# RNG65536/CUDA-volpath

Hardware: AMD Instinct MI355X
Metric: Msamples/sec (WxHxspp) + achieved HBM GB/s, Julia 256^3 @ 800x600 (higher is better)
Workload: dtype f32; 1 GPU; julia256_800x600_global_majorant; image=800x600, estimator=global_majorant, bound_brick=1, rng=philox2x32-7, parallelism=pixel-tiles x1

## Files before the change

### cuda-volpath_amd/csrc/vp_context.cpp

```cpp
#include "vp_state.h"

namespace vph __attribute__((visibility("hidden")))
{
State                      g_default;
static thread_local State* t_current = nullptr;
State& cur() { return t_current ? *t_current : g_default; }

int fail(int code, const char* fmt, ...)
{
    char    buf[512];
    va_list ap;
    va_start(ap, fmt);
    vsnprintf(buf, sizeof buf, fmt, ap);
    va_end(ap);
    G.err = buf;
    return code;
}
[[noreturn]] void die(const char* what)
{
    fprintf(stderr, "volpath_hip: %s: %s\n", what, G.err.c_str());
    exit(EXIT_FAILURE);
}
int ensure_device()
{
    if (G.dev_ready)
    {
        HIPCHK(hipSetDevice(G.device));
        return VP_OK;
    }
    int n = 0;
    if (hipGetDeviceCount(&n) != hipSuccess || n <= 0) return fail(VP_E_NODEVICE, "no HIP device visible");
    if (G.device >= n) return fail(VP_E_NODEVICE, "device %d out of range (%d visible)", G.device, n);
    HIPCHK(hipSetDevice(G.device));
    hipDeviceProp_t prop;
    HIPCHK(hipGetDeviceProperties(&prop, G.device));
    if (strncmp(prop.gcnArchName, "gfx950", 6) != 0)
        return fail(VP_E_NODEVICE, "device %d is %s; this library carries gfx950 code only", G.device, prop.gcnArchName);
    G.num_cu = prop.multiProcessorCount;
    HIPCHK(hipStreamCreateWithFlags(&G.own_stream, hipStreamNonBlocking));
    if (!G.stream) G.stream = G.own_stream;
    HIPCHK(hipMalloc((void**)&G.d_queue, 2 * kTargets * kQueueWords * sizeof(unsigned)));
    HIPCHK(hipMalloc((void**)&G.d_counters, kCounterWords * sizeof(unsigned long long)));
    HIPCHK(hipMemset(G.d_counters, 0, kCounterWords * sizeof(unsigned long long)));
    HIPCHK(hipMalloc((void**)&G.d_cancel, 3 * sizeof(unsigned)));
    HIPCHK(hipMemset(G.d_cancel, 0, 3 * sizeof(unsigned)));
    G.S.sun_cos = 94.0f / sqrtf(94.0f * 94.0f + 0.45f * 0.45f);
    G.S.cam_z   = (float)(-1.0f / tan((double)54.43f * 0.00872664626));
    auto knob = [](const char* name, long lo, long hi, long& out) {
        const char* e = getenv(name);
        if (!e || !*e) return false;
        char* end = nullptr;
        long  v   = strtol(e, &end, 10);
        if (*end || v < lo || v > hi)
        {
            fprintf(stderr, "volpath_hip: ignoring %s=%s (allowed %ld..%ld)\n", name, e, lo, hi);
            return false;
        }
        out = v;
        return true;
    };
    long v;
    if (knob("VP_WAIT_LANES", 1, 64, v)) { G.wait_lanes = (unsigned)v; G.wait_lanes_set = true; }
    if (knob("VP_WAIT_ITERS", VP_STEPS_PER_PASS, 1 << 20, v)) G.wait_iters = (unsigned)v;
    if (knob("VP_SETUP_LANES", 1, 64, v)) G.setup_lanes = (unsigned)v;
    if (knob("VP_END_LANES", 1, 64, v)) G.end_lanes = (unsigned)v;
    if (knob("VP_LIGHT_WAIT_ITERS", VP_STEPS_PER_PASS, 1 << 20, v)) G.light_wait_iters = (unsigned)v;
    if (knob("VP_STAGE_MB", 1, 256 << 10, v)) G.max_stage_bytes = (size_t)v << 20;
    if (knob("VP_BLOCKS_PER_CU", 1, 8, v)) G.blocks_per_cu = (unsigned)v;
    {
        long kmax = 0;
        while ((VP_CHUNK >> (kmax + 1)) >= 1) kmax++;
        if (knob("VP_CHUNK_FRAMES_LOG2", 0, kmax, v)) G.chunk_fshift = (unsigned)v;
    }
    if (knob("VP_NO_LDS_BOUNDS", 0, 1, v)) G.use_lds_bounds = v == 0;
    if (knob("VP_NO_LDS_HELPER", 0, 1, v)) G.lds_helper = v == 0;
    if (knob("VP_NO_LDS_COMPACT", 0, 1, v)) G.use_lds_compact = v == 0;
    if (knob("VP_LDS_COMPACT_CHROMATIC", 0, 1, v)) G.lds_compact_chromatic = v != 0;
    if (knob("VP_LDS_PAIRS", 0, 1, v)) G.lds_pairs = v != 0;
    if (knob("VP_CELL_BRICKS", 0, 1, v)) G.cell_bricks = (int)v;
    if (knob("VP_NO_CRAWL_TABLE", 0, 1, v)) G.use_crawl_table = v == 0;
    if (knob("VP_NO_EMPTY_TABLE", 0, 1, v)) G.use_empty_table = v == 0;
    if (knob("VP_NO_SUN_CLIP", 0, 1, v)) G.use_sun_clip = v == 0;
    if (knob("VP_DENSE_PERCENT", 0, 101, v)) G.dense_fraction = (float)v / 100.0f;
    if (knob("VP_NO_OPACITY_LDS", 0, 1, v)) G.opacity_lds = v == 0;
    if (knob("VP_NO_OPACITY_CELLS", 0, 1, v)) G.use_opacity_cells = v == 0;
    if (knob("VP_NO_LIGHT_CONST", 0, 1, v)) G.use_light_const = v == 0;
    if (knob("VP_NO_CONST_ROWS", 0, 1, v)) G.use_const_rows = v == 0;
    if (knob("VP_NO_APPROACH", 0, 1, v)) G.use_approach = v == 0;
    if (knob("VP_NO_APPROACH_LOCAL", 0, 1, v)) G.use_approach_local = v == 0;
    if (knob("VP_NO_APPROACH_TABLE", 0, 1, v)) G.use_approach_table = v == 0;
    if (knob("VP_APPROACH_FRAMES_LOG2", 0, 6, v)) G.approach_fshift_max = (unsigned)v;
    if (knob("VP_APPROACH_STEPS", 0, 1 << 30, v)) G.approach_steps = (unsigned)v;
    if (knob("VP_NO_LIGHT", 0, 1, v)) G.use_light = v == 0;
    if (knob("VP_NO_LIGHT_OVERLAP", 0, 1, v)) G.light_overlap = v == 0;
    if (knob("VP_NO_LIGHT_LOCAL", 0, 1, v)) G.use_light_local = v == 0;
    if (knob("VP_DEBUG_ONLY_CLASS", 0, 1, v)) G.debug_only_class = (int)v;
    if (knob("VP_GENERAL_BLOCKS_PER_CU", 1, 8, v)) G.general_blocks_per_cu = (unsigned)v;
    if (knob("VP_LIGHT_BLOCKS_PER_CU", 1, 8, v)) G.light_blocks_per_cu = (unsigned)v;
    if (knob("VP_THR_TABLE", 2, 1 << 20, v)) G.thr_entries = (unsigned)v;
    if (knob("VP_LOOKAHEAD", 0, 4096, v)) G.la_max = (int)v;
    if (knob("VP_LOOKAHEAD_OVERLAP_FROM", 1, 4096, v)) G.la_overlap_from = (int)v;
    if (knob("VP_LOOKAHEAD_RAMP_FROM", 2, 4096, v)) G.la_ramp_from = (int)v;
    if (knob("VP_LOOKAHEAD_FLOOR", 1, 4096, v)) G.la_floor = (int)v;
    if (knob("VP_LOOKAHEAD_DIV", 1, 16, v)) G.la_div = (int)v;
    if (knob("VP_LOOKAHEAD_NO_SPECULATION", 0, 1, v)) G.la_speculate = v == 0;
    if (knob("VP_NO_LA_CANCEL", 0, 1, v)) G.la_cancel = v == 0;
    if (knob("VP_NO_PIPELINE", 0, 1, v)) G.pipeline = v == 0;
    if (knob("VP_NO_EXIT", 0, 1, v)) G.use_exit = v == 0;
    if (knob("VP_EXIT_LOCAL", 0, 1, v)) { G.exit_local = v != 0; G.exit_local_auto = false; }
    if (knob("VP_EXIT_K", 1, VP_EXIT_TRIP, v)) G.exit_k = (unsigned)v;
    G.dev_ready = true;
    return VP_OK;
}


hipError_t create_internal_stream(hipStream_t* st)
{
    int lo = 0, hi = 0;
    if (hipDeviceGetStreamPriorityRange(&lo, &hi) != hipSuccess) { (void)hipGetLastError(); lo = hi = 0; }
    return hipStreamCreateWithPriority(st, hipStreamNonBlocking, lo);
}

int free_volume()
{
    G.epoch++;
    (void)la_quiesce();

    if (G.d_cells) HIPCHK(hipFree(G.d_cells));
    if (G.d_bounds) HIPCHK(hipFree(G.d_bounds));
    if (G.d_opacity) HIPCHK(hipFree(G.d_opacity));
    if (G.d_opacity_cells) { if (G.opacity_cells_on_host) HIPCHK(hipHostFree(G.h_opacity_cells)); else HIPCHK(hipFree(G.d_opacity_cells)); }
    G.d_opacity_cells = nullptr; G.h_opacity_cells = nullptr; G.S.opacity_cells = nullptr; G.opacity_cells_on_host = false;
    if (G.d_bound_codes) HIPCHK(hipFree(G.d_bound_codes));
    G.d_bound_codes = nullptr; G.bound_codes_ok = false;
    if (G.d_danger) HIPCHK(hipFree(G.d_danger));
    G.d_danger = nullptr;
    if (G.d_sunclip) HIPCHK(hipFree(G.d_sunclip));
    G.d_sunclip = nullptr; G.sunclip_key.clear();
    if (G.d_exit) HIPCHK(hipFree(G.d_exit));
    G.d_exit = nullptr;
    G.d_cells = G.d_bounds = nullptr;
    G.d_opacity   = nullptr;
    G.S.cells_u8  = nullptr;
    G.S.cells_f32 = nullptr;
    G.S.bounds_u8 = nullptr;
    G.S.bounds_f32 = nullptr;
    G.S.opacity    = nullptr;
    G.have_volume  = false;
    return VP_OK;
}

static int do_init_volume_(const void* h_volume, vp_extent ext, bool quantized, const vp_float3* bmin, const vp_float3* bmax);
int do_init_volume(const void* h_volume, vp_extent ext, bool quantized, const vp_float3* bmin, const vp_float3* bmax)
{
    int rc = do_init_volume_(h_volume, ext, quantized, bmin, bmax);
    if (rc)
    {
        std::string why = G.err;
        (void)free_volume();
        G.err = why;
    }
    return rc;
}
int do_init_volume_(const void* h_volume, vp_extent ext, bool quantized, const vp_float3* bmin, const vp_float3* bmax)
{
    G.epoch++;
    (void)la_quiesce();

    int rc = ensure_device();
    if (rc) return rc;
    if (ext.width == 0 || ext.height == 0 || ext.depth == 0) return fail(VP_E_ARG, "empty volume extent");
    size_t n = ext.width * ext.height * ext.depth;
    if (n > ((size_t)1 << 32) - 1) return fail(VP_E_ARG, "volume of %zu voxels exceeds the 2^32 cell index", n);
    if (ext.width > 4096 || ext.height > 4096 || ext.depth > 4096) return fail(VP_E_ARG, "volume edge > 4096 voxels");
    HIPCHK(hipStreamSynchronize(G.stream));
    rc = free_volume();
    if (rc) return rc;
    const int nx = (int)ext.width, ny = (int)ext.height, nz = (int)ext.depth;
    SceneDev& S = G.S;
    S.nx = nx; S.ny = ny; S.nz = nz;
    if (bmin && bmax)
    {
        S.bmin[0] = bmin->x; S.bmin[1] = bmin->y; S.bmin[2] = bmin->z;
        S.bmax[0] = bmax->x; S.bmax[1] = bmax->y; S.bmax[2] = bmax->z;
    }
    else
    {
        S.bmin[0] = -1.0f; S.bmin[1] = -(float)ny / (float)nx; S.bmin[2] = -(float)nz / (float)nx;
        S.bmax[0] = 1.0f;  S.bmax[1] = (float)ny / (float)nx;  S.bmax[2] = (float)nz / (float)nx;
    }
    for (int a = 0; a < 3; a++) S.linv[a] = 1.0f / (S.bmax[a] - S.bmin[a]);
    G.quant = quantized;
    struct Scratch
    {
        void* p[3] = {nullptr, nullptr, nullptr};
        ~Scratch() { for (void* q : p) if (q) (void)hipFree(q); }
    } tmp;
    void*& d_raw = tmp.p[0];
    void*& d_ta  = tmp.p[1];
    void*& d_tb  = tmp.p[2];
    const size_t vbytes = n * (quantized ? 1 : 4);
    HIPCHK(hipMalloc(&d_raw, vbytes));
    HIPCHK(hipMemcpyAsync(d_raw, h_volume, vbytes, hipMemcpyHostToDevice, G.stream));
    const size_t ncells_bricks = (((size_t)nx + 3) / 4) * (((size_t)ny + 3) / 4) * (((size_t)nz + 3) / 4) * 64;
    const bool   bricks = G.cell_bricks > 0;
    const size_t ncells = bricks ? ncells_bricks : n;
    S.cell_bricks = bricks ? 1 : 0;
    HIPCHK(hipMalloc(&G.d_cells, ncells * (quantized ? 8 : 32)));
    if (bricks && ncells != n) HIPCHK(hipMemsetAsync(G.d_cells, 0, ncells * (quantized ? 8 : 32), G.stream));
    if (quantized) launch_pack_u8((const unsigned char*)d_raw, (uint2*)G.d_cells, nx, ny, nz, bricks, G.stream);
    else launch_pack_f32((const float*)d_raw, (float*)G.d_cells, nx, ny, nz, bricks, G.stream);
    HIPCHK(hipGetLastError());
    G.brick  = G.brick_next;
    G.radius = bound_radius(nx, 0.05f ) + (G.brick > 1 ? 1 : 0);
    int shift = 0;
    while ((1 << shift) < G.brick) shift++;
    S.brick_shift = shift;
    S.bnx = (nx + G.brick - 1) / G.brick; S.bny = (ny + G.brick - 1) / G.brick; S.bnz = (nz + G.brick - 1) / G.brick;
    const size_t nb    = (size_t)S.bnx * S.bny * S.bnz;
    const size_t psize = quantized ? 2 : 8;
    HIPCHK(hipMalloc(&d_ta, n * psize));
// ... 223 lines not shown
}
void gamma_correct(vp_float4* dst, vp_float4* src, int size, float s, float gamma)
{
    if (ensure_device()) die("gamma_correct");
    launch_gamma((float4*)dst, (const float4*)src, size, s, 1.0f / gamma, G.stream);
}

const char* vp_last_error(void) { return G.err.c_str(); }
const char* vp_version(void) { return "volpath_hip 0.3 (gfx950)"; }
int vp_device_count(void)
{
    int n = 0;
    if (hipGetDeviceCount(&n) != hipSuccess) return 0;
    return n;
}
int vp_set_device(int device)
{
    if (G.dev_ready && device != G.device)
        return fail(VP_E_STATE, "this context is bound to device %d; use vp_ctx_create(%d) for another GPU", G.device, device);
    G.device = device;
    return ensure_device();
}

struct vp_ctx { State st; };
vp_ctx* vp_ctx_create(int device)
{
    int n = 0;
    if (hipGetDeviceCount(&n) != hipSuccess || device < 0 || device >= n)
    {
        fail(VP_E_NODEVICE, "vp_ctx_create: device %d not visible (%d devices)", device, n);
        return nullptr;
    }
    vp_ctx* c = new vp_ctx();
    c->st.device = device;
    State* prev = t_current;
    t_current   = &c->st;
    int rc      = ensure_device();
    std::string why = c->st.err;
    t_current   = prev;
    if (rc)
    {
        delete c;
        fail(rc, "vp_ctx_create(%d): %s", device, why.c_str());
        return nullptr;
    }
    return c;
}
int vp_ctx_set_current(vp_ctx* ctx)
{
    t_current = ctx ? &ctx->st : nullptr;
    if (G.dev_ready) HIPCHK(hipSetDevice(G.device));
    return VP_OK;
}
vp_ctx* vp_ctx_get_current(void) { return t_current ? reinterpret_cast<vp_ctx*>(t_current) : nullptr; }
int vp_ctx_device(void) { return G.device; }
int vp_ctx_destroy(vp_ctx* ctx)
{
    if (!ctx) return VP_OK;
    State* prev = t_current;
    t_current   = &ctx->st;
    State& D    = ctx->st;
    int rc = VP_OK;
    if (D.dev_ready)
    {
        (void)hipSetDevice(D.device);
        (void)hipStreamSynchronize(D.stream);
        (void)la_quiesce();
        rc = free_volume();
        free_envmap();
        for (auto& sl : D.la)
        {
            if (sl.done) (void)hipEventDestroy(sl.done);
            if (sl.stream) (void)hipStreamDestroy(sl.stream);
        }
        for (auto& ev : D.events) { (void)hipEventDestroy(ev.first); (void)hipEventDestroy(ev.second); }
        for (auto& ev : D.class_events) { (void)hipEventDestroy(ev.a); (void)hipEventDestroy(ev.b); }
        for (auto e : D.event_pool) (void)hipEventDestroy(e);
        (void)pipe_quiesce();
        for (hipStream_t st : D.pipe_stream) if (st) (void)hipStreamDestroy(st);
        for (hipEvent_t e : {D.pipe_done[0], D.pipe_done[1], D.pipe_free[0], D.pipe_free[1], D.pipe_gate[0], D.pipe_gate[1], D.pipe_fence_ev, D.last_end,
                             D.class_last_end[0], D.class_last_end[1], D.class_last_end[2]})
            if (e) (void)hipEventDestroy(e);
        D.d_crawl.release(); D.d_seg.release(); D.d_sub_cls.release(); D.d_tiles.release(); D.d_act.release(); D.d_act_scratch.release();
        for (void* q : {(void*)D.d_thr, (void*)D.d_sunclip, (void*)D.d_bound_codes, (void*)D.d_light_flag, (void*)D.d_tile_rows, (void*)D.d_tile_scratch})
            if (q) (void)hipFree(q);
        for (RenderTarget& t : D.target)
        {
            if (t.aux_stream) { (void)hipStreamSynchronize(t.aux_stream); (void)hipStreamDestroy(t.aux_stream); }
            t.stage.release();
            t.handover.release();
            for (hipEvent_t e : t.aux_ev) if (e) (void)hipEventDestroy(e);
        }
        if (D.d_queue) (void)hipFree(D.d_queue);
        if (D.d_counters) (void)hipFree(D.d_counters);
        if (D.ctrl_stream) (void)hipStreamDestroy(D.ctrl_stream);
        if (D.d_cancel) (void)hipFree(D.d_cancel);
        if (D.own_stream) (void)hipStreamDestroy(D.own_stream);
    }
    t_current = (prev == &ctx->st) ? nullptr : prev;
    delete ctx;
    if (G.dev_ready) (void)hipSetDevice(G.device);
    return rc;
}
int vp_accumulate(vp_float4* dst, const vp_float4* src, size_t n)
{
    int rc = ensure_device();
    if (rc) return rc;
    if (!dst || !src) return fail(VP_E_ARG, "vp_accumulate: null pointer");
    if (n) launch_accumulate((float4*)dst, (const float4*)src, n, G.stream);
    HIPCHK(hipGetLastError());
    return VP_OK;
}
int vp_tile_owner(unsigned tx, unsigned ty, int world)
{
    if (world < 1) return -1;
    return (int)((tx + vp::tile_row_shift(ty, (unsigned)world)) % (unsigned)world);
}
int vp_set_stream(void* s)
{
    int rc = ensure_device();
    if (rc) return rc;
    HIPCHK(hipStreamSynchronize(G.stream));
    if (la_quiesce()) return VP_E_NODEVICE;
    G.stream = s ? (hipStream_t)s : G.own_stream;
    return VP_OK;
}
void* vp_get_stream(void)
{
    if (ensure_device()) return nullptr;
    return (void*)G.stream;
}
int vp_synchronize(void)
{
    int rc = ensure_device();
    if (rc) return rc;
    HIPCHK(hipStreamSynchronize(G.stream));
    return VP_OK;
}
int vp_set_estimator(int est)
{
    if (int rc = pipe_quiesce()) return rc;
    if (est != VP_EST_GLOBAL && est != VP_EST_DECOMP && est != VP_EST_BOUNDED) return fail(VP_E_ARG, "unknown estimator %d", est);
    G.est = est;
    return VP_OK;
}
int vp_set_rng(int mode, uint32_t k0, uint32_t k1)
{
    if (int rc = pipe_quiesce()) return rc;
    if (mode != VP_RNG_SAMPLERH && mode != VP_RNG_PHILOX && mode != VP_RNG_PHILOX7) return fail(VP_E_ARG, "unknown rng %d", mode);
    G.rng = mode; G.key0 = k0; G.key1 = k1;
    return VP_OK;
}
int vp_set_exit_flights(int mode)
{
    if (mode < 0 || mode > 2) return fail(VP_E_ARG, "exit flights: 0 off, 1 global-majorant estimator (default), 2 every estimator that has them");
    int rc = ensure_device();
    if (rc || (rc = pipe_quiesce())) return rc;
    G.use_exit = mode != 0; G.exit_local = mode == 2; G.exit_local_auto = false;
    if (G.use_exit && G.have_volume && !G.d_exit && G.d_danger)
    {
        if (la_quiesce()) return VP_E_NODEVICE;
        const size_t n = (size_t)G.S.nx * G.S.ny * G.S.nz;
        if (hipMalloc((void**)&G.d_exit, 3 * n) == hipSuccess)
        {
            launch_exit_table(G.d_danger, G.d_exit, G.S.nx, G.S.ny, G.S.nz, G.stream);
            HIPCHK(hipGetLastError());
        }
// ... 277 lines not shown
```

### cuda-volpath_amd/csrc/vp_device.h

```cpp
#pragma once
#include <hip/hip_runtime.h>
#include <stdint.h>

#include "vp_math.h"

namespace vp
{
struct f3 { float x, y, z; };
VP_ARITH_BEGIN
__device__ __forceinline__ f3 mk3(float x, float y, float z) { return f3{x, y, z}; }
__device__ __forceinline__ f3 operator+(f3 a, f3 b) { return f3{a.x + b.x, a.y + b.y, a.z + b.z}; }
__device__ __forceinline__ f3 operator-(f3 a, f3 b) { return f3{a.x - b.x, a.y - b.y, a.z - b.z}; }
__device__ __forceinline__ f3 operator*(f3 a, f3 b) { return f3{a.x * b.x, a.y * b.y, a.z * b.z}; }
__device__ __forceinline__ f3 operator*(f3 a, float s) { return f3{a.x * s, a.y * s, a.z * s}; }
__device__ __forceinline__ f3 operator/(f3 a, float s) { return f3{a.x / s, a.y / s, a.z / s}; }
__device__ __forceinline__ float dot(f3 a, f3 b) { return a.x * b.x + a.y * b.y + a.z * b.z; }
__device__ __forceinline__ f3 cross(f3 a, f3 b)
{
    return f3{a.y * b.z - a.z * b.y, a.z * b.x - a.x * b.z, a.x * b.y - a.y * b.x};
}
__device__ __forceinline__ f3 normalize(f3 v) { return v * rsqrt_(dot(v, v)); }
__device__ __forceinline__ f3 normalize_ieee(f3 v) { return v * (1.0f / __builtin_sqrtf(dot(v, v))); }
__device__ __forceinline__ float max3(f3 v) { return fmaxf(fmaxf(v.x, v.y), v.z); }
__device__ __forceinline__ float min3(f3 v) { return fminf(fminf(v.x, v.y), v.z); }
// ... 292 lines not shown
    if (lz) hi = lo;
    float x00 = lerpf(lo.x, lo.y, fx);
    float x10 = lerpf(lo.z, lo.w, fx);
    float x01 = lerpf(hi.x, hi.y, fx);
    float x11 = lerpf(hi.z, hi.w, fx);
    float y0  = lerpf(x00, x10, fy);
    float y1  = lerpf(x01, x11, fy);
    return lerpf(y0, y1, fz);
}

template <bool QUANT>
__device__ __forceinline__ void sample_bound(const SceneDev& S, f3 pos, float& bmax, float& bmin)
{
    f3  p = to_local(S, pos);
    int i = axis_point(p.x, S.nx) >> S.brick_shift;
    int j = axis_point(p.y, S.ny) >> S.brick_shift;
    int k = axis_point(p.z, S.nz) >> S.brick_shift;
    size_t o = (size_t)((unsigned)i + (unsigned)S.bnx * ((unsigned)j + (unsigned)S.bny * (unsigned)k));
    if (QUANT)
    {
        unsigned short v = reinterpret_cast<const unsigned short*>(S.bounds_u8)[o];
        bmax = (float)(v & 0xffu) * VP_U8_SCALE;
        bmin = (float)(v >> 8) * VP_U8_SCALE;
    }
    else
    {
        float2 v = reinterpret_cast<const float2*>(S.bounds_f32)[o];
        bmax = v.x;
        bmin = v.y;
    }
}

__device__ __forceinline__ f3 eval_envmap(const SceneDev& S, f3 dir)
{
    float phi   = acosf_(dir.y);
    float theta = atanf_(dir.z / dir.x) + kPi2;
    if (dir.x < 0.0f) theta += kPi;
    float  u = theta * k1TwoPi;
    float  v = phi * k1Pi;
    int    i = axis_point(u, S.env_w);
    int    j = axis_point(v, S.env_h);
    float4 t = S.env[(size_t)i + (size_t)S.env_w * (size_t)j];
    return f3{t.x, t.y, t.z};
}

__device__ __forceinline__ float luminance(f3 c)
{
    return (float)((double)c.x * 0.2126 + (double)c.y * 0.7152 + (double)c.z * 0.0722);
}
__device__ __forceinline__ int cdf_search(const float* cdf, int n, float r)
{
    int begin = 0, end = n - 1;
    while (end > begin)
    {
        int   mid = begin + (end - begin) / 2;
        float c   = cdf[mid];
        if (c >= r) end = mid;
        else begin = mid + 1;
    }
    return begin;
}
__device__ __forceinline__ float sample_envmap(const SceneDev& S, float& u, float& v, f3& c)
{
    int iy = cdf_search(S.env_cdf_y, S.env_h, v);
    int ix = cdf_search(S.env_cdf_x + (size_t)iy * (size_t)S.env_w, S.env_w, u);
    u = ((float)ix + 0.5f) / (float)S.env_w;
    v = ((float)iy + 0.5f) / (float)S.env_h;
    int    i = axis_point(u, S.env_w);
    int    j = axis_point(v, S.env_h);
    float4 t = S.env[(size_t)i + (size_t)S.env_w * (size_t)j];
    c        = f3{t.x, t.y, t.z};
    return luminance(c) * S.env_pdfnorm_alt;
}
__device__ __forceinline__ f3 uv_to_dir(float u, float v)
{
    float theta = u * kTwoPi;
    float phi   = v * kPi;
    float st, ct, sp, cp;
    sincosf_(theta, st, ct);
    sincosf_(phi, sp, cp);
    return f3{sp * st, cp, sp * -ct};
}

__device__ __forceinline__ bool intersect_box(f3 o, f3 d, const SceneDev& S, float& tnear, float& tfar)
{
#ifndef VP_EXP_BOX_PARALLEL
    float tmn, tmx;
    {
        const float ir = 1.0f / d.x, tb = ir * (S.bmin[0] - o.x), tt = ir * (S.bmax[0] - o.x);
        tmn = fminf(tt, tb); tmx = fmaxf(tt, tb);
    }
    __builtin_amdgcn_sched_barrier(0);
    float tmn_y, tmx_y;
    {
        const float ir = 1.0f / d.y, tb = ir * (S.bmin[1] - o.y), tt = ir * (S.bmax[1] - o.y);
        tmn_y = fminf(tt, tb); tmx_y = fmaxf(tt, tb);
    }
    __builtin_amdgcn_sched_barrier(0);
    float tmn_z, tmx_z;
    {
        const float ir = 1.0f / d.z, tb = ir * (S.bmin[2] - o.z), tt = ir * (S.bmax[2] - o.z);
        tmn_z = fminf(tt, tb); tmx_z = fmaxf(tt, tb);
    }
    const float lt = max3(f3{tmn, tmn_y, tmn_z}), st_ = min3(f3{tmx, tmx_y, tmx_z});
    tnear = lt; tfar = st_;
    return st_ > lt && st_ >= 1e-3f;
#endif
    f3 invR = f3{1.0f / d.x, 1.0f / d.y, 1.0f / d.z};
    f3 tbot = invR * (f3{S.bmin[0], S.bmin[1], S.bmin[2]} - o);
    f3 ttop = invR * (f3{S.bmax[0], S.bmax[1], S.bmax[2]} - o);
    f3 tmin = f3{fminf(ttop.x, tbot.x), fminf(ttop.y, tbot.y), fminf(ttop.z, tbot.z)};
    f3 tmax = f3{fmaxf(ttop.x, tbot.x), fmaxf(ttop.y, tbot.y), fmaxf(ttop.z, tbot.z)};
    float largest_tmin  = max3(tmin);
    float smallest_tmax = min3(tmax);
    tnear = largest_tmin;
    tfar  = smallest_tmax;
    return smallest_tmax > largest_tmin && smallest_tmax >= 1e-3f;
}

__device__ __forceinline__ bool intersect_box_inv(f3 o, f3 invR, const SceneDev& S, float& tnear, float& tfar)
{
    f3 tbot = invR * (f3{S.bmin[0], S.bmin[1], S.bmin[2]} - o);
    f3 ttop = invR * (f3{S.bmax[0], S.bmax[1], S.bmax[2]} - o);
    f3 tmin = f3{fminf(ttop.x, tbot.x), fminf(ttop.y, tbot.y), fminf(ttop.z, tbot.z)};
    f3 tmax = f3{fmaxf(ttop.x, tbot.x), fmaxf(ttop.y, tbot.y), fmaxf(ttop.z, tbot.z)};
    float largest_tmin  = max3(tmin);
    float smallest_tmax = min3(tmax);
    tnear = largest_tmin;
    tfar  = smallest_tmax;
    return smallest_tmax > largest_tmin && smallest_tmax >= 1e-3f;
}

__device__ __forceinline__ void camera_ray(const SceneDev& S, unsigned width, unsigned height, unsigned px, unsigned py, f3& ro, f3& rd)
{
    float u = ((float)px * 2.0f - (float)width) / (float)width;
    float v = ((float)py * 2.0f - (float)height) / (float)width;
    ro      = f3{S.cam[3], S.cam[7], S.cam[11]};
    f3 dv   = f3{u, v, S.cam_z};
    rd      = normalize_ieee(f3{dot(dv, f3{S.cam[0], S.cam[1], S.cam[2]}), dot(dv, f3{S.cam[4], S.cam[5], S.cam[6]}), dot(dv, f3{S.cam[8], S.cam[9], S.cam[10]})});
}

__host__ __device__ __forceinline__ void subpixel_offset(unsigned px, unsigned py, unsigned frame, unsigned m, unsigned& i, unsigned& j)
{
    const unsigned h = wang_hash(((px << 16) | py) ^ 0x9E3779B9u);
    const unsigned k = (frame + h) & ((1u << (2u * m)) - 1u);
    i = j = 0u;
#pragma unroll
    for (unsigned b = 0; b < 3u; b++)
        if (b < m)
        {
            i |= ((k >> (2u * m - 1u - 2u * b)) & 1u) << b;
            j |= ((k >> (2u * m - 2u - 2u * b)) & 1u) << b;
        }
}

struct Frame
{
    f3 n, t, b;
    __device__ __forceinline__ explicit Frame(f3 normal)
    {
        n    = normal;
        f3 a = (__builtin_fabsf(n.x) >= 0.1f) ? f3{0.0f, 1.0f, 0.0f} : f3{1.0f, 0.0f, 0.0f};
        t    = normalize(cross(a, n));
        b    = cross(n, t);
    }
    __device__ __forceinline__ f3 to_world(f3 c) const { return (t * c.x + b * c.y) + n * c.z; }
};

__device__ __forceinline__ f3 hg_sample_local(float g, float rnd0, float rnd1)
{
    float cos_theta;
    if (__builtin_fabsf(g) > 1e-6f)
    {
        float s   = 2.0f * rnd0 - 1.0f;
        float f   = div_(1.0f - g * g, 1.0f + g * s);
        cos_theta = div_(0.5f, g) * (1.0f + g * g - f * f);
        cos_theta = fmaxf(0.0f, fminf(1.0f, cos_theta));
    }
    else
        cos_theta = 2.0f * rnd0 - 1.0f;
    float sin_theta = sqrt_(1.0f - cos_theta * cos_theta);
    float sp, cp;
    sincos_turns_(rnd1, sp, cp);
    return f3{cp * sin_theta, sp * sin_theta, cos_theta};
}
__device__ __forceinline__ float hg_eval(float g, float cos_theta)
{
    return div_(1.0f - g * g, (4.0f * kPi) * pow15f_(1.0f + g * g - (2.0f * g) * cos_theta));
}

__device__ __forceinline__ float hyperion_s(int n_minus)
{
    return fmaxf(0.0f, fminf(1.0f, (float)n_minus * 0.066666666666666666667f));
}

enum : int
{
    CR_G    = 0,
    CR_OMG2 = 1,
    CR_OPG2 = 2,
// ... 55 lines not shown
```

### cuda-volpath_amd/csrc/vp_integrator.h

```cpp
enum : int
{
    ST_DONE    = 0,
    ST_SETUP   = 1,
    ST_TRACK   = 2,
    ST_SHADOW  = 3,
    EV_SCATTER = 4,
    EV_NEE     = 5,
    EV_BG      = 6,
    EV_WRITE   = 7,
    EV_MIS     = 8,
    EV_HG      = 9
};

#ifndef VP_PAD_STEP
#define VP_PAD_STEP 0
#endif
#ifndef VP_PAD_FETCH
#define VP_PAD_FETCH 0
#endif
#ifndef VP_PAD_EOF
#define VP_PAD_EOF 0
#endif
#ifndef VP_PAD_SETUP
#define VP_PAD_SETUP 0
// ... 22 lines not shown
    }
}

__device__ __forceinline__ unsigned lane_rank(unsigned long long mask)
{
    return __builtin_amdgcn_mbcnt_hi((unsigned)(mask >> 32), __builtin_amdgcn_mbcnt_lo((unsigned)mask, 0u));
}

template <class T, bool COLD>
struct ColdVal;
template <class T>
struct ColdVal<T, true>
{
    static_assert(sizeof(T) == sizeof(float), "one LDS word per lane and field");
    float* p;
    __device__ __forceinline__ explicit ColdVal(float* q) : p(q) {}
    __device__ __forceinline__ operator T() const { return __builtin_bit_cast(T, *p); }
    __device__ __forceinline__ ColdVal& operator=(T v) { *p = __builtin_bit_cast(float, v); return *this; }
};
template <class T>
struct ColdVal<T, false>
{
    T v = T();
    __device__ __forceinline__ explicit ColdVal(float*) {}
    __device__ __forceinline__ operator T() const { return v; }
    __device__ __forceinline__ ColdVal& operator=(T w) { v = w; return *this; }
};
template <bool COLD, int STRIDE>
struct ColdF3;
template <int STRIDE>
struct ColdF3<true, STRIDE>
{
    float* p;
    __device__ __forceinline__ explicit ColdF3(float* q) : p(q) {}
    __device__ __forceinline__ operator f3() const { return f3{p[0], p[STRIDE], p[2 * STRIDE]}; }
    __device__ __forceinline__ ColdF3& operator=(f3 v) { p[0] = v.x; p[STRIDE] = v.y; p[2 * STRIDE] = v.z; return *this; }
};
template <int STRIDE>
struct ColdF3<false, STRIDE>
{
    f3 v = {};
    __device__ __forceinline__ explicit ColdF3(float*) {}
    __device__ __forceinline__ operator f3() const { return v; }
    __device__ __forceinline__ ColdF3& operator=(f3 w) { v = w; return *this; }
};
__device__ __forceinline__ float null_collision_in_empty_space(float t, float sigma_t_prime, float inv_sigma_t)
{
    float mn = __builtin_fabsf(sigma_t_prime * t);
    float Pn = (mn + mn) + mn;
    return t * (sigma_t_prime * wdiv_(inv_sigma_t * Pn, Pn));
}
__device__ __forceinline__ bool null_collision_is_identity(f3 t, float sigma_t_prime, float inv_sigma_t)
{
    const float Ps = __builtin_fabsf(0.0f * t.x) + __builtin_fabsf(0.0f * t.y) + __builtin_fabsf(0.0f * t.z);
    const float Pn = __builtin_fabsf(sigma_t_prime * t.x) + __builtin_fabsf(sigma_t_prime * t.y) + __builtin_fabsf(sigma_t_prime * t.z);
    const float c  = Ps + Pn;
    return Ps == 0.0f && sigma_t_prime * wdiv_(inv_sigma_t * c, Pn) == 1.0f;
}

__global__ void light_identity_k(ParamDev P, int local, const unsigned* mask, unsigned* flag)
{
    const unsigned b = threadIdx.x;
    if (local && !(mask[b >> 5] >> (b & 31u) & 1u)) return;
    if (!local && b) return;
    const float max_sig = max3(f3{P.sigma_t[0], P.sigma_t[1], P.sigma_t[2]});
    const float s       = hyperion_s(0 - 5);
    float sigma_t_prime;
    if (local)
    {
        const float reduction   = (1.0f - s) + s * (1.0f - P.g);
        const float cur_density = reduction * P.density;
        const float d_max       = fmaxf(0.0001f, (float)b * VP_U8_SCALE);
        sigma_t_prime           = max_sig * cur_density * d_max;
    }
    else
    {
        const float cur_density = (1.0f - s) * P.density + s * P.density * (1.0f - P.g);
        sigma_t_prime           = max_sig * cur_density;
    }
    const float inv_sigma_t = rcp_(sigma_t_prime);
    if (!(null_collision_in_empty_space(1.0f, sigma_t_prime, inv_sigma_t) == 1.0f)) atomicAnd(flag, 0u);
}

#ifndef VP_LOCAL_MIN_WAVES
#define VP_LOCAL_MIN_WAVES 6
#endif
constexpr int render_min_waves(int est, bool count, int ldsb, bool ach, bool mis, int trk, bool light, bool cancel)
{
    if (VP_MIN_WAVES > 1) return VP_MIN_WAVES;
    if (light) return count ? 5 : (est != EST_GLOBAL ? VP_LIGHT_LOCAL_MIN_WAVES : VP_LIGHT_MIN_WAVES);
    if (mis || ldsb == 1) return 1;
    if (count) return 4;
    if (est == EST_GLOBAL && trk == 0) return VP_GLOBAL_MIN_WAVES;
    if (trk) return 4;
    return (ach && !cancel) ? VP_LOCAL_MIN_WAVES : 5;
}
template <int EST, class RNG, bool QUANT, bool COUNT, int LDSB, bool ACH, bool MIS, int TRK, bool LIGHT = false, bool CANCEL = false>
__global__ __launch_bounds__(LDSB == 1 ? VP_BLOCK_LDS : VP_BLOCK, render_min_waves(EST, COUNT, LDSB, ACH, MIS, TRK, LIGHT, CANCEL))
void render_k(SceneDev S, LaunchDev L)
{
    __shared__ unsigned short lds_bounds[LDSB == 1 ? VP_LDS_BOUND_ENTRIES : 1];
    __shared__ unsigned lds_codes[LDSB == 2 ? VP_LDS_BOUND_ENTRIES / 16 : 1];
    if (LDSB == 2)
    {
        const uint4* src = reinterpret_cast<const uint4*>(L.bound_codes);
        uint4*       dst = reinterpret_cast<uint4*>(lds_codes);
        const int    n16 = (S.bnx * S.bny * S.bnz + 63) / 64;
        for (int w = threadIdx.x; w < n16; w += VP_BLOCK) dst[w] = src[w];
        __syncthreads();
    }
    if (LDSB == 1)
    {
        const uint4* src = reinterpret_cast<const uint4*>(S.bounds_u8);
        uint4*       dst = reinterpret_cast<uint4*>(lds_bounds);
        const int    n16 = (S.bnx * S.bny * S.bnz * 2 + 15) / 16;
        for (int w = threadIdx.x; w < n16; w += VP_BLOCK_LDS) dst[w] = src[w];
        __syncthreads();
    }
    constexpr unsigned KARG_L_   = ((sizeof(SceneDev) + alignof(LaunchDev) - 1) / alignof(LaunchDev)) * alignof(LaunchDev);
    constexpr unsigned KARG_WDS_ = (KARG_L_ + sizeof(LaunchDev) + 3) / 4;
    __shared__ __attribute__((aligned(16))) unsigned kargs_lds_[KARG_WDS_];
    {
        const unsigned* src = (const unsigned*)__builtin_amdgcn_kernarg_segment_ptr();
        for (unsigned w = threadIdx.x; w < KARG_WDS_; w += (LDSB == 1 ? VP_BLOCK_LDS : VP_BLOCK)) kargs_lds_[w] = src[w];
    }
    constexpr bool LOCAL = EST != EST_GLOBAL;
    constexpr bool TAB = TRK == 0 && LDSB != 1 && !LIGHT && !MIS;
    __shared__ __attribute__((aligned(16))) float coll_tab_[TAB ? VP_COLL_ROWS : 1][CR_WORDS];
    if (TAB && threadIdx.x < VP_COLL_ROWS)
        coll_row_fill(coll_tab_[threadIdx.x], (int)threadIdx.x, L.P.g, L.P.density, max3(f3{L.P.sigma_t[0], L.P.sigma_t[1], L.P.sigma_t[2]}), LOCAL);
    __syncthreads();
    auto coll_row = [&](int n) __attribute__((always_inline)) -> const float* {
        return TAB ? coll_tab_[n < 0 ? 0 : (n > VP_COLL_ROWS - 1 ? VP_COLL_ROWS - 1 : n)] : nullptr;
    };
    constexpr bool EARLY = RNG::kShadowSubstream && !MIS && !LIGHT;
    constexpr bool APPR = EST == EST_GLOBAL && TRK == 0 && !LIGHT && !MIS;
    constexpr bool APPR_L = EST == EST_DECOMP && TRK == 0 && !LIGHT && !MIS;
    constexpr bool EXITC = TRK == 0 && !MIS && !LIGHT && EST != EST_BOUNDED && (QUANT || EST == EST_GLOBAL);
    const ParamDev& P = L.P;
    const f3    sig_t     = f3{P.sigma_t[0], P.sigma_t[1], P.sigma_t[2]};
    const f3    sig_s     = sig_t * f3{P.albedo[0], P.albedo[1], P.albedo[2]};
    const float max_sig   = max3(sig_t);
    const float min_sig   = min3(sig_t);
    const float density   = P.density;

    int      st = ST_DONE;
    bool     exhausted = false;
    constexpr bool COLD = LDSB != 1 && !LIGHT;
    constexpr int  CS_  = COLD ? VP_BLOCK : 1;
    static_assert(!COLD || (LOCAL ? VP_LOCAL_MIN_WAVES : VP_GLOBAL_MIN_WAVES) * (14 * VP_BLOCK * 4 + KARG_WDS_ * 4 + VP_COLL_ROWS * CR_WORDS * 4 + (LDSB == 2 ? VP_LDS_BOUND_ENTRIES / 4 : 0)) <= VP_LDS_BYTES_PER_CU,
                  "cold per-path state: more workgroups per CU than the LDS holds -- lower VP_*_MIN_WAVES for this ARCH");
    __shared__ float cold_[COLD ? 14 : 1][CS_];
    float* const cold_p = &cold_[0][COLD ? threadIdx.x : 0];
    ColdF3<COLD, CS_>       rad(cold_p), pd(cold_p + 3 * CS_);
    ColdVal<float, COLD>    ph(cold_p + 6 * CS_), phase_g(cold_p + 7 * CS_);
    ColdVal<unsigned, COLD> item(cold_p + 8 * CS_);
    ColdVal<unsigned, COLD> px(cold_p + 9 * CS_), py(cold_p + 10 * CS_);
    ColdVal<int, COLD>      frame(cold_p + 11 * CS_);
    ColdVal<int, COLD>      nsc(cold_p + 12 * CS_);
    ColdVal<unsigned, COLD> rng_saved(cold_p + 13 * CS_);
    if (COLD) { rad = f3{0.0f, 0.0f, 0.0f}; pd = f3{0.0f, 0.0f, 0.0f}; ph = 0.0f; phase_g = 0.0f; item = 0u; px = 0u; py = 0u; frame = 0; nsc = 0; rng_saved = 0u; }
    RNG      rng;
    f3       ro = {}, rd = {};
    f3       inv_rd = {};
    f3       thr = {};
    int      seg = 0;
    float    dist = 0, t_end = 0;
    float    t_far = 0, distc = 0, inv_sigma = 0, inv_sigma_t = 0, sigma_t_prime = 0, sigma_c = 0;
    float    cur_density = 0, d_max = 0;
    f3       nee_a = {};
    int      terms = 0;
    f3       nee_c = {}, nee_t = {}, seg_o = {};
    int      nee_stage = 0;
    float    sh_inv_sigma = 0, sh_density = 0;
    float    sig_base = density;
    int      chan = 0;
    float    t_empty = 0.0f;
    float    t_clip = 1e30f;
    bool     ex_clear = false;
    unsigned long long c_load = 0, c_xtest = 0, c_xout = 0, c_xok = 0;
    unsigned zrun = 0;

    unsigned long long c_den = 0, c_bnd = 0, c_opa = 0, c_env = 0, c_sca = 0, c_smp = 0;
    unsigned long long d_iter = 0, d_act = 0, d_outer = 0, d_shadow = 0;
    constexpr bool PROF = COUNT && VP_PROFILE_BLOCKS;
    unsigned long long t_slow = 0, t_fast = 0, t_mark = PROF ? __builtin_amdgcn_s_memtime() : 0ull;
    enum { B_SETUP, B_HALF, B_LOOK, B_EXIT, B_SCATTER, B_NEE, B_HG, B_BG, B_WRITE, B_REFILL, B_GSETUP, B_FETCH, B_ZERO, B_ZERO_SH, B_EXITT, B_NBLK };
    unsigned long long bw[B_NBLK] = {}, bl[B_NBLK] = {};
    unsigned long long hist[3][8] = {};
    unsigned long long ctrl_w = 0, ctrl_l = 0;
    auto tally = [&](int b, bool on) __attribute__((always_inline)) {
        if (PROF)
        {
            unsigned long long m = __ballot(on);
            if (m)
            {
                bw[b] += 1; bl[b] += (unsigned)__popcll(m);
                const int h = b == B_SCATTER ? 0 : b == B_EXIT ? 1 : b == B_SETUP ? 2 : -1;
                if (h >= 0) hist[h][((unsigned)__popcll(m) - 1u) >> 3] += 1;
            }
        }
    };

    const unsigned lane = threadIdx.x & 63u;
    unsigned chunk_s = 0, chunk_n = 0;
    unsigned chunk_q = 0, chunk_f0 = 0;
    bool     queue_empty = false;
    unsigned q_cur   = __builtin_amdgcn_s_getreg((4 - 1) << 11 | 20) & (VP_NQUEUES - 1);
    unsigned q_tried = 0;
    unsigned end_skipped = 0;
    unsigned visits = 0;

    for (;;)
    {
        if (PROF && lane == 0) d_outer++;
        {
#ifdef VP_EXP_FLAT_KARGS
        const char* kargs_ = (const char*)__builtin_amdgcn_kernarg_segment_ptr();
        asm volatile("" : "+s"(kargs_));
#else
        unsigned ko_ = 0;
        asm volatile("" : "+v"(ko_));
        const char* kargs_ = reinterpret_cast<const char*>(kargs_lds_) + ko_;
#endif
        const SceneDev&  S = *reinterpret_cast<const SceneDev*>(kargs_);
        const LaunchDev& L = *reinterpret_cast<const LaunchDev*>(kargs_ + KARG_L_);
        const ParamDev&  P = L.P;
        const f3 sun_dir   = f3{S.sun_dir[0], S.sun_dir[1], S.sun_dir[2]};
        const f3 sun_power = f3{S.sun_power[0], S.sun_power[1], S.sun_power[2]};
        auto start_shadow = [&](f3 end, float inv_s, float den, unsigned stage) __attribute__((always_inline)) {
            f3    sd = normalize(end - ro);
            float tn, tf;
            bool  hitv = intersect_box(ro, sd, S, tn, tf);
            if (!hitv)
            {
                nee_a = f3{1.0f, 1.0f, 1.0f};
                st    = EV_NEE;
            }
            else
            {
                if (tn < 0.0f) tn = 0.0f;
                f3 se       = ro - end;
                t_end       = fminf(tf, sqrt_(dot(se, se)));
                dist        = tn;
                terms       = 0;
                rd          = sd;
                inv_sigma   = inv_s;
                cur_density = den;
                st          = ST_SHADOW;
                rng_saved = rng.enter_shadow(2u * (unsigned)(int)nsc + stage);
                if (COUNT) t_clip = 1e30f;
                if (RNG::kShadowSubstream && stage == 0u && L.sun_clip)
                {
                    f3    pl = to_local(S, ro);
                    int   ci, cj, ck;
                    float w_;
                    axis_linear(pl.x, S.nx, ci, w_);
                    axis_linear(pl.y, S.ny, cj, w_);
                    axis_linear(pl.z, S.nz, ck, w_);
                    const unsigned n = L.sun_clip[(size_t)((unsigned)ci + __umul24((unsigned)S.nx, (unsigned)cj + __umul24((unsigned)S.ny, (unsigned)ck)))];
                    if (n != 0xffffu)
                    {
                        const float tc = (float)n * L.clip_ds;
                        if (COUNT && !L.count_clips) t_clip = tc;
                        else t_end = fminf(t_end, tc);
                    }
                }
            }
        };
        auto segment_medium = [&]() __attribute__((always_inline)) {
            if (LOCAL && TAB) cur_density = coll_row(nsc - 5)[CR_DENS];
            else if (LOCAL)
            {
                float s         = hyperion_s(nsc - 5);
                phase_g         = (1.0f - s) * P.g;
                float reduction = (1.0f - s) + s * (1.0f - P.g);
                cur_density     = TRK ? reduction * sig_base : reduction * density;
            }
        };
        auto next_segment = [&]() __attribute__((always_inline)) {
            st = ST_SETUP;
            if (LOCAL) dist = -1.0f;
            if (EXITC) terms = L.exit_start;
            if (EST == EST_GLOBAL) nsc = nsc + 1;
            if (EST == EST_BOUNDED) seg++;
            if ((EST == EST_BOUNDED ? seg : nsc) >= 800) st = EV_WRITE;
            segment_medium();
        };
        auto finish_light = [&]() __attribute__((always_inline)) {
            rad = rad + sun_power * (((ACH ? f3{thr.x, thr.x, thr.x} : thr) * ph) * nee_a);
            rd  = pd;
            next_segment();
        };
        tally(B_SCATTER, st == EV_SCATTER);
        if (!LIGHT && st == EV_SCATTER)
        {
            vp_pad<VP_PAD_COLL>();
            if (COUNT) c_sca++;
            if (PROF) zrun = 0;
            t_empty = 0.0f;
            if (LOCAL) nsc = nsc + 1;
            const int          n2   = LOCAL ? (nsc - 5) : (nsc - 4);
            const float* const row2 = coll_row(n2);
            const float* const rowp = coll_row(n2 - 1);
            float s2 = hyperion_s(n2);
            float dp2, stp2;
            if (TAB)
            {
                dp2  = row2[CR_DENS];
                stp2 = LOCAL ? row2[CR_STP] * d_max : row2[CR_STP];
            }
            else if (TRK)
            {
                thr  = thr * f3{P.albedo[0], P.albedo[1], P.albedo[2]};
                stp2 = LOCAL ? ((1.0f - s2) + s2 * (1.0f - P.g)) * sig_base : (1.0f - s2) * sig_base + s2 * sig_base * (1.0f - P.g);
                dp2  = stp2;
            }
            else if (LOCAL)
            {
                float reduction2 = (1.0f - s2) + s2 * (1.0f - P.g);
                dp2              = reduction2 * density;
                stp2             = max_sig * dp2 * d_max;
            }
            else
            {
                dp2  = (1.0f - s2) * density + s2 * density * (1.0f - P.g);
                stp2 = max_sig * dp2;
            }
            ph = TAB ? hg_eval_row(rowp, dot(rd, sun_dir)) : hg_eval(phase_g, dot(rd, sun_dir));
            pd = rd;
            if (EARLY)
            {
                Frame fr(rd);
                float r0 = rng.next_a();
                float r1 = rng.next_b();
                pd       = normalize(fr.to_world(TAB ? hg_sample_local_row(rowp, r0, r1) : hg_sample_local(phase_g, r0, r1)));
                if (LOCAL) { const f3 pdv = pd; inv_rd = f3{rcp_(pdv.x), rcp_(pdv.y), rcp_(pdv.z)}; }
            }
            if (MIS)
            {
                sh_inv_sigma = rcp_(stp2);
                sh_density   = dp2;
                nee_stage    = 0;
                nee_c        = sun_power;
                nee_t        = (ACH ? f3{thr.x, thr.x, thr.x} : thr) * ph;
            }
            if (EST == EST_DECOMP && frame > 10 && nsc > 20)
            {
                float op = sample_float_cells(S, S.opacity_cells, ro);
// ... 957 lines not shown
```

### cuda-volpath_amd/csrc/vp_kernels.h

```cpp
#pragma once
#include <hip/hip_runtime.h>

#include "vp_device.h"

#define VP_BLOCK 256
#ifndef VP_BLOCK_LDS
#define VP_BLOCK_LDS 512
#endif
#ifndef VP_MIN_WAVES
#define VP_MIN_WAVES 1
#endif
#define VP_LDS_BYTES_PER_CU (160 * 1024)
#define VP_LDS_BOUND_ENTRIES 32768
#ifndef VP_CHUNK
#define VP_CHUNK 128
#endif
#define VP_NQUEUES 8
#define VP_QUEUE_STRIDE 16
#ifndef VP_WAIT_LANES
#define VP_WAIT_LANES 28
#endif
#ifndef VP_WAIT_ITERS
#define VP_WAIT_ITERS 16
#endif
#ifndef VP_END_LANES
#define VP_END_LANES 4
#endif
#ifndef VP_SETUP_LANES
#define VP_SETUP_LANES 8
#endif
#ifndef VP_LIGHT_MIN_WAVES
#define VP_LIGHT_MIN_WAVES 8
#endif
#ifndef VP_PROFILE_BLOCKS
#define VP_PROFILE_BLOCKS 0
#endif
#ifndef VP_GLOBAL_MIN_WAVES
#define VP_GLOBAL_MIN_WAVES 7
#endif
#ifndef VP_LIGHT_LOCAL_MIN_WAVES
#define VP_LIGHT_LOCAL_MIN_WAVES 7
#endif
#ifndef VP_LIGHT_STEPS_PER_PASS
#define VP_LIGHT_STEPS_PER_PASS 16
#endif
#ifndef VP_STEPS_PER_PASS
#define VP_STEPS_PER_PASS 4
#endif
#define VP_EXIT_TRIP 64

namespace vp
{
__host__ __device__ inline unsigned tile_row_shift(unsigned ty, unsigned world) { return ((ty * 0x9E3779B1u) >> 15) % world; }
constexpr int EST_GLOBAL = 0, EST_DECOMP = 1, EST_BOUNDED = 2;
constexpr int RNG_SAMPLERH = 0, RNG_PHILOX = 1, RNG_PHILOX7 = 2;

struct LaunchDev
{
    ParamDev P;
    int      frame0, nframes;
    unsigned nslots;
    unsigned total_items;
    const unsigned* pixels;
    unsigned stage_stride;
    unsigned slot_base;
    float4*  out;
    float4*  stage;
    const float4* crawl;
    unsigned* queue;
    unsigned chunk_fshift;
    unsigned q_start[VP_NQUEUES + 1];
    unsigned long long* counters;
    unsigned key0, key1;
    unsigned wait_lanes, wait_iters;
    unsigned end_lanes;
    unsigned setup_lanes;
    const unsigned short* sun_clip;
    float    clip_ds;
    unsigned count_clips;
    const float* thr_table;
    unsigned thr_n;
    uint2*   approach_aux;
    unsigned approach;
    unsigned approach_fshift;
    unsigned approach_steps;
    const unsigned char* exit_oct;
    int      exit_start;
    unsigned exit_nbytes;
    unsigned exit_bytes;
    unsigned* cancel;
    unsigned  batch_id;
    unsigned      const_from;
    const float4* stage_const;
    const unsigned* bound_codes;
    unsigned        bound_pal[2];
    const float4* seg_table;
    unsigned sub_shift;
};

void launch_render(const SceneDev& S, const LaunchDev& L, int est, int rng, bool quant, bool count, int lds_form, bool mis, int trk,
                   int blocks, hipStream_t st);
void launch_render_fast(const SceneDev& S, const LaunchDev& L, int est, int rng, bool quant, bool count, int lds_form, bool mis, int trk,
                        int blocks, hipStream_t st);
void launch_render_light(const SceneDev& S, const LaunchDev& L, int est, int rng, bool quant, bool count, int blocks, hipStream_t st);
void launch_miss_fill(const SceneDev& S, const LaunchDev& L, bool local_estimator, hipStream_t st);
void launch_approach(const SceneDev& S, const LaunchDev& L, int est, int rng, bool quant, hipStream_t st);
void launch_approach_fast(const SceneDev& S, const LaunchDev& L, int est, int rng, bool quant, hipStream_t st);
unsigned segment_table_records(void);
void launch_segment_table(const SceneDev& S, unsigned width, unsigned height, const float4* crawl, const unsigned* pixels, unsigned nslots, float4* seg,
                          hipStream_t st);
void launch_thr_table(const ParamDev& P, float* table, unsigned count, hipStream_t st);
void launch_bound_bytes(const unsigned char* bounds, size_t nbricks, unsigned* mask, hipStream_t st);
void launch_light_identity(const ParamDev& P, bool local, const unsigned* mask, unsigned* flag, hipStream_t st);
void launch_light_identity_fast(const ParamDev& P, bool local, const unsigned* mask, unsigned* flag, hipStream_t st);
inline unsigned pixel_list_blocks(unsigned ntiles) { return (unsigned)(((size_t)ntiles * 64 + 1023) / 1024); }
void launch_pixel_lists(unsigned width, unsigned height, unsigned rank, unsigned world, unsigned ntiles, const unsigned* d_row_start,
                        const float4* table, const unsigned char* cls, unsigned* d_block_counts, unsigned* d_totals, unsigned* d_out, hipStream_t st);
void launch_subpixel_classes(const float4* fine, unsigned width, unsigned height, unsigned shift, unsigned char* cls, hipStream_t st);
void launch_env_tables(const float4* env, int w, int h, float* lum, float* row_sum, float* cdf_x, float* cdf_y, float* pdfnorm_alt,
                       hipStream_t st);
void launch_crawl_table(const SceneDev& S, bool quant, unsigned width, unsigned height, bool control_draw, const unsigned char* danger, float4* table,
                        hipStream_t st);
void launch_danger(const SceneDev& S, bool quant, unsigned char* out, unsigned long long* marked, hipStream_t st);
float sun_clip_step(const SceneDev& S);
void launch_sun_clip(const SceneDev& S, const unsigned char* danger, float ds, unsigned short* out, hipStream_t st);
void launch_empty_table(const SceneDev& S, unsigned width, unsigned height, const unsigned char* danger, float4* table, hipStream_t st);
void launch_exit_table(const unsigned char* danger, unsigned char* planes, int nx, int ny, int nz, hipStream_t st);
void launch_reduce(const LaunchDev& L, hipStream_t st);
struct PixelStatsDev { double sum_y, sum_y2; unsigned n, flags; };
struct StatsDev
{
    PixelStatsDev* stats;
    unsigned adaptive;
    unsigned min_frames;
    double   tol, fl;
};
void launch_reduce_stats(const LaunchDev& L, const StatsDev& T, hipStream_t st);
inline unsigned compact_blocks(unsigned n) { return (n + 1023u) / 1024u; }
void launch_compact_active(const unsigned* src, const unsigned n[3], unsigned width, const PixelStatsDev* stats, unsigned* d_block_counts,
                           unsigned* d_totals, unsigned* d_out, hipStream_t st);
void launch_scale_by_count(float4* dst, const float4* src, const PixelStatsDev* stats, int size, float s, hipStream_t st);
void launch_stats_rel_error(float* dst, const PixelStatsDev* stats, int size, float floor_y, hipStream_t st);
void launch_pack_u8(const unsigned char* vol, uint2* cells, int nx, int ny, int nz, bool bricks, hipStream_t st);
void launch_pack_f32(const float* vol, float* cells, int nx, int ny, int nz, bool bricks, hipStream_t st);
void launch_opacity(const SceneDev& S, bool quant, bool lds, const float dir[3], float* out, hipStream_t st);
void launch_build_bounds(const void* d_vol, bool quant, void* d_out, void* d_tmp_a, void* d_tmp_b, int nx, int ny, int nz, int radius, int brick,
                         hipStream_t st);
void launch_julia(unsigned char* grid, int n, hipStream_t st);
void launch_cloud(float* grid, int n, unsigned seed, hipStream_t st);
void launch_scale(float4* dst, const float4* src, int size, float s, hipStream_t st);
void launch_gamma(float4* dst, const float4* src, int size, float s, float inv_gamma, hipStream_t st);
void launch_accumulate(float4* dst, const float4* src, size_t n, hipStream_t st);
void launch_test_hg(const float* g, const float* r0, const float* r1, const float* nrm, const float* cosq, float* dir, float* ev, int n, hipStream_t st);
void launch_test_box(const SceneDev& S, const float* o, const float* d, int* hit, float* tn, float* tf, int n, hipStream_t st);
void launch_test_env(const SceneDev& S, const float* d, float* out, int n, hipStream_t st);
void launch_test_math(int which, const float* in, float* out, int n, hipStream_t st);
void launch_test_hg_fast(const float* g, const float* r0, const float* r1, const float* nrm, const float* cosq, float* dir, float* ev, int n, hipStream_t st);
void launch_test_math_fast(int which, const float* in, float* out, int n, hipStream_t st);
void launch_test_rng(int mode, unsigned x, unsigned y, unsigned f, unsigned k0, unsigned k1, int n, float* out, hipStream_t st);
void launch_test_density(const SceneDev& S, bool quant, const float* pos, float* out, int n, hipStream_t st);
}
```

### cuda-volpath_amd/csrc/vp_kernels.hip

```cpp
#include <hip/hip_runtime.h>

#include <cmath>
#include <cstdio>
#include <cstdlib>

#include "vp_device.h"
#include "vp_kernels.h"

namespace vp
{
#include "vp_integrator.h"

__global__ void thr_table_k(ParamDev P, float* table, unsigned count)
{
    if (threadIdx.x || blockIdx.x) return;
    const float max_sig       = max3(f3{P.sigma_t[0], P.sigma_t[1], P.sigma_t[2]});
    const float s             = hyperion_s(0 - 5);
    const float cur_density   = (1.0f - s) * P.density + s * P.density * (1.0f - P.g);
    const float sigma_t_prime = max_sig * cur_density;
    const float inv_sigma_t   = 1.0f / sigma_t_prime;
    float t = 1.0f;
    for (unsigned n = 0; n < count; n++)
    {
        table[n] = t;
// ... 38 lines not shown
        bool  hit = intersect_box_inv(ro, inv_rd, S, t_near, tf);
        t_near    = fmaxf(t_near, 0.0f);
        float t_far = fminf(tf, 0.05f);
        if (!hit || !(t_near >= t_far)) break;
        float bx, by;
        sample_bound<QUANT>(S, ro + rd * t_near, bx, by);
        draws += (control_draw && by > 0.0f) ? 2u : 1u;
        ro = ro + rd * t_far;
        t_left -= t_far;
    }
    table[2 * idx]     = make_float4(ro.x, ro.y, ro.z, u2f(segs | (draws << 16)));
    table[2 * idx + 1] = make_float4(t_left > 0.0f ? t_left : 0.0f, cls, 0.0f, 0.0f);
}

template <bool QUANT>
__global__ __launch_bounds__(256) void danger_k(SceneDev S, unsigned char* out, unsigned long long* marked)
{
    size_t n   = (size_t)S.nx * S.ny * S.nz;
    size_t idx = (size_t)blockIdx.x * blockDim.x + threadIdx.x;
    if (idx >= n) return;
    int i = (int)(idx % S.nx), j = (int)((idx / S.nx) % S.ny), k = (int)(idx / ((size_t)S.nx * S.ny));
    bool any = false;
    for (int dk = -1; dk <= 1; dk++)
        for (int dj = -1; dj <= 1; dj++)
            for (int di = -1; di <= 1; di++)
            {
                int a = min(max(i + di, 0), S.nx - 1), b = min(max(j + dj, 0), S.ny - 1), c = min(max(k + dk, 0), S.nz - 1);
                size_t o = cell_index(S, a, b, c);
                if (QUANT) { uint2 v = S.cells_u8[o]; any = any || (v.x | v.y) != 0u; }
                else
                {
                    const float4* q = reinterpret_cast<const float4*>(S.cells_f32) + o * 2;
                    float4 lo = q[0], hi = q[1];
                    any = any || lo.x != 0.0f || lo.y != 0.0f || lo.z != 0.0f || lo.w != 0.0f || hi.x != 0.0f || hi.y != 0.0f || hi.z != 0.0f || hi.w != 0.0f;
                }
            }
    bool self;
    {
        size_t o = cell_index(S, i, j, k);
        if (QUANT) { uint2 v = S.cells_u8[o]; self = (v.x | v.y) != 0u; }
        else
        {
            const float4* q = reinterpret_cast<const float4*>(S.cells_f32) + o * 2;
            float4 lo = q[0], hi = q[1];
            self = lo.x != 0.0f || lo.y != 0.0f || lo.z != 0.0f || lo.w != 0.0f || hi.x != 0.0f || hi.y != 0.0f || hi.z != 0.0f || hi.w != 0.0f;
        }
    }
    out[idx] = (unsigned char)((any ? 1 : 0) | (self ? 2 : 0));
    if (marked)
    {
        const unsigned long long m = __ballot(any);
        if ((threadIdx.x & 63u) == (unsigned)__builtin_ctzll(m | (1ull << 63)) && m) atomicAdd(marked, (unsigned long long)__popcll(m));
    }
}
__global__ __launch_bounds__(256) void exit_dir_slice_k(const unsigned char* danger, unsigned char* plane, int nx, int ny, int nz, int axis, int a, int up)
{
    const int n[3]  = {nx, ny, nz};
    const int B     = axis == 0 ? 1 : 0, C = axis == 2 ? 1 : 2;
    const int nb    = n[B], nc = n[C], na = n[axis];
    const int t     = blockIdx.x * blockDim.x + threadIdx.x;
    if (t >= nb * nc) return;
    const int b = t % nb, c = t / nb;
    const size_t st[3] = {1, (size_t)nx, (size_t)nx * ny};
    auto at = [&](int ia, int ib, int ic) -> size_t {
        ib = min(max(ib, 0), nb - 1); ic = min(max(ic, 0), nc - 1);
        return (size_t)ia * st[axis] + (size_t)ib * st[B] + (size_t)ic * st[C];
    };
    const int  an   = up ? a + 1 : a - 1;
    const bool more = an >= 0 && an < na;
    unsigned   bits = 0;
    for (int q = 0; q < 4; q++)
    {
        const int sb = (q & 1) ? 1 : -1, sc = (q & 2) ? 1 : -1;
        const unsigned bit = (up ? 1u : 0u) | ((q & 1) ? 2u : 0u) | ((q & 2) ? 4u : 0u);
        bool ok = !((danger[at(a, b, c)] | danger[at(a, b + sb, c)] | danger[at(a, b, c + sc)] | danger[at(a, b + sb, c + sc)]) & 1);
        if (ok && more)
            ok = ((plane[at(an, b, c)] & plane[at(an, b + sb, c)] & plane[at(an, b, c + sc)] & plane[at(an, b + sb, c + sc)]) >> bit) & 1u;
        bits |= ok ? (1u << bit) : 0u;
    }
    unsigned char* out = plane + at(a, b, c);
    const unsigned mine = up ? 0xaau : 0x55u;
    *out = (unsigned char)((*out & ~mine) | bits);
}
__global__ __launch_bounds__(256) void sun_clip_k(SceneDev S, const unsigned char* danger, float ds, unsigned short* out)
{
    const size_t n   = (size_t)S.nx * S.ny * S.nz;
    const size_t idx = (size_t)blockIdx.x * blockDim.x + threadIdx.x;
    if (idx >= n) return;
    if (!(danger[idx] & 2)) { out[idx] = 0xffffu; return; }
    const int i = (int)(idx % S.nx), j = (int)((idx / S.nx) % S.ny), k = (int)(idx / ((size_t)S.nx * S.ny));
    auto mid = [](int c, int nc) -> float {
        const float lo = c == 0 ? -0.5f : (float)c, hi = c == nc - 1 ? (float)nc - 0.5f : (float)c + 1.0f;
        return 0.5f * (lo + hi);
    };
    const f3 bmin = f3{S.bmin[0], S.bmin[1], S.bmin[2]};
    const f3 ext  = f3{S.bmax[0], S.bmax[1], S.bmax[2]} - bmin;
    const f3 pl   = f3{(mid(i, S.nx) + 0.5f) / (float)S.nx, (mid(j, S.ny) + 0.5f) / (float)S.ny, (mid(k, S.nz) + 0.5f) / (float)S.nz};
    const f3 o    = pl * ext + bmin;
    const f3 sun  = f3{S.sun_dir[0], S.sun_dir[1], S.sun_dir[2]};
    const f3 d    = normalize(sun * 1e10f - o);
    int      last = -1;
    unsigned m    = 0;
    for (; m < 65000u; m++)
    {
        const f3    q  = to_local(S, o + d * ((float)m * ds));
        const float xa = fma_(q.x, (float)S.nx, -0.5f), xb = fma_(q.y, (float)S.ny, -0.5f), xc = fma_(q.z, (float)S.nz, -0.5f);
        if (!(xa >= -1.5f && xa <= (float)S.nx + 0.5f && xb >= -1.5f && xb <= (float)S.ny + 0.5f && xc >= -1.5f && xc <= (float)S.nz + 0.5f)) break;
        int   a, b, c;
        float w_;
        axis_linear(q.x, S.nx, a, w_);
        axis_linear(q.y, S.ny, b, w_);
        axis_linear(q.z, S.nz, c, w_);
        if (danger[(size_t)a + (size_t)S.nx * ((size_t)b + (size_t)S.ny * c)] & 1) last = (int)m;
    }
    out[idx] = (m >= 65000u || !(d.x == d.x && d.y == d.y && d.z == d.z)) ? 0xffffu : (unsigned short)min(last + 2, 0xfffe);
}
template <bool QUANT>
__device__ bool chord_has_positive_minimum(const SceneDev& S, f3 ro, f3 rd)
{
    float t_near, tf;
    if (!intersect_box(ro, rd, S, t_near, tf)) return false;
    float t0   = fmaxf(t_near, 0.0f);
    float cell = fminf(fminf((S.bmax[0] - S.bmin[0]) / (float)S.nx, (S.bmax[1] - S.bmin[1]) / (float)S.ny), (S.bmax[2] - S.bmin[2]) / (float)S.nz);
    float ds   = 0.25f * cell;
    for (unsigned n = 0; n < 200000u; n++)
    {
        float tt = t0 + (float)n * ds;
        if (tt > tf + ds) return false;
        float bx, by;
        sample_bound<QUANT>(S, ro + rd * tt, bx, by);
        if (by > 0.0f) return true;
    }
    return true;
}
__device__ float certified_empty_distance(const SceneDev& S, f3 ro, f3 rd, const unsigned char* danger, float& cls)
{
    float t_near, tf;
    bool  hit = intersect_box(ro, rd, S, t_near, tf);
    cls = 0.0f;
    if (!hit && danger) cls = 2.0f;
    if (!danger || !hit || !(tf == tf) || !(t_near == t_near)) return 0.0f;
    float t0 = fmaxf(t_near, 0.0f);
    float cell = fminf(fminf((S.bmax[0] - S.bmin[0]) / (float)S.nx, (S.bmax[1] - S.bmin[1]) / (float)S.ny), (S.bmax[2] - S.bmin[2]) / (float)S.nz);
    float ds   = 0.25f * cell;
    float t_empty = 1e30f;
    for (unsigned n = 0; n < 200000u; n++)
    {
        float tt = t0 + (float)n * ds;
        if (tt > tf + ds) break;
        f3    p = to_local(S, ro + rd * tt);
        int   i, j, k;
        float w;
        axis_linear(p.x, S.nx, i, w);
        axis_linear(p.y, S.ny, j, w);
        axis_linear(p.z, S.nz, k, w);
        if (danger[(size_t)i + (size_t)S.nx * ((size_t)j + (size_t)S.ny * k)] & 1)
        {
            bool hit_cell = false;
            const float cx = fmaxf(fma_(p.x, (float)S.nx, -0.5f), 0.0f), cy = fmaxf(fma_(p.y, (float)S.ny, -0.5f), 0.0f),
                        cz = fmaxf(fma_(p.z, (float)S.nz, -0.5f), 0.0f);
            const int i0 = max((int)__builtin_floorf(cx - 0.27f), 0), i1 = min((int)__builtin_floorf(cx + 0.27f), S.nx - 1);
            const int j0 = max((int)__builtin_floorf(cy - 0.27f), 0), j1 = min((int)__builtin_floorf(cy + 0.27f), S.ny - 1);
            const int k0 = max((int)__builtin_floorf(cz - 0.27f), 0), k1 = min((int)__builtin_floorf(cz + 0.27f), S.nz - 1);
            for (int c = k0; c <= k1; c++)
                for (int b = j0; b <= j1; b++)
                    for (int a = i0; a <= i1; a++) hit_cell = hit_cell || (danger[(size_t)a + (size_t)S.nx * ((size_t)b + (size_t)S.ny * c)] & 2);
            if (hit_cell)
            {
                t_empty = fmaxf(tt - 2.0f * ds, 0.0f);
                break;
            }
        }
        if (n == 199999u) t_empty = 0.0f;
    }
    if (t_empty >= 1e29f) cls = 1.0f;
    return t_empty > t0 ? t_empty : 0.0f;
}
__global__ __launch_bounds__(256) void empty_table_k(SceneDev S, unsigned width, unsigned height, const unsigned char* danger, float4* table)
{
    unsigned idx = blockIdx.x * blockDim.x + threadIdx.x;
    if (idx >= width * height) return;
    unsigned py = idx / width, px = idx - py * width;
    f3 ro, rd;
    camera_ray(S, width, height, px, py, ro, rd);
    float cls;
    float te = certified_empty_distance(S, ro, rd, danger, cls);
    table[2 * idx]     = make_float4(ro.x, ro.y, ro.z, 0.0f);
    table[2 * idx + 1] = make_float4(te, cls, 0.0f, 0.0f);
}

__global__ __launch_bounds__(256) void reduce_stage_k(LaunchDev L)
{
    unsigned slot = blockIdx.x * blockDim.x + threadIdx.x;
    if (slot >= L.nslots) return;
    unsigned pix = L.pixels[slot];
    size_t   idx = (size_t)(pix & 0xffffu) + (size_t)(pix >> 16) * L.P.width;
    float4   a   = L.out[idx];
    if (slot >= L.const_from)
// ... 721 lines not shown
}
template <int EST, class RNG>
static void launch_render_scalar(const SceneDev& S, const LaunchDev& L, bool quant, int trk, int blocks, hipStream_t st)
{
    const dim3 blk(VP_BLOCK);
    if (quant)
    {
        if (trk == 1) hipLaunchKernelGGL((render_k<EST, RNG, true, false, false, false, false, 1>), dim3(blocks), blk, 0, st, S, L);
        else hipLaunchKernelGGL((render_k<EST, RNG, true, false, false, false, false, 2>), dim3(blocks), blk, 0, st, S, L);
    }
    else
    {
        if (trk == 1) hipLaunchKernelGGL((render_k<EST, RNG, false, false, false, false, false, 1>), dim3(blocks), blk, 0, st, S, L);
        else hipLaunchKernelGGL((render_k<EST, RNG, false, false, false, false, false, 2>), dim3(blocks), blk, 0, st, S, L);
    }
}
template <int EST, class RNG, int LDSB>
static void launch_render3(const SceneDev& S, const LaunchDev& L, bool quant, bool count, bool ach, bool mis, int blocks, hipStream_t st)
{
    if (mis)
    {
        if (ach) launch_render5<EST, RNG, 0, true, true>(S, L, quant, count, blocks, st);
        else launch_render5<EST, RNG, 0, false, true>(S, L, quant, count, blocks, st);
    }
    else if (ach) launch_render5<EST, RNG, LDSB, true, false>(S, L, quant, count, blocks, st);
    else launch_render5<EST, RNG, LDSB, false, false>(S, L, quant, count, blocks, st);
}

template <int EST, int LDSB>
static void launch_render_p7(const SceneDev& S, const LaunchDev& L, bool quant, bool count, bool ach, int blocks, hipStream_t st)
{
    if (ach) launch_render5<EST, RngPhilox7, LDSB, true, false>(S, L, quant, count, blocks, st);
    else launch_render5<EST, RngPhilox7, LDSB, false, false>(S, L, quant, count, blocks, st);
}

template <int EST, class RNGT>
static void launch_light2(const SceneDev& S, const LaunchDev& L, bool quant, bool count, bool ach, int blocks, hipStream_t st)
{
    const dim3 g(blocks), b(VP_BLOCK);
    constexpr bool LOC = EST != EST_GLOBAL;
#define VP_LL(Q, C, A) hipLaunchKernelGGL((render_k<EST, RNGT, Q, C, false, A, false, 0, true>), g, b, 0, st, S, L)
    (void)ach;
    if (LOC && !quant) { if (count) VP_LL(false, true, true); else VP_LL(false, false, true); }
    else { if (count) VP_LL(true, true, true); else VP_LL(true, false, true); }
#undef VP_LL
}
void launch_render_light(const SceneDev& S, const LaunchDev& L, int est, int rng, bool quant, bool count, int blocks, hipStream_t st)
{
    const ParamDev& P = L.P;
    const bool ach = P.sigma_t[0] == P.sigma_t[1] && P.sigma_t[1] == P.sigma_t[2] && P.albedo[0] == P.albedo[1] && P.albedo[1] == P.albedo[2];
#ifdef VP_DEV_BUILD
    if (rng == RNG_SAMPLERH || est == EST_BOUNDED) { fprintf(stderr, "volpath_hip DEV build: this kernel variant is not compiled\n"); abort(); }
#define VP_LE(RNGT)                                                                             \
    do                                                                                          \
    {                                                                                           \
        if (est == EST_DECOMP) launch_light2<EST_DECOMP, RNGT>(S, L, true, count, ach, blocks, st);  \
        else launch_light2<EST_GLOBAL, RNGT>(S, L, true, count, ach, blocks, st);                    \
    } while (0)
    if (rng == RNG_PHILOX) VP_LE(RngPhilox);
    else VP_LE(RngPhilox7);
#else
#define VP_LE(RNGT)                                                                             \
    do                                                                                          \
    {                                                                                           \
        if (est == EST_DECOMP) launch_light2<EST_DECOMP, RNGT>(S, L, quant, count, ach, blocks, st);        \
        else if (est == EST_BOUNDED) launch_light2<EST_BOUNDED, RNGT>(S, L, quant, count, ach, blocks, st); \
        else launch_light2<EST_GLOBAL, RNGT>(S, L, quant, count, ach, blocks, st);                          \
    } while (0)
    if (rng == RNG_PHILOX) VP_LE(RngPhilox);
    else if (rng == RNG_PHILOX7) VP_LE(RngPhilox7);
    else VP_LE(RngSamplerH);
#endif
#undef VP_LE
}
void launch_bound_bytes(const unsigned char* bounds, size_t nbricks, unsigned* mask, hipStream_t st)
{
    unsigned blocks = (unsigned)std::fmin((double)((nbricks + 255) / 256), 1024.0);
    hipLaunchKernelGGL(bound_bytes_k, dim3(blocks ? blocks : 1), dim3(256), 0, st, reinterpret_cast<const unsigned short*>(bounds), nbricks, mask);
}
void launch_light_identity(const ParamDev& P, bool local, const unsigned* mask, unsigned* flag, hipStream_t st)
{
    hipLaunchKernelGGL(light_identity_k, dim3(1), dim3(256), 0, st, P, local ? 1 : 0, mask, flag);
}
void launch_thr_table(const ParamDev& P, float* table, unsigned count, hipStream_t st)
{
    hipLaunchKernelGGL(thr_table_k, dim3(1), dim3(64), 0, st, P, table, count);
}
void launch_miss_fill(const SceneDev& S, const LaunchDev& L, bool local_estimator, hipStream_t st)
{
    if (L.sub_shift)
    {
        hipLaunchKernelGGL(subpixel_fill_k, dim3(((L.nslots << (2u * L.sub_shift)) + 255) / 256), dim3(256), 0, st, S, L);
        return;
    }
    hipLaunchKernelGGL(miss_fill_k, dim3((L.nslots + 255) / 256), dim3(256), 0, st, S, L, local_estimator ? 1 : 0);
}
unsigned segment_table_records(void) { return 2u * VP_SEG_CAP; }
void launch_segment_table(const SceneDev& S, unsigned width, unsigned height, const float4* crawl, const unsigned* pixels, unsigned nslots, float4* seg,
                          hipStream_t st)
{
    hipLaunchKernelGGL(approach_segments_k, dim3((nslots + 255u) / 256u), dim3(256), 0, st, S, width, height, crawl, pixels, nslots, seg);
}
void launch_approach(const SceneDev& S, const LaunchDev& L, int est, int rng, bool quant, hipStream_t st)
{
    const unsigned sh = L.approach_fshift, spb = 256u >> sh;
    const dim3 grid((L.nslots + spb - 1u) / spb, ((unsigned)L.nframes + (1u << sh) - 1u) >> sh);
    if (est == EST_GLOBAL)
    {
        if (rng == RNG_PHILOX7) hipLaunchKernelGGL(approach_k<RngPhilox7>, grid, dim3(256), 0, st, S, L);
        else if (rng == RNG_PHILOX) hipLaunchKernelGGL(approach_k<RngPhilox>, grid, dim3(256), 0, st, S, L);
        else hipLaunchKernelGGL(approach_k<RngSamplerH>, grid, dim3(256), 0, st, S, L);
    }
    else if (quant && L.seg_table && sh == 6u)
    {
        static_assert(VP_SEG_CAP > 64 && VP_SEG_CAP <= 128, "approach_local_tab_k copies a chain with two loads per lane");
        if (rng == RNG_PHILOX7) hipLaunchKernelGGL(approach_local_tab_k<RngPhilox7>, grid, dim3(256), 0, st, S, L);
        else if (rng == RNG_PHILOX) hipLaunchKernelGGL(approach_local_tab_k<RngPhilox>, grid, dim3(256), 0, st, S, L);
        else hipLaunchKernelGGL(approach_local_tab_k<RngSamplerH>, grid, dim3(256), 0, st, S, L);
    }
    else if (quant)
    {
        if (rng == RNG_PHILOX7) hipLaunchKernelGGL((approach_local_k<RngPhilox7, true>), grid, dim3(256), 0, st, S, L);
        else if (rng == RNG_PHILOX) hipLaunchKernelGGL((approach_local_k<RngPhilox, true>), grid, dim3(256), 0, st, S, L);
        else hipLaunchKernelGGL((approach_local_k<RngSamplerH, true>), grid, dim3(256), 0, st, S, L);
    }
    else
    {
        if (rng == RNG_PHILOX7) hipLaunchKernelGGL((approach_local_k<RngPhilox7, false>), grid, dim3(256), 0, st, S, L);
        else if (rng == RNG_PHILOX) hipLaunchKernelGGL((approach_local_k<RngPhilox, false>), grid, dim3(256), 0, st, S, L);
        else hipLaunchKernelGGL((approach_local_k<RngSamplerH, false>), grid, dim3(256), 0, st, S, L);
    }
}
void launch_pixel_lists(unsigned width, unsigned height, unsigned rank, unsigned world, unsigned ntiles, const unsigned* d_row_start,
                        const float4* table, const unsigned char* cls, unsigned* d_block_counts, unsigned* d_totals, unsigned* d_out, hipStream_t st)
{
    PixListDev D;
    D.cls = cls;
    D.width = width; D.height = height; D.rank = rank; D.world = world;
    D.tiles_x = (width + 7) / 8; D.tiles_y = (height + 7) / 8; D.ntiles = ntiles; D.row_start = d_row_start; D.table = table;
    const unsigned nblocks = pixel_list_blocks(ntiles);
    if (!nblocks) return;
    hipLaunchKernelGGL(pixlist_count_k, dim3(nblocks), dim3(VP_PIXLIST_BLOCK), 0, st, D, d_block_counts);
    hipLaunchKernelGGL(pixlist_scan_k, dim3(1), dim3(VP_PIXLIST_BLOCK), 0, st, d_block_counts, nblocks, d_totals);
    hipLaunchKernelGGL(pixlist_write_k, dim3(nblocks), dim3(VP_PIXLIST_BLOCK), 0, st, D, (const unsigned*)d_block_counts, (const unsigned*)d_totals, d_out);
}

void launch_render(const SceneDev& S, const LaunchDev& L, int est, int rng, bool quant, bool count, int lds_form, bool mis, int trk,
                   int blocks, hipStream_t st)
{
    const bool lds_bounds = lds_form != 0;
    if (lds_form == 2 && est == EST_DECOMP && quant && !count && !mis && !trk && !L.cancel && (rng == RNG_PHILOX7 || rng == RNG_PHILOX))
    {
        const ParamDev& Pc = L.P;
        const bool achc = Pc.sigma_t[0] == Pc.sigma_t[1] && Pc.sigma_t[1] == Pc.sigma_t[2] && Pc.albedo[0] == Pc.albedo[1] && Pc.albedo[1] == Pc.albedo[2];
        if (rng == RNG_PHILOX7) launch_render_p7<EST_DECOMP, 2>(S, L, true, false, achc, blocks, st);
        else launch_render3<EST_DECOMP, RngPhilox, 2>(S, L, true, false, achc, false, blocks, st);
        return;
    }
#ifdef VP_DEV_BUILD
    {
        const ParamDev& Pd = L.P;
        const bool achd = Pd.sigma_t[0] == Pd.sigma_t[1] && Pd.sigma_t[1] == Pd.sigma_t[2] && Pd.albedo[0] == Pd.albedo[1] && Pd.albedo[1] == Pd.albedo[2];
        if (trk || mis || !quant || (rng != RNG_PHILOX && rng != RNG_PHILOX7) || est == EST_BOUNDED)
        {
            fprintf(stderr, "volpath_hip DEV build: this kernel variant is not compiled\n");
            abort();
// ... 57 lines not shown
        else launch_render3<EST_GLOBAL, RngSamplerH, 0>(S, L, quant, count, ach, mis, blocks, st);
    }
#endif
}

__global__ void env_lum_k(const float4* env, float* lum, int w, int h)
{
    int i = blockIdx.x * blockDim.x + threadIdx.x;
    if (i >= w * h) return;
    int    y   = i / w;
    float  phi = kPi * ((float)y + 0.5f) / (float)h;
    float  sp, cp;
    sincosf_(phi, sp, cp);
    float4 t = env[i];
    lum[i]   = luminance(f3{t.x, t.y, t.z}) * sp;
}
__global__ void env_row_cdf_k(const float* lum, float* cdf_x, float* row_sum, int w, int h)
{
    int y = blockIdx.x * blockDim.x + threadIdx.x;
    if (y >= h) return;
    const float* f   = lum + (size_t)y * w;
    float*       cdf = cdf_x + (size_t)y * w;
    float        sum = 0.0f;
    for (int i = 0; i < w; i++) sum += f[i];
    float norm = 1.0f / sum;
    float I    = 0.0f;
    for (int i = 0; i < w; i++) { I += f[i] * norm; cdf[i] = I; }
    cdf[w - 1] = 1.0f;
    row_sum[y] = sum;
}
__global__ void env_col_cdf_k(const float* lum, const float* row_sum, float* cdf_y, float* pdfnorm_alt, int w, int h)
{
    if (blockIdx.x || threadIdx.x) return;
    float lumsum = 0.0f;
    for (size_t i = 0, n = (size_t)w * h; i < n; i++) lumsum += lum[i];
    *pdfnorm_alt = (float)w * (float)h * k1TwoPiPi / lumsum;
    float sum = 0.0f;
    for (int i = 0; i < h; i++) sum += row_sum[i];
    float norm = 1.0f / sum;
    float I    = 0.0f;
    for (int i = 0; i < h; i++) { I += row_sum[i] * norm; cdf_y[i] = I; }
    cdf_y[h - 1] = 1.0f;
}
void launch_env_tables(const float4* env, int w, int h, float* lum, float* row_sum, float* cdf_x, float* cdf_y, float* pdfnorm_alt,
                       hipStream_t st)
{
    int n = w * h;
    hipLaunchKernelGGL(env_lum_k, dim3((n + 255) / 256), dim3(256), 0, st, env, lum, w, h);
    hipLaunchKernelGGL(env_row_cdf_k, dim3((h + 63) / 64), dim3(64), 0, st, lum, cdf_x, row_sum, w, h);
    hipLaunchKernelGGL(env_col_cdf_k, dim3(1), dim3(64), 0, st, lum, row_sum, cdf_y, pdfnorm_alt, w, h);
}
void launch_crawl_table(const SceneDev& S, bool quant, unsigned width, unsigned height, bool control_draw, const unsigned char* danger, float4* table,
                        hipStream_t st)
{
    unsigned n = width * height;
    if (quant) hipLaunchKernelGGL(crawl_table_k<true>, dim3((n + 255) / 256), dim3(256), 0, st, S, width, height, control_draw ? 1 : 0, danger, table);
    else hipLaunchKernelGGL(crawl_table_k<false>, dim3((n + 255) / 256), dim3(256), 0, st, S, width, height, control_draw ? 1 : 0, danger, table);
}
void launch_danger(const SceneDev& S, bool quant, unsigned char* out, unsigned long long* marked, hipStream_t st)
{
    size_t n = (size_t)S.nx * S.ny * S.nz;
    dim3   g((unsigned)((n + 255) / 256));
    if (quant) hipLaunchKernelGGL(danger_k<true>, g, dim3(256), 0, st, S, out, marked);
    else hipLaunchKernelGGL(danger_k<false>, g, dim3(256), 0, st, S, out, marked);
}
void launch_exit_table(const unsigned char* danger, unsigned char* planes, int nx, int ny, int nz, hipStream_t st)
{
    const size_t n = (size_t)nx * ny * nz;
    const int    dims[3] = {nx, ny, nz};
    for (int axis = 0; axis < 3; axis++)
    {
        unsigned char* plane = planes + (size_t)axis * n;
        const int      na = dims[axis], cells = (int)(n / (size_t)na);
        const dim3     g((unsigned)((cells + 255) / 256));
        for (int a = na - 1; a >= 0; a--) hipLaunchKernelGGL(exit_dir_slice_k, g, dim3(256), 0, st, danger, plane, nx, ny, nz, axis, a, 1);
        for (int a = 0; a < na; a++) hipLaunchKernelGGL(exit_dir_slice_k, g, dim3(256), 0, st, danger, plane, nx, ny, nz, axis, a, 0);
    }
}
float sun_clip_step(const SceneDev& S)
{
    const float cx = (S.bmax[0] - S.bmin[0]) / (float)S.nx, cy = (S.bmax[1] - S.bmin[1]) / (float)S.ny, cz = (S.bmax[2] - S.bmin[2]) / (float)S.nz;
    return 0.25f * std::fmin(std::fmin(cx, cy), cz);
}
void launch_sun_clip(const SceneDev& S, const unsigned char* danger, float ds, unsigned short* out, hipStream_t st)
{
    size_t n = (size_t)S.nx * S.ny * S.nz;
    hipLaunchKernelGGL(sun_clip_k, dim3((unsigned)((n + 255) / 256)), dim3(256), 0, st, S, danger, ds, out);
}
void launch_empty_table(const SceneDev& S, unsigned width, unsigned height, const unsigned char* danger, float4* table, hipStream_t st)
{
    unsigned n = width * height;
    hipLaunchKernelGGL(empty_table_k, dim3((n + 255) / 256), dim3(256), 0, st, S, width, height, danger, table);
}
void launch_subpixel_classes(const float4* fine, unsigned width, unsigned height, unsigned shift, unsigned char* cls, hipStream_t st)
{
    hipLaunchKernelGGL(subpixel_class_k, dim3((width * height + 255) / 256), dim3(256), 0, st, fine, width, height, shift, cls);
}
void launch_reduce(const LaunchDev& L, hipStream_t st)
{
    unsigned per_frame = L.nslots;
    hipLaunchKernelGGL(reduce_stage_k, dim3((per_frame + 255) / 256), dim3(256), 0, st, L);
}
void launch_reduce_stats(const LaunchDev& L, const StatsDev& T, hipStream_t st)
{
    hipLaunchKernelGGL(reduce_stats_k, dim3((L.nslots + 255) / 256), dim3(256), 0, st, L, T);
}
void launch_compact_active(const unsigned* src, const unsigned n[3], unsigned width, const PixelStatsDev* stats, unsigned* d_block_counts,
                           unsigned* d_totals, unsigned* d_out, hipStream_t st)
{
    CompactDev D;
    D.src = src; D.n[0] = n[0]; D.n[1] = n[1]; D.n[2] = n[2]; D.width = width; D.stats = stats;
    const unsigned nblocks = compact_blocks(n[0] + n[1] + n[2]);
    hipLaunchKernelGGL(compact_count_k, dim3(nblocks), dim3(VP_PIXLIST_BLOCK), 0, st, D, d_block_counts);
    hipLaunchKernelGGL(pixlist_scan_k, dim3(1), dim3(VP_PIXLIST_BLOCK), 0, st, d_block_counts, nblocks, d_totals);
    hipLaunchKernelGGL(compact_write_k, dim3(nblocks), dim3(VP_PIXLIST_BLOCK), 0, st, D, (const unsigned*)d_block_counts, (const unsigned*)d_totals, d_out);
}
void launch_scale_by_count(float4* dst, const float4* src, const PixelStatsDev* stats, int size, float s, hipStream_t st)
{
    hipLaunchKernelGGL(scale_by_count_k, dim3((size + 255) / 256), dim3(256), 0, st, dst, src, stats, size, s);
}
void launch_stats_rel_error(float* dst, const PixelStatsDev* stats, int size, float floor_y, hipStream_t st)
{
    hipLaunchKernelGGL(stats_rel_error_k, dim3((size + 255) / 256), dim3(256), 0, st, dst, stats, size, (double)floor_y);
}
void launch_pack_u8(const unsigned char* vol, uint2* cells, int nx, int ny, int nz, bool bricks, hipStream_t st)
{
    size_t n = (size_t)nx * ny * nz;
    hipLaunchKernelGGL(pack_cells_u8_k, dim3((unsigned)((n + 255) / 256)), dim3(256), 0, st, vol, cells, nx, ny, nz, bricks ? 1 : 0);
}
void launch_pack_f32(const float* vol, float* cells, int nx, int ny, int nz, bool bricks, hipStream_t st)
{
    size_t n = (size_t)nx * ny * nz;
    hipLaunchKernelGGL(pack_cells_f32_k, dim3((unsigned)((n + 255) / 256)), dim3(256), 0, st, vol, cells, nx, ny, nz, bricks ? 1 : 0);
}
void launch_opacity(const SceneDev& S, bool quant, bool lds, const float dir[3], float* out, hipStream_t st)
{
    size_t n = (size_t)S.nx * S.ny * S.nz;
    f3     d = f3{dir[0], dir[1], dir[2]};
    dim3   g((unsigned)((n + 255) / 256));
    if (quant && lds)
    {
        float per_step = 0.0f;
        const int nn[3] = {S.nx, S.ny, S.nz};
        for (int a = 0; a < 3; a++) per_step = fmaxf(per_step, fabsf(dir[a]) * 0.001f * S.linv[a] * (float)nn[a]);
        int chunk = per_step > 0.0f && per_step == per_step ? (int)fminf(5.0f / per_step, 64.0f) : 1;
        if (chunk < 1) chunk = 1;
        const unsigned nb = (unsigned)((S.nx + VP_OPA_B - 1) / VP_OPA_B) * (unsigned)((S.ny + VP_OPA_B - 1) / VP_OPA_B) * (unsigned)((S.nz + VP_OPA_B - 1) / VP_OPA_B);
        hipLaunchKernelGGL(opacity_lds_k, dim3(nb), dim3(VP_OPA_B * VP_OPA_B * VP_OPA_B), 0, st, S, d, out, chunk);
    }
    else if (quant) hipLaunchKernelGGL(opacity_k<true>, g, dim3(256), 0, st, S, d, out);
    else hipLaunchKernelGGL(opacity_k<false>, g, dim3(256), 0, st, S, d, out);
}
template <class PR>
static void build_bounds_t(const void* d_vol, void* d_out, void* d_tmp_a, void* d_tmp_b, int nx, int ny, int nz, int radius, int brick, hipStream_t st)
{
    typedef typename PR::P P;
    size_t   n = (size_t)nx * ny * nz;
    unsigned g = (unsigned)((n + 255) / 256);
    P *a = (P*)d_tmp_a, *b = (P*)d_tmp_b;
    hipLaunchKernelGGL(bounds_init_k<PR>, dim3(g), dim3(256), 0, st, (const typename PR::T*)d_vol, a, n);
    for (int axis = 0; axis < 3; axis++)
    {
        hipLaunchKernelGGL(bounds_pass_k<PR>, dim3(g), dim3(256), 0, st, (const P*)a, b, nx, ny, nz, axis, radius);
        P* t = a; a = b; b = t;
    }
    int bnx = (nx + brick - 1) / brick, bny = (ny + brick - 1) / brick, bnz = (nz + brick - 1) / brick;
    size_t nb = (size_t)bnx * bny * bnz;
    hipLaunchKernelGGL(bounds_brick_k<PR>, dim3((unsigned)((nb + 255) / 256)), dim3(256), 0, st, (const P*)a, (P*)d_out, nx, ny, nz, brick, bnx, bny, bnz);
}
void launch_build_bounds(const void* d_vol, bool quant, void* d_out, void* d_tmp_a, void* d_tmp_b, int nx, int ny, int nz, int radius, int brick,
// ... 56 lines not shown
```

### cuda-volpath_amd/csrc/vp_kernels_fast.hip

```cpp
#define VP_ARITH_FAST 1

#include <hip/hip_runtime.h>

#include <cstdio>
#include <cstdlib>

#include "vp_device.h"
#include "vp_kernels.h"

namespace vp
{
namespace fast
{
#include "vp_integrator.h"
#include "vp_test_kernels.h"

template <int EST, class RNG, bool QUANT, int LDSB, bool ACH>
static void launch_render_t(const SceneDev& S, const LaunchDev& L, int blocks, hipStream_t st)
{
    const dim3 g(blocks), b(LDSB == 1 ? VP_BLOCK_LDS : VP_BLOCK);
    if constexpr (LDSB == 2)
        hipLaunchKernelGGL((render_k<EST, RNG, QUANT, false, 2, ACH, false, 0>), g, b, 0, st, S, L);
    else if (L.cancel)
        hipLaunchKernelGGL((render_k<EST, RNG, QUANT, false, LDSB, ACH, false, 0, false, true>), g, b, 0, st, S, L);
    else
        hipLaunchKernelGGL((render_k<EST, RNG, QUANT, false, LDSB, ACH, false, 0>), g, b, 0, st, S, L);
}
template <int EST, class RNG, bool QUANT, int LDSB>
static void launch_render_a(const SceneDev& S, const LaunchDev& L, bool ach, int blocks, hipStream_t st)
{
    if (ach) launch_render_t<EST, RNG, QUANT, LDSB, true>(S, L, blocks, st);
    else launch_render_t<EST, RNG, QUANT, LDSB, false>(S, L, blocks, st);
}
template <class RNG>
static void launch_render_r(const SceneDev& S, const LaunchDev& L, int est, bool quant, int lds_form, bool ach, int blocks, hipStream_t st)
{
    if (est == EST_GLOBAL)
    {
#ifndef VP_DEV_BUILD
        if (!quant) { launch_render_a<EST_GLOBAL, RNG, false, 0>(S, L, ach, blocks, st); return; }
#endif
        launch_render_a<EST_GLOBAL, RNG, true, 0>(S, L, ach, blocks, st);
        return;
    }
#ifndef VP_DEV_BUILD
    if (!quant) { launch_render_a<EST_DECOMP, RNG, false, 0>(S, L, ach, blocks, st); return; }
#endif
    if (lds_form == 2 && !L.cancel) launch_render_a<EST_DECOMP, RNG, true, 2>(S, L, ach, blocks, st);
    else if (lds_form != 0) launch_render_a<EST_DECOMP, RNG, true, 1>(S, L, ach, blocks, st);
    else launch_render_a<EST_DECOMP, RNG, true, 0>(S, L, ach, blocks, st);
}
}

void launch_render_fast(const SceneDev& S, const LaunchDev& L, int est, int rng, bool quant, bool count, int lds_form, bool mis, int trk,
                        int blocks, hipStream_t st)
{
    if (count || mis || trk || (est != EST_GLOBAL && est != EST_DECOMP) || (rng != RNG_PHILOX && rng != RNG_PHILOX7))
    {
        fprintf(stderr, "volpath_hip: the fast arithmetic mode has no kernel for this configuration\n");
        abort();
    }
#ifdef VP_DEV_BUILD
    if (!quant) { fprintf(stderr, "volpath_hip DEV build: this kernel variant is not compiled\n"); abort(); }
#endif
    const ParamDev& P = L.P;
    const bool ach = P.sigma_t[0] == P.sigma_t[1] && P.sigma_t[1] == P.sigma_t[2] && P.albedo[0] == P.albedo[1] && P.albedo[1] == P.albedo[2];
    if (rng == RNG_PHILOX7) fast::launch_render_r<RngPhilox7>(S, L, est, quant, lds_form, ach, blocks, st);
    else fast::launch_render_r<RngPhilox>(S, L, est, quant, lds_form, ach, blocks, st);
}

void launch_light_identity_fast(const ParamDev& P, bool local, const unsigned* mask, unsigned* flag, hipStream_t st)
{
    hipLaunchKernelGGL(fast::light_identity_k, dim3(1), dim3(256), 0, st, P, local ? 1 : 0, mask, flag);
}

void launch_approach_fast(const SceneDev& S, const LaunchDev& L, int est, int rng, bool quant, hipStream_t st)
{
    if ((est != EST_GLOBAL && est != EST_DECOMP) || (rng != RNG_PHILOX && rng != RNG_PHILOX7))
    {
        fprintf(stderr, "volpath_hip: the fast arithmetic mode has no approach kernel for this configuration\n");
        abort();
    }
    const unsigned sh = L.approach_fshift, spb = 256u >> sh;
    const dim3 grid((L.nslots + spb - 1u) / spb, ((unsigned)L.nframes + (1u << sh) - 1u) >> sh);
    const bool p7 = rng == RNG_PHILOX7;
    if (est == EST_GLOBAL)
    {
        if (p7) hipLaunchKernelGGL(fast::approach_k<RngPhilox7>, grid, dim3(256), 0, st, S, L);
        else hipLaunchKernelGGL(fast::approach_k<RngPhilox>, grid, dim3(256), 0, st, S, L);
    }
    else if (quant && L.seg_table && sh == 6u)
    {
        if (p7) hipLaunchKernelGGL(fast::approach_local_tab_k<RngPhilox7>, grid, dim3(256), 0, st, S, L);
        else hipLaunchKernelGGL(fast::approach_local_tab_k<RngPhilox>, grid, dim3(256), 0, st, S, L);
    }
    else if (quant)
    {
        if (p7) hipLaunchKernelGGL((fast::approach_local_k<RngPhilox7, true>), grid, dim3(256), 0, st, S, L);
        else hipLaunchKernelGGL((fast::approach_local_k<RngPhilox, true>), grid, dim3(256), 0, st, S, L);
    }
    else
    {
#ifndef VP_DEV_BUILD
        if (p7) hipLaunchKernelGGL((fast::approach_local_k<RngPhilox7, false>), grid, dim3(256), 0, st, S, L);
        else hipLaunchKernelGGL((fast::approach_local_k<RngPhilox, false>), grid, dim3(256), 0, st, S, L);
#else
        fprintf(stderr, "volpath_hip DEV build: this kernel variant is not compiled\n");
        abort();
#endif
    }
}

void launch_test_hg_fast(const float* g, const float* r0, const float* r1, const float* nrm, const float* cosq, float* dir, float* ev, int n, hipStream_t st)
{
    hipLaunchKernelGGL(fast::test_hg_k, dim3((n + 255) / 256), dim3(256), 0, st, g, r0, r1, nrm, cosq, dir, ev, n);
}
void launch_test_math_fast(int which, const float* in, float* out, int n, hipStream_t st)
{
    hipLaunchKernelGGL(fast::test_math_k, dim3((n + 255) / 256), dim3(256), 0, st, which, in, out, n);
}
}
```

### cuda-volpath_amd/csrc/vp_render.cpp

```cpp
#include "vp_state.h"

namespace vph __attribute__((visibility("hidden")))
{
static float span_ms(hipEvent_t a, hipEvent_t b, hipEvent_t& end)
{
    float ms = 0.0f, since = 0.0f;
    if (hipEventElapsedTime(&ms, a, b) != hipSuccess) { (void)hipGetLastError(); return 0.0f; }
    if (end && hipEventElapsedTime(&since, end, b) == hipSuccess)
    {
        if (since <= 0.0f) return 0.0f;
        ms = std::min(ms, since);
    }
    else (void)hipGetLastError();
    end = b;
    return std::max(ms, 0.0f);
}
static void fold_span(hipEvent_t a, hipEvent_t b, hipEvent_t& end, double& sum)
{
    hipEvent_t e = end;
    if (hipEventQuery(b) == hipSuccess) sum += span_ms(a, b, e);
    else (void)hipGetLastError();
    put_event(a);
    if (e == b) { put_event(end); end = b; }
    else put_event(b);
// ... 102 lines not shown
{
    if (G.pipe_free_set[ps]) HIPCHK(hipStreamWaitEvent(st, G.pipe_free[ps], 0));
    if (G.pipe_gate_set[ps ^ 1]) HIPCHK(hipStreamWaitEvent(st, G.pipe_gate[ps ^ 1], 0));
    G.pipe_gate_set[ps] = false;
    if (G.pipe_fence)
    {
        HIPCHK(hipEventRecord(G.pipe_fence_ev, G.stream));
        HIPCHK(hipStreamWaitEvent(st, G.pipe_fence_ev, 0));
        G.pipe_fence = false;
    }
    G.pipe_busy = true;
    return VP_OK;
}
static int pipe_await_launch(int ps, hipStream_t st)
{
    HIPCHK(hipEventRecord(G.pipe_done[ps], st));
    HIPCHK(hipStreamWaitEvent(G.stream, G.pipe_done[ps], 0));
    return VP_OK;
}
int check_render(unsigned what, const Param* p, long long last_frame)
{
    if (what & CHK_STATE)
    {
        if (!G.have_volume) return fail(VP_E_STATE, "render before init_cuda");
        if (!G.have_env) return fail(VP_E_STATE, "render before init_envmap");
        if (!G.have_sun) return fail(VP_E_STATE, "render before set_sun");
        if (!G.have_cam) return fail(VP_E_STATE, "render before copy_inv_view_matrix");
    }
    if ((what & CHK_IMAGE) && (p->width == 0 || p->height == 0 || p->width > 65535 || p->height > 65535))
        return fail(VP_E_ARG, (what & CHK_IMAGE_NOTE) ? "image %ux%u out of range (sampler.h packs x<<16|y)" : "image %ux%u out of range", p->width, p->height);
    if (what & CHK_MODES)
    {
        if (G.trk && G.env_mis) return fail(VP_E_STATE, "scalar tracking builds exist with passive environment lighting only");
        if (G.trk && G.count) return fail(VP_E_STATE, "work counters are not built for the scalar tracking kernels");
        if (G.rng == VP_RNG_PHILOX7 && (G.trk || G.env_mis))
            return fail(VP_E_STATE, "VP_RNG_PHILOX7 is built for spectral tracking with passive environment lighting only");
        if (G.arith == VP_ARITH_FAST)
        {
            if (G.rng == VP_RNG_SAMPLERH) return fail(VP_E_STATE, "VP_ARITH_FAST is not built for VP_RNG_SAMPLERH (the parity mode is exact by definition)");
            if (G.est == VP_EST_BOUNDED) return fail(VP_E_STATE, "VP_ARITH_FAST is not built for VP_EST_BOUNDED");
            if (G.env_mis) return fail(VP_E_STATE, "VP_ARITH_FAST is built for passive environment lighting only");
            if (G.trk) return fail(VP_E_STATE, "VP_ARITH_FAST is built for spectral tracking only");
            if (G.count) return fail(VP_E_STATE, "work counters are not built for VP_ARITH_FAST");
        }
        if (int rc = subpixel_check(p)) return rc;
    }
    if ((what & CHK_OPACITY) && G.est == VP_EST_DECOMP && last_frame > 10 && !G.S.opacity)
        return fail(VP_E_NOOPACITY, "frames beyond 10 need precompute_opacity (kernel.cu:2183, host.cpp:336-343)");
    return VP_OK;
}
static bool approach_built()
{
    const bool dense_volume = G.marked_fraction > G.dense_fraction;
    return G.use_approach && !G.sub_shift && (G.est == VP_EST_GLOBAL || (G.est == VP_EST_DECOMP && G.use_approach_local && !dense_volume)) && !G.trk && !G.env_mis;
}
static bool approach_possible(const float4* crawl, unsigned n_general) { return approach_built() && crawl && n_general; }
struct LaunchPlan
{
    Target     T;
    bool       lookahead;
    bool       stage_only;
    const StatsDev* stats;
    PixelLists PL;
    size_t     per_frame;
    bool       staged;
    bool       light_const;
    bool       approach, approach_thr, appr_aux_needed;
    bool       piped; int slot;
    size_t     max_f;
    bool both() const { return PL.n_light && PL.n_general && !light_const; }
    size_t sized_frames(int f) const { return std::min<size_t>(stage_only ? std::max<size_t>((size_t)f, (size_t)std::max(G.la_max, 1)) : (size_t)f, max_f); }
};
static int prepare_tables(const Param* p, const Shard& sh, int nframes, const PixelLists* lists, LaunchDev& L, LaunchPlan& A)
{
    int rc = VP_OK;
    L.sub_shift = (unsigned)G.sub_shift;
    const Param fine = subpixel_param(p);
    if ((rc = ensure_crawl_table(&fine, &L.crawl))) return rc;
    if ((rc = ensure_pixel_lists(p, L.crawl, sh))) return rc;
    const PixelLists& PL = A.PL = lists ? *lists : PixelLists{G.d_tiles, G.n_general, G.n_light, G.n_miss};
    A.per_frame = (size_t)PL.n_general + PL.n_light + PL.n_miss;
    if (A.per_frame == 0) return VP_OK;
    if ((rc = ensure_sun_clip(&L.sun_clip, &L.clip_ds))) return rc;
    L.count_clips = getenv("VP_DEBUG_COUNT_CLIPS") ? 1u : 0u;
    if ((rc = exit_flights(L))) return rc;
    A.light_const = false;
    if (PL.n_light && (rc = ensure_light_const(p, &A.light_const))) return rc;
    G.last_light_const = A.light_const ? 1 : 0;
    if (G.est == VP_EST_GLOBAL && PL.n_light && !A.light_const)
    {
        if ((rc = ensure_thr_table(p, &L.thr_table))) return rc;
        L.thr_n = G.thr_entries;
    }
    A.approach = A.approach_thr = false;
    if (approach_possible(L.crawl, PL.n_general) && (!G.count || getenv("VP_COUNT_APPROACH")))
    {
        bool identity = true;
        if (G.est == VP_EST_GLOBAL) rc = G.arith == VP_ARITH_FAST ? ensure_fast_identity(p, &identity) : ensure_light_identity(p, &identity);
        if (rc) return rc;
        A.approach = identity || G.arith != VP_ARITH_FAST;
        if (!identity && A.approach)
        {
            if ((rc = ensure_thr_table(p, &L.thr_table))) return rc;
            L.thr_n  = G.thr_entries;
            A.approach_thr = true;
        }
    }
    L.seg_table = nullptr;
    if (A.approach && G.est == VP_EST_DECOMP && G.approach_fshift_max >= 6 && !lists)
    {
        const float4* seg = nullptr;
        if ((rc = ensure_segment_table(p, L.crawl, &seg))) return rc;
        if (nframes >= 64) L.seg_table = seg;
    }
    return VP_OK;
}
static int plan_target(int nframes, const Target* tgt, const PixelLists* lists, LaunchPlan& A)
{
    A.staged = nframes > 1 || A.stage_only || A.stats;
    A.T      = tgt ? *tgt : Target{&G.target[0], G.stream};
    A.max_f  = A.staged ? stage_frames_cap(A.per_frame, A.T.rt->stage.bytes) : 1;
    A.appr_aux_needed = A.approach && G.est == VP_EST_DECOMP && A.staged;
    A.slot  = G.pipe_next;
    A.piped = !tgt && !A.stage_only && !lists && !A.stats && nframes > 1 && G.pipeline && !G.count && pipe_target(A.per_frame, nframes, A.appr_aux_needed, &A.T);
    if (A.piped) A.max_f = (size_t)nframes;
    else if (!tgt) G.pipe_fence = true;
    G.last_pipelined = A.piped ? 1 : 0;
    if (!A.appr_aux_needed) return VP_OK;
    const size_t one = A.per_frame * sizeof(uint2);
    return reserve_handover(A.T, one * std::min<size_t>((size_t)nframes, A.max_f), one * A.sized_frames(nframes));
}
static int reserve_launch_stage(LaunchPlan& A, int f, bool* smaller)
{
    *smaller = false;
    const size_t exact = A.per_frame * (size_t)f * sizeof(float4);
    const int rc = reserve_stage(A.T, exact, A.per_frame * A.sized_frames(f) * sizeof(float4));
    if (rc || exact <= A.T.rt->stage.bytes) return rc;
    if (A.stage_only) return fail(VP_E_NOMEM, "no memory for a look-ahead batch of %d frames", f);
    if (f <= 1) return fail(VP_E_NOMEM, "no memory for one staged frame (%zu bytes)", exact);
    A.max_f = (size_t)std::max(f / 2, 1);
    *smaller = true;
    return VP_OK;
}

static int brick_table_form(const LaunchPlan& A, const Param* p, const SceneDev& S)
{
    const bool lds_bounds = G.use_lds_bounds && G.est == VP_EST_DECOMP && G.quant && !G.env_mis && !G.trk &&
                            (size_t)S.bnx * S.bny * S.bnz <= (size_t)VP_LDS_BOUND_ENTRIES;
    const bool ach_lds = p->sigma_t.x == p->sigma_t.y && p->sigma_t.y == p->sigma_t.z && p->albedo.x == p->albedo.y && p->albedo.y == p->albedo.z;
    const bool timed_l  = !G.count && !A.lookahead;
    const bool timed_cb = timed_l && G.rng != VP_RNG_SAMPLERH;
    return !lds_bounds ? 0 : (G.bound_codes_ok && G.d_bound_codes && timed_cb && (ach_lds || G.lds_compact_chromatic)) ? 2
                             : (timed_l && !G.lds_pairs) ? 0 : 1;
}
static bool brick_table_helper(const LaunchPlan& A, int lds_form) { return lds_form == 1 && G.lds_helper && A.PL.n_general && !(A.PL.n_light && !A.light_const) && !A.lookahead; }
struct ClassGrid { bool ldsb; unsigned blocks, cap, wait_iters; };
static ClassGrid class_grid(const LaunchPlan& A, int cls, int lds_form, unsigned total_items)
{
    ClassGrid g;
    g.ldsb = lds_form == 1 && !cls;
    const unsigned bsz  = g.ldsb ? VP_BLOCK_LDS : VP_BLOCK;
    unsigned waves  = (total_items + 63) / 64;
    g.blocks = (waves + (bsz / 64) - 1) / (bsz / 64);
    const bool     both = A.both();
    unsigned       bpc  = G.blocks_per_cu;
    if (both && cls) bpc = G.light_blocks_per_cu ? G.light_blocks_per_cu : (G.est == VP_EST_GLOBAL ? 2u : 6u);
// ... 284 lines not shown
    for (auto& ev : G.events) tot += span_ms(ev.first, ev.second, end);
    if (total_ms) *total_ms = tot;
    if (launches) *launches = G.timed_n;
    if (reset)
    {
        for (auto& ev : G.events) { put_event(ev.first); if (ev.second != end) put_event(ev.second); }
        if (end != G.last_end) { put_event(G.last_end); G.last_end = end; }
        G.events.clear();
        G.timed_ms = 0.0; G.timed_n = 0;
    }
    return VP_OK;
}
int vp_last_approach_mode(void) { return G.last_approach; }
int vp_last_approach_table(void) { return G.last_approach_table; }
int vp_last_light_const(void) { return G.last_light_const; }
int vp_last_lds_form(void) { return G.last_lds_form; }
int vp_last_arithmetic(void) { return G.last_arith; }
int vp_last_pipelined(void) { return G.last_pipelined; }
int vp_set_pipeline(int on)
{
    int rc = pipe_quiesce();
    if (rc) return rc;
    G.pipeline = on != 0;
    return VP_OK;
}
int vp_lookahead_stats(unsigned* launched, unsigned* cancelled_in_flight)
{
    if (launched) *launched = G.la_launched;
    if (cancelled_in_flight) *cancelled_in_flight = G.la_cancelled;
    return VP_OK;
}
int vp_render_class_time_ms(double ms[3], unsigned pixels[3], int reset)
{
    if (int rc = await_launches(true, true)) return rc;
    double     tot[3] = {G.class_ms[0], G.class_ms[1], G.class_ms[2]};
    hipEvent_t end[3] = {G.class_last_end[0], G.class_last_end[1], G.class_last_end[2]};
    for (auto& ev : G.class_events) tot[ev.cls] += span_ms(ev.a, ev.b, end[ev.cls]);
    if (ms) for (int i = 0; i < 3; i++) ms[i] = tot[i];
    if (pixels) { pixels[0] = G.n_general; pixels[1] = G.n_light; pixels[2] = G.n_miss; }
    if (reset)
    {
        for (auto& ev : G.class_events) { put_event(ev.a); if (ev.b != end[ev.cls]) put_event(ev.b); }
        for (int i = 0; i < 3; i++)
            if (end[i] != G.class_last_end[i]) { put_event(G.class_last_end[i]); G.class_last_end[i] = end[i]; }
        G.class_events.clear();
        G.class_ms[0] = G.class_ms[1] = G.class_ms[2] = 0.0;
    }
    return VP_OK;
}
int vp_get_pixel_lists(const Param* p, uint32_t* dst, size_t count, unsigned counts[3])
{
    int rc = vp_prepare(p);
    if (rc) return rc;
    const size_t n = (size_t)G.n_general + G.n_light + G.n_miss;
    if (counts) { counts[0] = G.n_general; counts[1] = G.n_light; counts[2] = G.n_miss; }
    if (dst)
    {
        if (count < n) return fail(VP_E_ARG, "pixel lists hold %zu entries", n);
        if (n) HIPCHK(hipMemcpy(dst, G.d_tiles, n * sizeof(unsigned), hipMemcpyDeviceToHost));
    }
    return VP_OK;
}
int vp_prepare(const Param* p)
{
    int rc = ensure_device();
    if (rc) return rc;
    if (!p) return fail(VP_E_ARG, "vp_prepare: null Param");
    if (!G.have_volume || !G.have_cam) return fail(VP_E_STATE, "vp_prepare needs a volume and a camera");
    if ((rc = check_render(CHK_IMAGE, p))) return rc;
    const Shard sh = shard_of(p);
    if (sh.per_frame == 0)
    {
        G.n_general = G.n_light = G.n_miss = 0; G.tiles_key.clear();
        return VP_OK;
    }
    if ((rc = subpixel_check(p))) return rc;
    const float4 *table = nullptr, *seg = nullptr;
    const unsigned short* sc = nullptr; float ds = 0.0f;
    const float* thr = nullptr;
    const Param fine = subpixel_param(p);
    if ((rc = ensure_crawl_table(&fine, &table))) return rc;
    if ((rc = ensure_pixel_lists(p, table, sh))) return rc;
    if (G.have_sun && (rc = ensure_sun_clip(&sc, &ds))) return rc;
    if (G.est == VP_EST_GLOBAL && G.n_light && (rc = ensure_thr_table(p, &thr))) return rc;
    if (G.est == VP_EST_DECOMP && G.approach_fshift_max >= 6 && approach_possible(table, G.n_general) && (rc = ensure_segment_table(p, table, &seg))) return rc;
    HIPCHK(hipStreamSynchronize(G.stream));
    return VP_OK;
}
int vp_reserve_frames(const Param* p, int nframes)
{
    int rc = ensure_device();
    if (rc) return rc;
    if (!p || nframes <= 0) return fail(VP_E_ARG, "vp_reserve_frames: bad arguments");
    if ((rc = check_render(CHK_IMAGE, p))) return rc;
    const Shard sh = shard_of(p);
    if (sh.per_frame == 0 || nframes == 1) return VP_OK;
    const Target T      = {&G.target[0], G.stream};
    const size_t f      = std::min<size_t>((size_t)nframes, stage_frames_cap(sh.per_frame, T.rt->stage.bytes));
    const size_t need   = sh.per_frame * f * sizeof(float4);
    const size_t need4  = (G.est == VP_EST_DECOMP && approach_built()) ? sh.per_frame * f * sizeof(uint2) : 0;
    if ((rc = reserve_handover(T, need4, need4))) return rc;
    if (need > T.rt->stage.bytes)
    {
        if (la_quiesce()) return VP_E_NODEVICE;
        HIPCHK(hipStreamSynchronize(G.stream));
        (void)reserve_stage(T, need, need, true);
        if (need > T.rt->stage.bytes) return VP_OK;
    }
    if (G.pipeline && f == (size_t)nframes && pipe_streams()) (void)pipe_reserve(1, sh.per_frame, nframes, need4 > 0);
    return VP_OK;
}
}
```

### cuda-volpath_amd/csrc/vp_state.h

```cpp
#pragma once
#include <hip/hip_runtime.h>

#include <cmath>
#include <cstdarg>
#include <cstdio>
#include <cstdlib>
#include <cstring>
#include <deque>
#include <string>
#include <chrono>
#include <vector>

#include "../../include/volpath.h"
#include "vp_kernels.h"

namespace vph __attribute__((visibility("hidden")))
{
using namespace vp;

inline int bound_radius(int nx, float search_radius)
{
    float cell_size = 2.0f / (float)nx;
    return (int)std::ceil(search_radius / cell_size);
}
// ... 71 lines not shown
        hipEvent_t  done = nullptr;
        bool        valid = false;
        unsigned    const_from = 0;
        unsigned    launched_seq = 0;
        unsigned    cancel_seq = 0;
        bool        touched = false;
        int         first = 0, count = 0;
        std::vector<unsigned char> key;
    } la[2];
    hipStream_t ctrl_stream = nullptr;
    unsigned*   d_cancel    = nullptr;
    RenderTarget target[kTargets];
    bool        la_cancel   = true;
    int         la_prev_n   = 0;
    int         la_last     = -2;
    std::vector<unsigned char> la_key;
    int         trk         = 0;
    bool        env_mis     = false;
    bool        env_tables  = false;
    float*      d_env_cdf_x = nullptr;
    float*      d_env_cdf_y = nullptr;
    bool        linear      = false;
    int         brick_next  = 1;
    int         brick       = 1;
    int         radius      = 0;
    int         est         = VP_EST_DECOMP;
    int         rng         = VP_RNG_SAMPLERH;
    unsigned    key0 = 0, key1 = 0;
    unsigned    rank = 0, world = 1;
    bool        pipeline      = true;
    hipStream_t pipe_stream[2] = {nullptr, nullptr};
    hipEvent_t  pipe_done[2]   = {nullptr, nullptr};
    hipEvent_t  pipe_free[2]   = {nullptr, nullptr};
    bool        pipe_free_set[2] = {false, false};
    hipEvent_t  pipe_gate[2]   = {nullptr, nullptr};
    bool        pipe_gate_set[2] = {false, false};
    hipEvent_t  pipe_fence_ev = nullptr;
    bool        pipe_fence    = true;
    bool        pipe_busy     = false;
    int         pipe_next     = 0;
    int         last_pipelined = 0;
    unsigned*   d_queue       = nullptr;
    unsigned long long* d_counters = nullptr;
    bool        count       = false;
    bool        use_opacity_cells = true;
    bool        opacity_cells_on_host = false;
    void*       h_opacity_cells = nullptr;
    bool        opacity_lds = true;
    bool        wait_lanes_set = false;
    unsigned    wait_lanes  = VP_WAIT_LANES, wait_iters = VP_WAIT_ITERS, setup_lanes = VP_SETUP_LANES, end_lanes = VP_END_LANES, light_wait_iters = 0;
    unsigned    blocks_per_cu = 8;
    unsigned    chunk_fshift = 0;
    bool        use_lds_bounds = true;
    bool        use_lds_compact = true;
    bool        lds_compact_chromatic = true;
    bool        lds_pairs = false;
    unsigned*   d_bound_codes = nullptr;
    unsigned    bound_pal[2] = {0, 0};
    bool        bound_codes_ok = false;
    bool        lds_helper  = true;
    int         cell_bricks = 0;
    bool        use_crawl_table = true;
    bool        use_empty_table = true;
    bool        use_light   = true;
    bool        use_light_local = true;
    int         debug_only_class = -1;
    DevBuf<unsigned> d_tiles;
    unsigned    n_general   = 0, n_light = 0, n_miss = 0;
    std::vector<unsigned char> tiles_key;
    unsigned*   d_tile_rows = nullptr;
    unsigned*   d_tile_scratch = nullptr;
    std::vector<unsigned char> tiles_shape_key;
    DevBuf<unsigned> d_act, d_act_scratch;
    bool        light_overlap = true;
    unsigned    general_blocks_per_cu = 0, light_blocks_per_cu = 0;
    unsigned char* d_danger = nullptr;
    DevBuf<float4> d_crawl;
    std::vector<unsigned char> crawl_key;
    float       marked_fraction = 0.0f, dense_fraction = 0.40f;
    bool        use_sun_clip = true;
    unsigned short* d_sunclip = nullptr;
    float       sunclip_ds  = 0.0f;
    std::vector<unsigned char> sunclip_key;
    bool        use_light_const = true;
    int         last_approach = 0;
    int         last_approach_table = 0;
    int         last_light_const = 0;
    int         last_lds_form = 0;
    int         arith       = VP_ARITH_EXACT;
    int         last_arith  = VP_ARITH_EXACT;
    int         sub_shift   = subpixel_env_shift();
    DevBuf<unsigned char> d_sub_cls;
    unsigned    la_launched = 0, la_cancelled = 0;
    bool        use_const_rows = true;
    unsigned    last_const_from = 0;
    bool        use_approach_table = true;
    DevBuf<float4> d_seg;
    std::vector<unsigned char> seg_key;
    bool        use_approach_local = true;
    bool        use_approach = true;
    unsigned    approach_fshift_max = 6;
    unsigned    approach_steps = 1u << 20;
    unsigned*   d_light_flag = nullptr;
    bool        bound_mask_valid = false;
    unsigned    h_bound_mask[8] = {};
    bool        use_exit    = true;
    bool        exit_local  = false;
    bool        exit_local_auto = true;
    unsigned    exit_k      = 8;
    unsigned char* d_exit   = nullptr;
    float       light_key[7] = {};
    unsigned long long light_epoch = ~0ull;
    bool        light_const = false;
    float       fast_identity_key[5] = {};
    bool        fast_identity_valid = false, fast_identity = false;
    float*      d_thr       = nullptr;
    float       thr_key[5]  = {};
    bool        thr_valid   = false;
    unsigned    thr_entries = 4096;
    std::deque<std::pair<hipEvent_t, hipEvent_t>> events;
    std::vector<hipEvent_t> event_pool;
    hipEvent_t  last_end    = nullptr;
    double      timed_ms    = 0.0;
    int         timed_n     = 0;
    struct ClassEv { int cls; hipEvent_t a, b; };
    std::deque<ClassEv> class_events;
    double      class_ms[3] = {0.0, 0.0, 0.0};
    hipEvent_t  class_last_end[3] = {nullptr, nullptr, nullptr};
    size_t      max_stage_bytes = (size_t)16 << 30;
    float       inv_model[12] = {1, 0, 0, 0, 0, 1, 0, 0, 0, 0, 1, 0};
    std::string err;
};
State& cur();
#define G vph::cur()
constexpr size_t kMaxPendingEvents = 64;

constexpr size_t kQueueWords = VP_NQUEUES * VP_QUEUE_STRIDE;
constexpr size_t kCounterWords = 76;

int fail(int code, const char* fmt, ...);
[[noreturn]] void die(const char* what);
#define HIPCHK(expr)                                                                            \
    do                                                                                          \
    {                                                                                           \
        hipError_t e_ = (expr);                                                                 \
        if (e_ != hipSuccess)                                                                   \
        {                                                                                       \
            if (e_ == hipErrorOutOfMemory) (void)hipGetLastError();  \
            return fail(e_ == hipErrorOutOfMemory ? VP_E_NOMEM : VP_E_NODEVICE, "%s -> %s", #expr, hipGetErrorString(e_)); \
        }                                                                                       \
    } while (0)

int        ensure_device();
hipError_t create_internal_stream(hipStream_t* st);
int        free_volume();
int        do_init_volume(const void* h_volume, vp_extent ext, bool quantized, const vp_float3* bmin, const vp_float3* bmax);
int        do_envmap(const vp_float4* data, int w, int h);
int        build_env_tables();
hipEvent_t get_event();
inline void put_event(hipEvent_t e) { if (e) G.event_pool.push_back(e); }
struct Shard { unsigned tiles_x, tiles_y, owned; size_t per_frame; };
Shard  shard_of(const Param* p);
size_t stage_frames_cap(size_t per_frame, size_t have_bytes);
int    do_opacity(const float* dir);
int    ensure_crawl_table(const Param* p, const float4** out);
Param  subpixel_param(const Param* p);
int    subpixel_check(const Param* p);
int    ensure_sun_clip(const unsigned short** out, float* ds);
int    ensure_light_const(const Param* p, bool* out);
int    ensure_light_identity(const Param* p, bool* out);
int    ensure_fast_identity(const Param* p, bool* out);
int    ensure_bound_mask();
int    exit_flights(LaunchDev& L);
int    ensure_thr_table(const Param* p, const float** out);
int    ensure_pixel_lists(const Param* p, const float4* table, const Shard& sh);
int    ensure_segment_table(const Param* p, const float4* crawl, const float4** out);
struct Target { RenderTarget* rt; hipStream_t stream; };
struct PixelLists { const unsigned* pixels; unsigned n_general, n_light, n_miss; };
int  do_render(vp_float4* d_out, int first, int nframes, const Param* p, bool stage_only = false, const Target* tgt = nullptr,
               const PixelLists* lists = nullptr, const StatsDev* stats = nullptr);
enum : unsigned { CHK_STATE = 1, CHK_IMAGE = 2, CHK_IMAGE_NOTE = 4, CHK_MODES = 8, CHK_OPACITY = 16 };
int  check_render(unsigned what, const Param* p, long long last_frame = 0);
void trim_events();
int  pipe_quiesce();
void render_key(const Param* p, std::vector<unsigned char>& key);
bool la_cancel_running();
int  la_quiesce();
int  la_render_slot(int si, vp_float4* d_out, int first, int n, const Param* p, const std::vector<unsigned char>& key);
int  la_limit(int first, int n, size_t per_frame, size_t have_bytes);
int  serve_frame(vp_float4* d_out, int frame, const Param* p);
}
```

### cuda-volpath_amd/csrc/vp_tables.cpp

```cpp
#include "vp_state.h"

namespace vph __attribute__((visibility("hidden")))
{
int do_opacity(const float* dir)
{
    G.epoch++;
    (void)la_quiesce();

    if (!G.have_volume) return fail(VP_E_STATE, "precompute_opacity before init_cuda");
    size_t n = (size_t)G.S.nx * G.S.ny * G.S.nz;
    if (!G.d_opacity) HIPCHK(hipMalloc((void**)&G.d_opacity, n * sizeof(float)));
    SceneDev S = G.S;
    S.linear   = G.linear ? 1 : 0;
    launch_opacity(S, G.quant, G.opacity_lds, dir, G.d_opacity, G.stream);
    HIPCHK(hipGetLastError());
    const size_t cbytes = n * 8 * sizeof(float);
    if (G.d_opacity_cells && (G.opacity_cells_on_host != !G.use_opacity_cells))
    {
        if (G.opacity_cells_on_host) HIPCHK(hipHostFree(G.h_opacity_cells)); else HIPCHK(hipFree(G.d_opacity_cells));
        G.d_opacity_cells = nullptr; G.h_opacity_cells = nullptr;
    }
    if (!G.d_opacity_cells)
    {
        G.opacity_cells_on_host = !G.use_opacity_cells;
        if (G.use_opacity_cells && hipMalloc((void**)&G.d_opacity_cells, cbytes) != hipSuccess)
        {
            (void)hipGetLastError();
            G.d_opacity_cells = nullptr;
            G.opacity_cells_on_host = true;
        }
        if (!G.d_opacity_cells)
        {
            void* h = nullptr;
            if (hipHostMalloc(&h, cbytes, hipHostMallocMapped | hipHostMallocPortable) != hipSuccess)
            {
                (void)hipGetLastError();
                return fail(VP_E_NOMEM, "no memory for the integrator's copy of the optical-depth table (%zu bytes), on the device or pinned on the host", cbytes);
            }
            void* d = nullptr;
            if (hipHostGetDevicePointer(&d, h, 0) != hipSuccess || !d) { (void)hipGetLastError(); (void)hipHostFree(h); return fail(VP_E_NOMEM, "pinned host memory is not visible to the device"); }
            G.d_opacity_cells = (float*)d; G.h_opacity_cells = h;
            if (G.use_opacity_cells)
                fprintf(stderr, "volpath_hip: no device memory for the integrator's copy of the optical-depth table (%zu MB): it lies in pinned host "
                                "memory, frames from 11 on are read across the bus (same results, slow)\n", cbytes >> 20);
        }
    }
    launch_pack_f32(G.d_opacity, G.d_opacity_cells, G.S.nx, G.S.ny, G.S.nz, false, G.stream);
    HIPCHK(hipGetLastError());
    G.S.opacity = G.d_opacity;
    G.S.opacity_cells = G.d_opacity_cells;
    return VP_OK;
}


Shard shard_of(const Param* p)
{
    Shard s;
    s.tiles_x = (p->width + 7) / 8;
    s.tiles_y = (p->height + 7) / 8;
    s.owned   = 0;
    s.per_frame = 0;
    for (unsigned ty = 0; ty < s.tiles_y; ty++)
    {
        const unsigned rows = std::min(8u, p->height - ty * 8u);
        for (unsigned tx = (G.rank + G.world - tile_row_shift(ty, G.world)) % G.world; tx < s.tiles_x; tx += G.world)
        {
            s.owned++;
            s.per_frame += (size_t)rows * std::min(8u, p->width - tx * 8u);
        }
    }
    return s;
}
size_t stage_frames_cap(size_t per_frame, size_t have_bytes)
{
    size_t cap = G.max_stage_bytes;
    size_t free_b = 0, total_b = 0;
    if (hipMemGetInfo(&free_b, &total_b) == hipSuccess) cap = std::min(cap, std::max(have_bytes, (free_b + have_bytes) / 4));
    else (void)hipGetLastError();
    size_t f = cap / (per_frame * sizeof(float4));
    f = std::min<size_t>(f, 0xfffffff0u / per_frame);
    return std::max<size_t>(f, 1);
}

Param subpixel_param(const Param* p)
{
    Param f = *p;
    f.width <<= G.sub_shift; f.height <<= G.sub_shift;
    return f;
}
int subpixel_check(const Param* p)
{
    if (!G.sub_shift) return VP_OK;
    const unsigned s = 1u << G.sub_shift;
    if ((unsigned long long)p->width * s > 65536ull || (unsigned long long)p->height * s > 65536ull)
        return fail(VP_E_ARG, "image %ux%u with sub-pixel factor %u: the %llux%llu sample image is out of range (x << 16 | y)", p->width, p->height, s,
                    (unsigned long long)p->width * s, (unsigned long long)p->height * s);
    if (((unsigned long long)p->width * s) * ((unsigned long long)p->height * s) > 0xfffffff0ull)
        return fail(VP_E_ARG, "image %ux%u with sub-pixel factor %u: the sample image has too many pixels for its 32-bit table index", p->width, p->height, s);
    if ((unsigned long long)p->width * p->height * 64ull > 0xfffffff0ull) return fail(VP_E_ARG, "image %ux%u too large for a sub-pixel factor", p->width, p->height);
    if (G.count) return fail(VP_E_STATE, "work counters are not built for sub-pixel sampling");
    return VP_OK;
}

int ensure_crawl_table(const Param* p, const float4** out)
{
    *out = nullptr;
    const bool global = G.est == VP_EST_GLOBAL;
    if (global ? !(G.use_empty_table && G.d_danger && G.linear) : !G.use_crawl_table) return VP_OK;
    struct K { SceneDev S; unsigned w, h; int control, quant, global; unsigned long long epoch; };
    std::vector<unsigned char> key(sizeof(K), 0);
    K* k = reinterpret_cast<K*>(key.data());
    memcpy(&k->S, &G.S, sizeof(SceneDev));
    k->S.linear = G.linear ? 1 : 0; k->S.env = nullptr; k->S.opacity = nullptr; k->S.opacity_cells = nullptr; k->S.env_cdf_x = k->S.env_cdf_y = nullptr;
    k->S.env_w = k->S.env_h = 0; k->S.env_pdfnorm_alt = 0.0f;
    memset(k->S.sun_dir, 0, sizeof k->S.sun_dir); memset(k->S.sun_power, 0, sizeof k->S.sun_power); memset(k->S.sun_orig, 0, sizeof k->S.sun_orig);
    k->w = p->width; k->h = p->height;
    k->control = (G.est == VP_EST_DECOMP && G.trk == VP_TRACK_SPECTRAL) ? 1 : 0;
    k->quant = G.quant; k->epoch = G.epoch; k->global = global ? 1 : 0;
    const size_t need = (size_t)p->width * p->height * 2 * sizeof(float4);
    if (key != G.crawl_key || !G.d_crawl)
    {
        if (la_quiesce()) return VP_E_NODEVICE;
        HIPCHK(hipStreamSynchronize(G.stream));
        if (need > G.d_crawl.bytes)
        {
            G.crawl_key.clear();
            if (G.d_crawl.grow(need) != hipSuccess)
            {
                if (G.sub_shift) return fail(VP_E_NOMEM, "no memory for the %ux%u per-pixel table of the sub-pixel factor %d (%zu bytes)", p->width, p->height, 1 << G.sub_shift, need);
                return VP_OK;
            }
        }
        if (global)
        {
            SceneDev S = G.S;
            S.linear   = 1;
            launch_empty_table(S, p->width, p->height, G.d_danger, G.d_crawl, G.stream);
        }
        else
        {
            SceneDev S = G.S;
            S.linear   = G.linear ? 1 : 0;
            launch_crawl_table(S, G.quant, p->width, p->height, k->control != 0, G.use_empty_table ? G.d_danger : nullptr, G.d_crawl, G.stream);
        }
        HIPCHK(hipGetLastError());
        HIPCHK(hipStreamSynchronize(G.stream));
        G.crawl_key = key;
    }
    *out = G.d_crawl;
    return VP_OK;
}

int ensure_sun_clip(const unsigned short** out, float* ds)
{
    *out = nullptr; *ds = 0.0f;
    if (!G.use_sun_clip || G.rng == VP_RNG_SAMPLERH || !G.d_danger || !G.linear) return VP_OK;
    if (G.marked_fraction > G.dense_fraction) return VP_OK;
    struct K { int nx, ny, nz, quant; float bmin[3], bmax[3], sun[3]; unsigned long long epoch; };
    std::vector<unsigned char> key(sizeof(K), 0);
    K* k = reinterpret_cast<K*>(key.data());
    k->nx = G.S.nx; k->ny = G.S.ny; k->nz = G.S.nz; k->quant = G.quant; k->epoch = G.epoch;
    memcpy(k->bmin, G.S.bmin, sizeof k->bmin); memcpy(k->bmax, G.S.bmax, sizeof k->bmax); memcpy(k->sun, G.S.sun_dir, sizeof k->sun);
    if (key != G.sunclip_key || !G.d_sunclip)
    {
        if (la_quiesce()) return VP_E_NODEVICE;
        HIPCHK(hipStreamSynchronize(G.stream));
        const size_t n = (size_t)G.S.nx * G.S.ny * G.S.nz;
        if (!G.d_sunclip && hipMalloc((void**)&G.d_sunclip, n * sizeof(unsigned short)) != hipSuccess)
        {
            (void)hipGetLastError();
            G.d_sunclip = nullptr;
            return VP_OK;
        }
        SceneDev S = G.S;
        S.linear   = 1;
        G.sunclip_ds = sun_clip_step(S);
        launch_sun_clip(S, G.d_danger, G.sunclip_ds, G.d_sunclip, G.stream);
        HIPCHK(hipGetLastError());
        HIPCHK(hipStreamSynchronize(G.stream));
        G.sunclip_key = key;
    }
    *out = G.d_sunclip; *ds = G.sunclip_ds;
    return VP_OK;
}

int ensure_light_const(const Param* p, bool* out)
{
    *out = false;
    if (!G.use_light_const || G.count) return VP_OK;
    return ensure_light_identity(p, out);
}
int ensure_bound_mask()
{
    if (G.bound_mask_valid) return VP_OK;
    if (!G.d_light_flag) HIPCHK(hipMalloc((void**)&G.d_light_flag, 9 * sizeof(unsigned)));
    HIPCHK(hipMemsetAsync(G.d_light_flag + 1, 0, 8 * sizeof(unsigned), G.stream));
    launch_bound_bytes((const unsigned char*)G.d_bounds, (size_t)G.S.bnx * G.S.bny * G.S.bnz, G.d_light_flag + 1, G.stream);
    HIPCHK(hipGetLastError());
    HIPCHK(hipMemcpyAsync(G.h_bound_mask, G.d_light_flag + 1, sizeof G.h_bound_mask, hipMemcpyDeviceToHost, G.stream));
    HIPCHK(hipStreamSynchronize(G.stream));
    G.bound_mask_valid = true;
    return VP_OK;
}
int exit_flights(LaunchDev& L)
{
    L.exit_oct = nullptr; L.exit_start = -(1 << 30); L.exit_nbytes = 0; L.exit_bytes = 0;
    if (!G.use_exit || !G.d_exit || !G.linear || G.trk || G.env_mis || G.est == VP_EST_BOUNDED) return VP_OK;
    if (G.est != VP_EST_GLOBAL)
    {
        const bool local_on = G.exit_local_auto ? G.rng != VP_RNG_SAMPLERH : G.exit_local;
        if (!local_on || !G.quant) return VP_OK;
        int rc = ensure_bound_mask();
        if (rc) return rc;
        unsigned nb = 0, packed = 0;
        for (unsigned b = 0; b < 256; b++)
            if (G.h_bound_mask[b >> 5] >> (b & 31u) & 1u)
            {
                if (nb < 4) packed |= b << (8u * nb);
                nb++;
            }
        if (nb == 0 || nb > 4) return VP_OK;
        L.exit_nbytes = nb; L.exit_bytes = packed;
    }
    L.exit_oct   = G.d_exit;
    L.exit_start = VP_EXIT_TRIP - (int)G.exit_k;
    return VP_OK;
}
int ensure_light_identity(const Param* p, bool* out)
{
    *out = false;
    if (G.trk != VP_TRACK_SPECTRAL || G.est == VP_EST_BOUNDED) return VP_OK;
    const bool local = G.est != VP_EST_GLOBAL;
    if (local && !G.quant) return VP_OK;
    const float key[7] = {p->sigma_t.x, p->sigma_t.y, p->sigma_t.z, p->density, p->g, (float)G.est, (float)G.brick};
    if (G.light_epoch != G.epoch || memcmp(key, G.light_key, sizeof key) != 0)
    {
        if (!G.d_light_flag) HIPCHK(hipMalloc((void**)&G.d_light_flag, 9 * sizeof(unsigned)));
        if (local)
        {
            int rcm = ensure_bound_mask();
            if (rcm) return rcm;
        }
        const unsigned one = 1u;
        unsigned flag = 0u;
        HIPCHK(hipMemcpyAsync(G.d_light_flag, &one, sizeof one, hipMemcpyHostToDevice, G.stream));
        ParamDev P;
        memcpy(&P, p, sizeof(Param));
        launch_light_identity(P, local, G.d_light_flag + 1, G.d_light_flag, G.stream);
        HIPCHK(hipGetLastError());
        HIPCHK(hipMemcpyAsync(&flag, G.d_light_flag, sizeof flag, hipMemcpyDeviceToHost, G.stream));
        HIPCHK(hipStreamSynchronize(G.stream));
        G.light_const = flag == 1u;
        memcpy(G.light_key, key, sizeof key);
        G.light_epoch = G.epoch;
    }
    *out = G.light_const;
    return VP_OK;
}

int ensure_fast_identity(const Param* p, bool* out)
{
    const float key[5] = {p->sigma_t.x, p->sigma_t.y, p->sigma_t.z, p->density, p->g};
    if (!G.fast_identity_valid || memcmp(key, G.fast_identity_key, sizeof key) != 0)
    {
        if (!G.d_light_flag) HIPCHK(hipMalloc((void**)&G.d_light_flag, 9 * sizeof(unsigned)));
// ... 104 lines not shown
    if (light && G.sub_shift)
    {
        HIPCHK(G.d_sub_cls.grow((size_t)p->width * p->height));
        launch_subpixel_classes(table, p->width, p->height, (unsigned)G.sub_shift, G.d_sub_cls, G.stream);
        HIPCHK(hipGetLastError());
        cls = G.d_sub_cls;
    }
    launch_pixel_lists(p->width, p->height, G.rank, G.world, sh.owned, G.d_tile_rows, light ? table : nullptr, cls, G.d_tile_scratch, d_totals, G.d_tiles, G.stream);
    HIPCHK(hipGetLastError());
    unsigned totals[3] = {0, 0, 0};
    HIPCHK(hipMemcpyAsync(totals, d_totals, sizeof totals, hipMemcpyDeviceToHost, G.stream));
    HIPCHK(hipStreamSynchronize(G.stream));
    if ((size_t)totals[0] + totals[1] + totals[2] != sh.per_frame)
        return fail(VP_E_STATE, "pixel lists hold %zu pixels, the shard has %zu", (size_t)totals[0] + totals[1] + totals[2], sh.per_frame);
    G.n_general = totals[0]; G.n_light = totals[1]; G.n_miss = totals[2];
    G.tiles_key = key;
    return VP_OK;
}

}

using namespace vph;

extern "C" {
int vp_get_bound_table(void* dst, size_t bytes, int* bnx, int* bny, int* bnz, int* brick, int* radius)
{
    if (!G.have_volume) return fail(VP_E_STATE, "no volume");
    size_t need = (size_t)G.S.bnx * G.S.bny * G.S.bnz * (G.quant ? 2 : 8);
    if (bnx) *bnx = G.S.bnx;
    if (bny) *bny = G.S.bny;
    if (bnz) *bnz = G.S.bnz;
    if (brick) *brick = G.brick;
    if (radius) *radius = G.radius;
    if (dst)
    {
        if (bytes < need) return fail(VP_E_ARG, "bound table needs %zu bytes", need);
        HIPCHK(hipMemcpy(dst, G.d_bounds, need, hipMemcpyDeviceToHost));
    }
    return VP_OK;
}
int vp_get_pixel_table(const Param* p, float* dst, size_t count)
{
    int rc = ensure_device();
    if (rc) return rc;
    if (!p || !dst) return fail(VP_E_ARG, "vp_get_pixel_table: null argument");
    if (!G.have_volume || !G.have_cam) return fail(VP_E_STATE, "vp_get_pixel_table needs a volume and a camera");
    const size_t need = (size_t)p->width * p->height * 8;
    if (count < need) return fail(VP_E_ARG, "pixel table needs %zu floats", need);
    const float4* t = nullptr;
    rc = ensure_crawl_table(p, &t);
    if (rc) return rc;
    if (!t) return fail(VP_E_STATE, "no pixel table in this configuration (point filtering, or the tables are switched off)");
    HIPCHK(hipMemcpy(dst, t, need * sizeof(float), hipMemcpyDeviceToHost));
    return VP_OK;
}
int vp_get_exit_table(unsigned char* dst, size_t count)
{
    int rc = ensure_device();
    if (rc) return rc;
    if (!G.have_volume) return fail(VP_E_STATE, "vp_get_exit_table needs a volume");
    const size_t n = 3 * (size_t)G.S.nx * G.S.ny * G.S.nz;
    if (!dst || count < n) return fail(VP_E_ARG, "exit table needs %zu bytes", n);
    if (!G.d_exit) return fail(VP_E_STATE, "no exit table in this configuration (switched off, or no memory)");
    HIPCHK(hipStreamSynchronize(G.stream));
    HIPCHK(hipMemcpy(dst, G.d_exit, n, hipMemcpyDeviceToHost));
    return VP_OK;
}
int vp_get_sun_clip_table(unsigned short* dst, size_t count, float* step)
{
    int rc = ensure_device();
    if (rc) return rc;
    if (!G.have_volume || !G.have_sun) return fail(VP_E_STATE, "vp_get_sun_clip_table needs a volume and a sun");
    const size_t n = (size_t)G.S.nx * G.S.ny * G.S.nz;
    if (!dst || count < n) return fail(VP_E_ARG, "sun clip table needs %zu entries", n);
    const unsigned short* t = nullptr;
    float ds = 0.0f;
    rc = ensure_sun_clip(&t, &ds);
    if (rc) return rc;
    if (!t) return fail(VP_E_STATE, "no sun clip table in this configuration (sampler.h streams, point filtering, or switched off)");
    HIPCHK(hipMemcpy(dst, t, n * sizeof(unsigned short), hipMemcpyDeviceToHost));
    if (step) *step = ds;
    return VP_OK;
}
int vp_get_null_collision_table(const Param* p, float* dst, size_t count)
{
    int rc = ensure_device();
    if (rc) return rc;
    if (!p || !dst || !count || count > (1u << 24)) return fail(VP_E_ARG, "vp_get_null_collision_table: bad argument");
    struct Tmp { float* p = nullptr; ~Tmp() { if (p) (void)hipFree(p); } } tmp;
    HIPCHK(hipMalloc((void**)&tmp.p, count * sizeof(float)));
    ParamDev P;
    memcpy(&P, p, sizeof(Param));
    launch_thr_table(P, tmp.p, (unsigned)count, G.stream);
    HIPCHK(hipGetLastError());
    HIPCHK(hipStreamSynchronize(G.stream));
    HIPCHK(hipMemcpy(dst, tmp.p, count * sizeof(float), hipMemcpyDeviceToHost));
    return VP_OK;
}
int vp_get_opacity(float* dst, size_t count)
{
    if (!G.d_opacity) return fail(VP_E_STATE, "no opacity table");
    size_t n = (size_t)G.S.nx * G.S.ny * G.S.nz;
    if (count < n) return fail(VP_E_ARG, "opacity needs %zu floats", n);
    HIPCHK(hipStreamSynchronize(G.stream));
    HIPCHK(hipMemcpy(dst, G.d_opacity, n * sizeof(float), hipMemcpyDeviceToHost));
    return VP_OK;
}

}
```

### cuda-volpath_amd/volpath/__init__.py

```python
import ctypes as C
import os

import numpy as np

_HERE = os.path.dirname(os.path.abspath(__file__))
LIB_PATH = os.environ.get("VOLPATH_LIB", os.path.join(os.path.dirname(_HERE), "libvolpath_hip.so"))

EST_GLOBAL, EST_DECOMP, EST_BOUNDED = 0, 1, 2
RNG_SAMPLERH, RNG_PHILOX, RNG_PHILOX7 = 0, 1, 2
ENV_PASSIVE, ENV_MIS = 0, 1
TRACK_SPECTRAL, TRACK_SCALAR, TRACK_MULTI_CHANNEL = 0, 1, 2
ARITH_EXACT, ARITH_FAST = 0, 1
ARITH_FAST_REL_L2 = 2e-3
SUBPIXEL_MAX = 8

PART1_SYMBOLS = ["init_cuda", "set_texture_filter_mode", "free_cuda_buffers", "precompute_opacity", "init_envmap",
                 "free_envmap", "set_sun", "copy_inv_view_matrix", "copy_inv_model_matrix", "init_rng", "free_rng",
                 "render_kernel", "scale", "gamma_correct"]
PART2_SYMBOLS = ["vp_last_error", "vp_version", "vp_device_count", "vp_set_device", "vp_set_stream", "vp_get_stream", "vp_synchronize",
                 "vp_set_estimator", "vp_set_rng", "vp_set_envmap_sampling", "vp_get_env_tables", "vp_set_lookahead", "vp_set_tracking", "vp_set_bound_brick", "vp_set_shard", "vp_render_frames",
                 "vp_enable_counters", "vp_read_counters", "vp_render_time_ms", "vp_get_bound_table", "vp_get_opacity", "vp_get_pixel_table", "vp_get_null_collision_table", "vp_get_sun_clip_table", "vp_get_exit_table", "vp_set_exit_flights", "vp_render_class_time_ms", "vp_last_approach_mode", "vp_last_approach_table", "vp_last_light_const", "vp_last_lds_form", "vp_set_arithmetic", "vp_last_arithmetic", "vp_set_subpixel", "vp_get_subpixel", "vp_subpixel_offset", "vp_set_pipeline", "vp_last_pipelined", "vp_lookahead_stats", "vp_prepare", "vp_reserve_frames", "vp_get_pixel_lists",
                 "vp_render_frames_stats", "vp_render_adaptive", "vp_scale_by_count", "vp_stats_rel_error",
                 "vp_julia_voxelize", "vp_cloud_voxelize", "vp_test_math", "vp_test_rng", "vp_test_sample_density", "vp_test_hg", "vp_test_intersect_box",
                 "vp_test_eval_envmap", "vp_ctx_create", "vp_ctx_destroy", "vp_ctx_set_current", "vp_ctx_get_current", "vp_ctx_device",
                 "vp_accumulate", "vp_tile_owner", "vp_malloc", "vp_free", "vp_memset",
                 "vp_upload", "vp_download"]


class Float3(C.Structure):
    _fields_ = [("x", C.c_float), ("y", C.c_float), ("z", C.c_float)]


class Dim3(C.Structure):
    _fields_ = [("x", C.c_uint32), ("y", C.c_uint32), ("z", C.c_uint32)]


class Extent(C.Structure):
    _fields_ = [("width", C.c_size_t), ("height", C.c_size_t), ("depth", C.c_size_t)]


class Param(C.Structure):
    _fields_ = [("width", C.c_uint32), ("height", C.c_uint32), ("density", C.c_float), ("brightness", C.c_float),
                ("albedo", Float3), ("g", C.c_float), ("sigma_t", Float3)]


class Counters(C.Structure):
    _fields_ = [(n, C.c_uint64) for n in ("samples", "density_lookups", "density_loads", "bound_lookups",
                                          "opacity_lookups", "env_lookups", "scatters", "rng_draws")]

    def as_dict(self):
        return {n: int(getattr(self, n)) for n, _ in self._fields_}


class PixelStats(C.Structure):
    _fields_ = [("sum_y", C.c_double), ("sum_y2", C.c_double), ("n", C.c_uint32), ("flags", C.c_uint32)]


PIXEL_STATS_DTYPE = np.dtype([("sum_y", np.float64), ("sum_y2", np.float64), ("n", np.uint32), ("flags", np.uint32)])
STATS_FROZEN = 1


class Adaptive(C.Structure):
    _fields_ = [("rel_tol", C.c_float), ("floor_y", C.c_float), ("min_frames", C.c_int), ("round_frames", C.c_int)]


class AdaptiveResult(C.Structure):
    _fields_ = [("samples", C.c_uint64), ("rounds", C.c_uint32), ("active_left", C.c_uint32), ("frames_used", C.c_uint32)]

    def as_dict(self):
        return {n: int(getattr(self, n)) for n, _ in self._fields_}


class VolpathError(RuntimeError):
    pass


_lib = None


def lib():
    global _lib
    if _lib is None:
        if not os.path.exists(LIB_PATH):
            raise VolpathError(f"{LIB_PATH} is missing: run `make -C cuda-volpath_amd` (or __graft_entry__.build())")
        L = C.CDLL(LIB_PATH)
        L.vp_last_error.restype = C.c_char_p
        L.vp_version.restype = C.c_char_p
        L.vp_malloc.restype = C.c_void_p
        L.vp_malloc.argtypes = [C.c_size_t]
        L.vp_free.argtypes = [C.c_void_p]
        L.vp_memset.argtypes = [C.c_void_p, C.c_int, C.c_size_t]
        L.vp_upload.argtypes = [C.c_void_p, C.c_void_p, C.c_size_t]
        L.vp_download.argtypes = [C.c_void_p, C.c_void_p, C.c_size_t]
        L.vp_set_stream.argtypes = [C.c_void_p]
        L.vp_get_stream.restype = C.c_void_p
        L.vp_set_rng.argtypes = [C.c_int, C.c_uint32, C.c_uint32]
        L.vp_get_env_tables.argtypes = [C.c_void_p, C.c_void_p, C.POINTER(C.c_float)]
        L.vp_render_frames.argtypes = [C.c_void_p, C.c_int, C.c_int, C.POINTER(Param)]
        L.vp_render_frames_stats.argtypes = [C.c_void_p, C.c_void_p, C.c_int, C.c_int, C.POINTER(Param)]
        L.vp_render_adaptive.argtypes = [C.c_void_p, C.c_void_p, C.c_int, C.c_int, C.POINTER(Param), C.POINTER(Adaptive), C.POINTER(AdaptiveResult)]
        L.vp_scale_by_count.argtypes = [C.c_void_p, C.c_void_p, C.c_void_p, C.c_int, C.c_float]
        L.vp_stats_rel_error.argtypes = [C.c_void_p, C.c_void_p, C.c_int, C.c_float]
        L.vp_read_counters.argtypes = [C.POINTER(Counters), C.c_int]
        L.vp_render_time_ms.argtypes = [C.POINTER(C.c_double), C.POINTER(C.c_int), C.c_int]
        L.vp_get_bound_table.argtypes = [C.c_void_p, C.c_size_t] + [C.POINTER(C.c_int)] * 5
        L.vp_get_opacity.argtypes = [C.c_void_p, C.c_size_t]
        L.vp_get_pixel_table.argtypes = [C.POINTER(Param), C.c_void_p, C.c_size_t]
        L.vp_get_null_collision_table.argtypes = [C.POINTER(Param), C.c_void_p, C.c_size_t]
        L.vp_get_sun_clip_table.argtypes = [C.c_void_p, C.c_size_t, C.POINTER(C.c_float)]
        L.vp_render_class_time_ms.argtypes = [C.POINTER(C.c_double), C.POINTER(C.c_uint32), C.c_int]
        L.vp_prepare.argtypes = [C.POINTER(Param)]
        L.vp_set_subpixel.argtypes = [C.c_int]
        L.vp_subpixel_offset.argtypes = [C.c_uint, C.c_uint, C.c_int, C.c_int, C.POINTER(C.c_int), C.POINTER(C.c_int)]
        L.vp_get_pixel_lists.argtypes = [C.POINTER(Param), C.c_void_p, C.c_size_t, C.POINTER(C.c_uint32)]
        L.vp_julia_voxelize.argtypes = [C.c_int, C.c_void_p]
        L.vp_cloud_voxelize.argtypes = [C.c_int, C.c_uint32, C.c_void_p]
        L.vp_test_math.argtypes = [C.c_int, C.c_void_p, C.c_void_p, C.c_int]
        L.vp_test_rng.argtypes = [C.c_int] + [C.c_uint32] * 5 + [C.c_int, C.c_void_p]
        L.vp_test_sample_density.argtypes = [C.c_void_p, C.c_void_p, C.c_int]
        L.vp_test_hg.argtypes = [C.c_void_p] * 7 + [C.c_int]
        L.vp_test_intersect_box.argtypes = [C.c_void_p] * 5 + [C.c_int]
        L.vp_test_eval_envmap.argtypes = [C.c_void_p, C.c_void_p, C.c_int]
        L.vp_ctx_create.restype = C.c_void_p
        L.vp_ctx_create.argtypes = [C.c_int]
        L.vp_ctx_destroy.argtypes = [C.c_void_p]
        L.vp_ctx_set_current.argtypes = [C.c_void_p]
        L.vp_ctx_get_current.restype = C.c_void_p
        L.vp_accumulate.argtypes = [C.c_void_p, C.c_void_p, C.c_size_t]
        L.vp_tile_owner.argtypes = [C.c_uint, C.c_uint, C.c_int]
        L.init_cuda.argtypes = [C.c_void_p, Extent, C.c_bool, C.POINTER(Float3), C.POINTER(Float3)]
        L.init_cuda.restype = None
        L.set_texture_filter_mode.argtypes = [C.c_bool]
        L.precompute_opacity.argtypes = [C.POINTER(C.c_float)]
        L.init_envmap.argtypes = [C.c_void_p, C.c_int, C.c_int]
        L.set_sun.argtypes = [C.POINTER(C.c_float), C.POINTER(C.c_float)]
        L.copy_inv_view_matrix.argtypes = [C.POINTER(C.c_float), C.c_size_t]
        L.copy_inv_model_matrix.argtypes = [C.POINTER(C.c_float), C.c_size_t]
        L.init_rng.argtypes = [Dim3, Dim3, C.c_int, C.c_int]
        L.render_kernel.argtypes = [Dim3, Dim3, C.c_void_p, C.c_int, C.POINTER(Param)]
        L.scale.argtypes = [C.c_void_p, C.c_void_p, C.c_int, C.c_float]
        L.gamma_correct.argtypes = [C.c_void_p, C.c_void_p, C.c_int, C.c_float, C.c_float]
        for name in ("set_texture_filter_mode", "free_cuda_buffers", "precompute_opacity", "init_envmap",
                     "free_envmap", "set_sun", "copy_inv_view_matrix", "copy_inv_model_matrix", "init_rng",
                     "free_rng", "render_kernel", "scale", "gamma_correct"):
            getattr(L, name).restype = None
        _lib = L
    return _lib


def _chk(rc):
    if rc != 0:
        raise VolpathError(f"volpath error {rc}: {lib().vp_last_error().decode()}")


def _p(a):
    return a.ctypes.data_as(C.c_void_p)


def device_count():
    return lib().vp_device_count()


def make_param(width, height, density=800.0, g=0.877, brightness=1.0, albedo=(1, 1, 1), sigma_t=(1, 1, 1)):
    P = Param()
    P.width, P.height, P.density, P.brightness, P.g = width, height, density, brightness, g
    P.albedo = Float3(*albedo)
    P.sigma_t = Float3(*sigma_t)
    return P


def mat(P, X, Y, Z, R, G, B):
    f = np.float32
    st = [f(X) + f(R), f(Y) + f(G), f(Z) + f(B)]
    al = [f(X) / st[0], f(Y) / st[1], f(Z) / st[2]]
    m = max(st)
    st = [s / m for s in st]
    P.albedo = Float3(*[float(a) for a in al])
    P.sigma_t = Float3(*[float(s) for s in st])
    return P


DEFAULT_CAMERA = (0.0, 0.207912, 0.978148, 3.922986, 0.0, 0.978148, -0.207912, -0.782739, -1.0, 0.0, 0.0, 0.03)


class DeviceBuffer:

    def __init__(self, width, height):
        self.width, self.height = width, height
        self.nbytes = width * height * 16
        self.ptr = lib().vp_malloc(self.nbytes)
        if not self.ptr:
            raise VolpathError(lib().vp_last_error().decode())
# ... 201 lines not shown


def last_approach_table():
    return int(lib().vp_last_approach_table())


def reserve_frames(P, nframes):
    _chk(lib().vp_reserve_frames(C.byref(P), int(nframes)))


def lookahead_stats():
    a, b = C.c_uint(0), C.c_uint(0)
    _chk(lib().vp_lookahead_stats(C.byref(a), C.byref(b)))
    return int(a.value), int(b.value)


def last_lds_form():
    return int(lib().vp_last_lds_form())


def set_arithmetic(mode):
    _chk(lib().vp_set_arithmetic(mode))


def set_subpixel(s):
    _chk(lib().vp_set_subpixel(int(s)))


def get_subpixel():
    return int(lib().vp_get_subpixel())


def subpixel_offset(x, y, frame, s):
    i, j = C.c_int(0), C.c_int(0)
    _chk(lib().vp_subpixel_offset(int(x), int(y), int(frame), int(s), C.byref(i), C.byref(j)))
    return i.value, j.value


def last_arithmetic():
    return int(lib().vp_last_arithmetic())


def set_pipeline(on=True):
    _chk(lib().vp_set_pipeline(int(on)))


def last_pipelined():
    return int(lib().vp_last_pipelined())


def last_light_const():
    return bool(lib().vp_last_light_const())


def prepare(P):
    _chk(lib().vp_prepare(C.byref(P)))


def pixel_lists(P):
    cnt = (C.c_uint32 * 3)()
    _chk(lib().vp_get_pixel_lists(C.byref(P), None, 0, cnt))
    n = sum(cnt[:])
    out = np.empty(max(n, 1), np.uint32)
    _chk(lib().vp_get_pixel_lists(C.byref(P), _p(out), n, cnt))
    a, b = cnt[0], cnt[0] + cnt[1]
    return out[:a], out[a:b], out[b:n]


def bound_table(quantized=True):
    bnx, bny, bnz, brick, radius = (C.c_int() for _ in range(5))
    _chk(lib().vp_get_bound_table(None, 0, bnx, bny, bnz, brick, radius))
    out = np.empty((bnz.value, bny.value, bnx.value, 2), np.uint8 if quantized else np.float32)
    _chk(lib().vp_get_bound_table(_p(out), out.nbytes, bnx, bny, bnz, brick, radius))
    return out, brick.value, radius.value


def sun_clip_table(shape):
    out = np.empty(shape, np.uint16)
    step = C.c_float()
    _chk(lib().vp_get_sun_clip_table(_p(out), out.size, C.byref(step)))
    return out, step.value


def set_exit_flights(mode):
    _chk(lib().vp_set_exit_flights(mode))


def exit_table(shape):
    out = np.empty((3,) + tuple(shape), np.uint8)
    _chk(lib().vp_get_exit_table(_p(out), out.size))
    return out


def pixel_table(P):
    out = np.empty((P.height, P.width, 8), np.float32)
    _chk(lib().vp_get_pixel_table(C.byref(P), _p(out), out.size))
    return out


def null_collision_table(P, count):
    out = np.empty(count, np.float32)
    _chk(lib().vp_get_null_collision_table(C.byref(P), _p(out), out.size))
    return out


def opacity_table(shape):
    out = np.empty(shape, np.float32)
    _chk(lib().vp_get_opacity(_p(out), out.size))
    return out


def test_math(which, x):
    x = np.ascontiguousarray(x, np.float32)
    out = np.empty_like(x)
    _chk(lib().vp_test_math(which, _p(x), _p(out), x.size))
    return out


def test_rng(mode, x, y, frame, n, key=(0, 0)):
    out = np.empty(n, np.float32)
    _chk(lib().vp_test_rng(mode, x, y, frame, key[0], key[1], n, _p(out)))
    return out


def test_sample_density(pos):
    pos = np.ascontiguousarray(pos, np.float32)
    out = np.empty(pos.shape[0], np.float32)
    _chk(lib().vp_test_sample_density(_p(pos), _p(out), pos.shape[0]))
    return out


def test_hg(g, r0, r1, normal, cos_query):
    f = lambda a: np.ascontiguousarray(a, np.float32)
    g, r0, r1, normal, cos_query = f(g), f(r0), f(r1), f(normal), f(cos_query)
    n = g.size
    d = np.empty((n, 3), np.float32)
    e = np.empty(n, np.float32)
    _chk(lib().vp_test_hg(_p(g), _p(r0), _p(r1), _p(normal), _p(cos_query), _p(d), _p(e), n))
    return d, e


def test_intersect_box(origin, direction):
    o = np.ascontiguousarray(origin, np.float32)
    d = np.ascontiguousarray(direction, np.float32)
    n = o.shape[0]
    hit = np.empty(n, np.int32)
    tn = np.empty(n, np.float32)
    tf = np.empty(n, np.float32)
    _chk(lib().vp_test_intersect_box(_p(o), _p(d), _p(hit), _p(tn), _p(tf), n))
    return hit.astype(bool), tn, tf


def test_eval_envmap(direction):
    d = np.ascontiguousarray(direction, np.float32)
    out = np.empty_like(d)
    _chk(lib().vp_test_eval_envmap(_p(d), _p(out), d.shape[0]))
    return out


class Context:

    def __init__(self, device=0):
        self.h = lib().vp_ctx_create(device)
        if not self.h:
            raise VolpathError(lib().vp_last_error().decode())
        self._prev = []
# ... 42 lines not shown
```

### include/volpath.h

```cpp
#ifndef VOLPATH_H
#define VOLPATH_H

#include <stddef.h>
#include <stdint.h>
#ifndef __cplusplus
#include <stdbool.h>
#endif

#ifdef __cplusplus
extern "C" {
#endif

typedef struct { float x, y, z; } vp_float3;
typedef struct { float x, y, z, w; } vp_float4;
typedef struct { uint32_t x, y, z; } vp_dim3;
typedef struct { size_t width, height, depth; } vp_extent;

#ifndef VOLPATH_PARAM_DEFINED
#define VOLPATH_PARAM_DEFINED
typedef struct Param
{
    unsigned int width, height;
    float        density, brightness;
    vp_float3    albedo;
// ... 41 lines not shown
       VP_RNG_PHILOX7  = 2   };

const char* vp_last_error(void);
const char* vp_version(void);
int  vp_device_count(void);
int  vp_set_device(int device);

typedef struct vp_ctx vp_ctx;
vp_ctx* vp_ctx_create(int device);
int     vp_ctx_destroy(vp_ctx* ctx);
int     vp_ctx_set_current(vp_ctx* ctx);
vp_ctx* vp_ctx_get_current(void);
int     vp_ctx_device(void);
int     vp_accumulate(vp_float4* dst, const vp_float4* src, size_t n);
int  vp_set_stream(void* hip_stream);
void* vp_get_stream(void);
int  vp_synchronize(void);

int vp_set_estimator(int est);
int vp_set_rng(int mode, uint32_t key0, uint32_t key1);
enum { VP_TRACK_SPECTRAL = 0, VP_TRACK_SCALAR = 1, VP_TRACK_MULTI_CHANNEL = 2 };
int vp_set_tracking(int mode);
int vp_set_lookahead(int max_frames);
enum { VP_ENV_PASSIVE = 0, VP_ENV_MIS = 1 };
int vp_set_envmap_sampling(int mode);
enum { VP_ARITH_EXACT = 0, VP_ARITH_FAST = 1 };
#define VP_ARITH_FAST_REL_L2 2e-3
int vp_set_arithmetic(int mode);
#define VP_SUBPIXEL_MAX 8
int vp_set_subpixel(int s);
int vp_get_subpixel(void);
int vp_subpixel_offset(unsigned x, unsigned y, int frame, int s, int* i, int* j);
int vp_get_env_tables(float* cdf_y, float* cdf_x, float* pdfnorm_alt);
int vp_set_bound_brick(int brick);
int vp_set_shard(int rank, int world);
int vp_tile_owner(unsigned tx, unsigned ty, int world);

int vp_render_frames(vp_float4* d_output, int first_frame, int n_frames, const Param* p);

typedef struct { double sum_y, sum_y2; uint32_t n, flags; } vp_pixel_stats;
#define VP_STATS_FROZEN 1u
typedef struct { float rel_tol, floor_y; int min_frames, round_frames; } vp_adaptive;
typedef struct { uint64_t samples; uint32_t rounds, active_left, frames_used; } vp_adaptive_result;
int vp_render_frames_stats(vp_float4* d_output, vp_pixel_stats* d_stats, int first_frame, int n_frames, const Param* p);
int vp_render_adaptive(vp_float4* d_output, vp_pixel_stats* d_stats, int first_frame, int max_frames, const Param* p,
                       const vp_adaptive* a, vp_adaptive_result* result);
int vp_scale_by_count(vp_float4* dst, const vp_float4* src, const vp_pixel_stats* d_stats, int size, float scale);
int vp_stats_rel_error(float* dst, const vp_pixel_stats* d_stats, int size, float floor_y);

typedef struct
{
    uint64_t samples;
    uint64_t density_lookups;
    uint64_t density_loads;
    uint64_t bound_lookups;
    uint64_t opacity_lookups;
    uint64_t env_lookups;
    uint64_t scatters;
    uint64_t rng_draws;
} vp_counters;
int vp_enable_counters(int on);
int vp_read_counters(vp_counters* out, int reset);

int vp_render_time_ms(double* total_ms, int* launches, int reset);

int vp_render_class_time_ms(double ms[3], unsigned pixels[3], int reset);

int vp_last_approach_mode(void);
int vp_last_approach_table(void);
int vp_last_light_const(void);
int vp_last_lds_form(void);
int vp_last_arithmetic(void);
int vp_set_pipeline(int on);
int vp_last_pipelined(void);
int vp_lookahead_stats(unsigned* launched, unsigned* cancelled_in_flight);
int vp_prepare(const Param* p);
int vp_reserve_frames(const Param* p, int n_frames);
int vp_get_pixel_lists(const Param* p, uint32_t* dst, size_t count, unsigned counts[3]);

int vp_get_bound_table(void* dst, size_t bytes, int* bnx, int* bny, int* bnz, int* brick, int* radius);
int vp_get_opacity(float* dst, size_t count);
int vp_get_pixel_table(const Param* p, float* dst, size_t count);
int vp_get_sun_clip_table(unsigned short* dst, size_t count, float* step);
int vp_get_exit_table(unsigned char* dst, size_t count);
int vp_set_exit_flights(int mode);
int vp_get_null_collision_table(const Param* p, float* dst, size_t count);

int vp_test_math(int which, const float* in, float* out, int n);
int vp_test_rng(int mode, uint32_t x, uint32_t y, uint32_t frame, uint32_t k0, uint32_t k1, int n, float* out);
int vp_test_sample_density(const float* pos_xyz, float* out, int n);
int vp_test_hg(const float* g, const float* r0, const float* r1, const float* normal_xyz, const float* cos_query, float* dir_xyz,
               float* eval, int n);
int vp_test_intersect_box(const float* origin_xyz, const float* dir_xyz, int* hit, float* tnear, float* tfar, int n);
int vp_test_eval_envmap(const float* dir_xyz, float* rgb, int n);

int vp_julia_voxelize(int n, unsigned char* host_out);
int vp_cloud_voxelize(int n, uint32_t seed, float* host_out);

void* vp_malloc(size_t bytes);
int   vp_free(void* dptr);
int   vp_memset(void* dptr, int value, size_t bytes);
int   vp_upload(void* dptr, const void* src, size_t bytes);
int   vp_download(void* dst, const void* dptr, size_t bytes);

#ifdef __cplusplus
}
#endif
#endif
```

Before: 3352 Msamples/s.

## Precompute constant sun shadow-ray direction and skip box intersection inside volume

Adds a one-thread precompute kernel that checks whether the far-away sun point makes the shadow-ray direction and length effectively constant in float arithmetic. When it is, the shadow ray uses precomputed direction, inverse components and length instead of normalize, divisions and sqrt. The sun-clip kernel now also reports whether every clip distance ends before the ray nears the volume boundary; if so, sun shadow rays skip the box intersection and start at zero with the clipped end. This is meant to remove per-shadow-ray ALU work, but adds host syncs during setup and relies on bit-exact float certificates to keep results unchanged.

```diff
diff --git a/cuda-volpath_amd/csrc/vp_context.cpp b/cuda-volpath_amd/csrc/vp_context.cpp
--- a/cuda-volpath_amd/csrc/vp_context.cpp
+++ b/cuda-volpath_amd/csrc/vp_context.cpp
@@ -81,6 +81,8 @@
     if (knob("VP_NO_CRAWL_TABLE", 0, 1, v)) G.use_crawl_table = v == 0;
     if (knob("VP_NO_EMPTY_TABLE", 0, 1, v)) G.use_empty_table = v == 0;
     if (knob("VP_NO_SUN_CLIP", 0, 1, v)) G.use_sun_clip = v == 0;
+    if (knob("VP_NO_SUN_CONST", 0, 1, v)) G.use_sun_const = v == 0;
+    if (knob("VP_NO_SUN_INSIDE", 0, 1, v)) G.use_sun_inside = v == 0;
     if (knob("VP_DENSE_PERCENT", 0, 101, v)) G.dense_fraction = (float)v / 100.0f;
     if (knob("VP_NO_OPACITY_LDS", 0, 1, v)) G.opacity_lds = v == 0;
     if (knob("VP_NO_OPACITY_CELLS", 0, 1, v)) G.use_opacity_cells = v == 0;
@@ -136,7 +138,7 @@
     if (G.d_danger) HIPCHK(hipFree(G.d_danger));
     G.d_danger = nullptr;
     if (G.d_sunclip) HIPCHK(hipFree(G.d_sunclip));
-    G.d_sunclip = nullptr; G.sunclip_key.clear();
+    G.d_sunclip = nullptr; G.sunclip_key.clear(); G.sunclip_fail = 1u; G.sunray_key.clear();
     if (G.d_exit) HIPCHK(hipFree(G.d_exit));
     G.d_exit = nullptr;
     G.d_cells = G.d_bounds = nullptr;
@@ -526,7 +528,7 @@
                              D.class_last_end[0], D.class_last_end[1], D.class_last_end[2]})
             if (e) (void)hipEventDestroy(e);
         D.d_crawl.release(); D.d_seg.release(); D.d_sub_cls.release(); D.d_tiles.release(); D.d_act.release(); D.d_act_scratch.release();
-        for (void* q : {(void*)D.d_thr, (void*)D.d_sunclip, (void*)D.d_bound_codes, (void*)D.d_light_flag, (void*)D.d_tile_rows, (void*)D.d_tile_scratch})
+        for (void* q : {(void*)D.d_thr, (void*)D.d_sunclip, (void*)D.d_sunray, (void*)D.d_bound_codes, (void*)D.d_light_flag, (void*)D.d_tile_rows, (void*)D.d_tile_scratch})
             if (q) (void)hipFree(q);
         for (RenderTarget& t : D.target)
         {
diff --git a/cuda-volpath_amd/csrc/vp_device.h b/cuda-volpath_amd/csrc/vp_device.h
--- a/cuda-volpath_amd/csrc/vp_device.h
+++ b/cuda-volpath_amd/csrc/vp_device.h
@@ -398,31 +398,31 @@
     return f3{sp * st, cp, sp * -ct};
 }
 
-__device__ __forceinline__ bool intersect_box(f3 o, f3 d, const SceneDev& S, float& tnear, float& tfar)
+__device__ __forceinline__ bool intersect_box_ki(f3 o, f3 d, const SceneDev& S, unsigned mask, const float* ki, float& tnear, float& tfar)
 {
 #ifndef VP_EXP_BOX_PARALLEL
     float tmn, tmx;
     {
-        const float ir = 1.0f / d.x, tb = ir * (S.bmin[0] - o.x), tt = ir * (S.bmax[0] - o.x);
+        const float ir = (mask & 1u) ? ki[0] : 1.0f / d.x, tb = ir * (S.bmin[0] - o.x), tt = ir * (S.bmax[0] - o.x);
         tmn = fminf(tt, tb); tmx = fmaxf(tt, tb);
     }
     __builtin_amdgcn_sched_barrier(0);
     float tmn_y, tmx_y;
     {
-        const float ir = 1.0f / d.y, tb = ir * (S.bmin[1] - o.y), tt = ir * (S.bmax[1] - o.y);
+        const float ir = (mask & 2u) ? ki[1] : 1.0f / d.y, tb = ir * (S.bmin[1] - o.y), tt = ir * (S.bmax[1] - o.y);
         tmn_y = fminf(tt, tb); tmx_y = fmaxf(tt, tb);
     }
     __builtin_amdgcn_sched_barrier(0);
     float tmn_z, tmx_z;
     {
-        const float ir = 1.0f / d.z, tb = ir * (S.bmin[2] - o.z), tt = ir * (S.bmax[2] - o.z);
+        const float ir = (mask & 4u) ? ki[2] : 1.0f / d.z, tb = ir * (S.bmin[2] - o.z), tt = ir * (S.bmax[2] - o.z);
         tmn_z = fminf(tt, tb); tmx_z = fmaxf(tt, tb);
     }
     const float lt = max3(f3{tmn, tmn_y, tmn_z}), st_ = min3(f3{tmx, tmx_y, tmx_z});
     tnear = lt; tfar = st_;
     return st_ > lt && st_ >= 1e-3f;
 #endif
-    f3 invR = f3{1.0f / d.x, 1.0f / d.y, 1.0f / d.z};
+    f3 invR = f3{(mask & 1u) ? ki[0] : 1.0f / d.x, (mask & 2u) ? ki[1] : 1.0f / d.y, (mask & 4u) ? ki[2] : 1.0f / d.z};
     f3 tbot = invR * (f3{S.bmin[0], S.bmin[1], S.bmin[2]} - o);
     f3 ttop = invR * (f3{S.bmax[0], S.bmax[1], S.bmax[2]} - o);
     f3 tmin = f3{fminf(ttop.x, tbot.x), fminf(ttop.y, tbot.y), fminf(ttop.z, tbot.z)};
@@ -432,6 +432,10 @@
     tnear = largest_tmin;
     tfar  = smallest_tmax;
     return smallest_tmax > largest_tmin && smallest_tmax >= 1e-3f;
+}
+__device__ __forceinline__ bool intersect_box(f3 o, f3 d, const SceneDev& S, float& tnear, float& tfar)
+{
+    return intersect_box_ki(o, d, S, 0u, nullptr, tnear, tfar);
 }
 
 __device__ __forceinline__ bool intersect_box_inv(f3 o, f3 invR, const SceneDev& S, float& tnear, float& tfar)
diff --git a/cuda-volpath_amd/csrc/vp_integrator.h b/cuda-volpath_amd/csrc/vp_integrator.h
--- a/cuda-volpath_amd/csrc/vp_integrator.h
+++ b/cuda-volpath_amd/csrc/vp_integrator.h
@@ -128,6 +128,40 @@
     if (!(null_collision_in_empty_space(1.0f, sigma_t_prime, inv_sigma_t) == 1.0f)) atomicAnd(flag, 0u);
 }
 
+__global__ void sun_ray_const_k(SceneDev S, SunRayDev* out)
+{
+    if (threadIdx.x || blockIdx.x) return;
+    SunRayDev   R = {};
+    const float n[3] = {(float)S.nx, (float)S.ny, (float)S.nz};
+    f3 vmin, vmax;
+    float* const vmn = &vmin.x; float* const vmx = &vmax.x;
+    for (int c = 0; c < 3; c++)
+    {
+        const float e    = S.sun_dir[c] * 1e10f;
+        const float edge = (S.bmax[c] - S.bmin[c]) / n[c];
+        const float lo = S.bmin[c] - edge, hi = S.bmax[c] + edge;
+        const float va = e - lo, vb = e - hi;
+        if (va == e && vb == e) R.flags |= SUN_ABS_X << c;
+        const float aa = __builtin_fabsf(va), ab = __builtin_fabsf(vb);
+        vmn[c] = ((va < 0.0f) != (vb < 0.0f) || va == 0.0f || vb == 0.0f) ? 0.0f : fminf(aa, ab);
+        vmx[c] = fmaxf(aa, ab);
+        R.K[c] = 0.0f; R.KI[c] = 0.0f;
+    }
+    const float d0 = dot(vmin, vmin), d1 = dot(vmax, vmax);
+    if (d0 == d1 && d0 > 0.0f && d0 < __builtin_inff())
+    {
+        R.flags |= SUN_LEN_OK;
+        R.inv_len = rsqrt_(d0);
+        R.len     = sqrt_(d0);
+        for (int c = 0; c < 3; c++)
+            if (R.flags & (SUN_ABS_X << c))
+            {
+                R.K[c]  = (S.sun_dir[c] * 1e10f) * R.inv_len;
+                R.KI[c] = 1.0f / R.K[c];
+            }
+    }
+    *out = R;
+}
 #ifndef VP_LOCAL_MIN_WAVES
 #define VP_LOCAL_MIN_WAVES 6
 #endif
@@ -275,42 +309,65 @@
         const f3 sun_dir   = f3{S.sun_dir[0], S.sun_dir[1], S.sun_dir[2]};
         const f3 sun_power = f3{S.sun_power[0], S.sun_power[1], S.sun_power[2]};
         auto start_shadow = [&](f3 end, float inv_s, float den, unsigned stage) __attribute__((always_inline)) {
-            f3    sd = normalize(end - ro);
-            float tn, tf;
-            bool  hitv = intersect_box(ro, sd, S, tn, tf);
-            if (!hitv)
-            {
-                nee_a = f3{1.0f, 1.0f, 1.0f};
-                st    = EV_NEE;
+            const bool sun = stage == 0u;
+            unsigned   n   = 0xffffu;
+            if (RNG::kShadowSubstream && sun && L.sun_clip)
+            {
+                f3    pl = to_local(S, ro);
+                int   ci, cj, ck;
+                float w_;
+                axis_linear(pl.x, S.nx, ci, w_);
+                axis_linear(pl.y, S.ny, cj, w_);
+                axis_linear(pl.z, S.nz, ck, w_);
+                n = L.sun_clip[(size_t)((unsigned)ci + __umul24((unsigned)S.nx, (unsigned)cj + __umul24((unsigned)S.ny, (unsigned)ck)))];
+            }
+            const unsigned sf = sun ? L.sun.flags : 0u;
+            if (sf & SUN_LEN_OK)
+            {
+                const float il = L.sun.inv_len;
+                rd.x = (sf & SUN_ABS_X) ? L.sun.K[0] : (end.x - ro.x) * il;
+                rd.y = (sf & SUN_ABS_Y) ? L.sun.K[1] : (end.y - ro.y) * il;
+                rd.z = (sf & SUN_ABS_Z) ? L.sun.K[2] : (end.z - ro.z) * il;
             }
             else
-            {
-                if (tn < 0.0f) tn = 0.0f;
-                f3 se       = ro - end;
-                t_end       = fminf(tf, sqrt_(dot(se, se)));
-                dist        = tn;
+                rd = normalize(end - ro);
+            auto track = [&]() __attribute__((always_inline)) {
                 terms       = 0;
-                rd          = sd;
                 inv_sigma   = inv_s;
                 cur_density = den;
                 st          = ST_SHADOW;
                 rng_saved = rng.enter_shadow(2u * (unsigned)(int)nsc + stage);
-                if (COUNT) t_clip = 1e30f;
-                if (RNG::kShadowSubstream && stage == 0u && L.sun_clip)
-                {
-                    f3    pl = to_local(S, ro);
-                    int   ci, cj, ck;
-                    float w_;
-                    axis_linear(pl.x, S.nx, ci, w_);
-                    axis_linear(pl.y, S.ny, cj, w_);
-                    axis_linear(pl.z, S.nz, ck, w_);
-                    const unsigned n = L.sun_clip[(size_t)((unsigned)ci + __umul24((unsigned)S.nx, (unsigned)cj + __umul24((unsigned)S.ny, (unsigned)ck)))];
+            };
+            if (COUNT) t_clip = 1e30f;
+            if (!COUNT && (sf & SUN_INSIDE) && n != 0xffffu)
+            {
+                dist  = 0.0f;
+                t_end = (float)n * L.clip_ds;
+                track();
+            }
+            else
+            {
+                static_assert(SUN_ABS_X == 1u && SUN_ABS_Y == 2u && SUN_ABS_Z == 4u, "intersect_box_ki's axis mask");
+                float tn, tf;
+                const bool hitv = intersect_box_ki(ro, rd, S, (sf & SUN_LEN_OK) ? (sf & 7u) : 0u, L.sun.KI, tn, tf);
+                if (!hitv)
+                {
+                    nee_a = f3{1.0f, 1.0f, 1.0f};
+                    st    = EV_NEE;
+                }
+                else
+                {
+                    if (tn < 0.0f) tn = 0.0f;
+                    f3 se = ro - end;
+                    t_end = fminf(tf, (sf & SUN_LEN_OK) ? L.sun.len : sqrt_(dot(se, se)));
+                    dist  = tn;
                     if (n != 0xffffu)
                     {
                         const float tc = (float)n * L.clip_ds;
                         if (COUNT && !L.count_clips) t_clip = tc;
                         else t_end = fminf(t_end, tc);
                     }
+                    track();
                 }
             }
         };
diff --git a/cuda-volpath_amd/csrc/vp_kernels.h b/cuda-volpath_amd/csrc/vp_kernels.h
--- a/cuda-volpath_amd/csrc/vp_kernels.h
+++ b/cuda-volpath_amd/csrc/vp_kernels.h
@@ -55,6 +55,21 @@
 constexpr int EST_GLOBAL = 0, EST_DECOMP = 1, EST_BOUNDED = 2;
 constexpr int RNG_SAMPLERH = 0, RNG_PHILOX = 1, RNG_PHILOX7 = 2;
 
+enum : unsigned
+{
+    SUN_ABS_X = 1u, SUN_ABS_Y = 2u, SUN_ABS_Z = 4u,
+    SUN_LEN_OK = 8u,
+    SUN_INSIDE = 16u
+};
+struct SunRayDev
+{
+    unsigned flags;
+    float    inv_len;
+    float    len;
+    float    K[3];
+    float    KI[3];
+};
+
 struct LaunchDev
 {
     ParamDev P;
@@ -96,6 +111,7 @@
     unsigned        bound_pal[2];
     const float4* seg_table;
     unsigned sub_shift;
+    SunRayDev sun;
 };
 
 void launch_render(const SceneDev& S, const LaunchDev& L, int est, int rng, bool quant, bool count, int lds_form, bool mis, int trk,
@@ -123,7 +139,9 @@
                         hipStream_t st);
 void launch_danger(const SceneDev& S, bool quant, unsigned char* out, unsigned long long* marked, hipStream_t st);
 float sun_clip_step(const SceneDev& S);
-void launch_sun_clip(const SceneDev& S, const unsigned char* danger, float ds, unsigned short* out, hipStream_t st);
+void launch_sun_clip(const SceneDev& S, const unsigned char* danger, float ds, unsigned short* out, unsigned* fail, hipStream_t st);
+void launch_sun_ray_const(const SceneDev& S, SunRayDev* out, hipStream_t st);
+void launch_sun_ray_const_fast(const SceneDev& S, SunRayDev* out, hipStream_t st);
 void launch_empty_table(const SceneDev& S, unsigned width, unsigned height, const unsigned char* danger, float4* table, hipStream_t st);
 void launch_exit_table(const unsigned char* danger, unsigned char* planes, int nx, int ny, int nz, hipStream_t st);
 void launch_reduce(const LaunchDev& L, hipStream_t st);
diff --git a/cuda-volpath_amd/csrc/vp_kernels.hip b/cuda-volpath_amd/csrc/vp_kernels.hip
--- a/cuda-volpath_amd/csrc/vp_kernels.hip
+++ b/cuda-volpath_amd/csrc/vp_kernels.hip
@@ -144,7 +144,7 @@
     const unsigned mine = up ? 0xaau : 0x55u;
     *out = (unsigned char)((*out & ~mine) | bits);
 }
-__global__ __launch_bounds__(256) void sun_clip_k(SceneDev S, const unsigned char* danger, float ds, unsigned short* out)
+__global__ __launch_bounds__(256) void sun_clip_k(SceneDev S, const unsigned char* danger, float ds, unsigned short* out, unsigned* fail)
 {
     const size_t n   = (size_t)S.nx * S.ny * S.nz;
     const size_t idx = (size_t)blockIdx.x * blockDim.x + threadIdx.x;
@@ -162,12 +162,14 @@
     const f3 sun  = f3{S.sun_dir[0], S.sun_dir[1], S.sun_dir[2]};
     const f3 d    = normalize(sun * 1e10f - o);
     int      last = -1;
-    unsigned m    = 0;
+    unsigned m    = 0, first_near = 0xffffffffu;
     for (; m < 65000u; m++)
     {
         const f3    q  = to_local(S, o + d * ((float)m * ds));
         const float xa = fma_(q.x, (float)S.nx, -0.5f), xb = fma_(q.y, (float)S.ny, -0.5f), xc = fma_(q.z, (float)S.nz, -0.5f);
         if (!(xa >= -1.5f && xa <= (float)S.nx + 0.5f && xb >= -1.5f && xb <= (float)S.ny + 0.5f && xc >= -1.5f && xc <= (float)S.nz + 0.5f)) break;
+        if (first_near == 0xffffffffu && !(xa >= 2.0f && xa <= (float)S.nx - 3.0f && xb >= 2.0f && xb <= (float)S.ny - 3.0f && xc >= 2.0f && xc <= (float)S.nz - 3.0f))
+            first_near = m;
         int   a, b, c;
         float w_;
         axis_linear(q.x, S.nx, a, w_);
@@ -176,6 +178,7 @@
         if (danger[(size_t)a + (size_t)S.nx * ((size_t)b + (size_t)S.ny * c)] & 1) last = (int)m;
     }
     out[idx] = (m >= 65000u || !(d.x == d.x && d.y == d.y && d.z == d.z)) ? 0xffffu : (unsigned short)min(last + 2, 0xfffe);
+    if (fail && out[idx] != 0xffffu && (first_near <= (unsigned)(last + 2) || !(6.0f * ds >= 2e-3f))) atomicOr(fail, 1u);
 }
 template <bool QUANT>
 __device__ bool chord_has_positive_minimum(const SceneDev& S, f3 ro, f3 rd)
@@ -1063,6 +1066,10 @@
 {
     hipLaunchKernelGGL(light_identity_k, dim3(1), dim3(256), 0, st, P, local ? 1 : 0, mask, flag);
 }
+void launch_sun_ray_const(const SceneDev& S, SunRayDev* out, hipStream_t st)
+{
+    hipLaunchKernelGGL(sun_ray_const_k, dim3(1), dim3(1), 0, st, S, out);
+}
 void launch_thr_table(const ParamDev& P, float* table, unsigned count, hipStream_t st)
 {
     hipLaunchKernelGGL(thr_table_k, dim3(1), dim3(64), 0, st, P, table, count);
@@ -1286,10 +1293,10 @@
     const float cx = (S.bmax[0] - S.bmin[0]) / (float)S.nx, cy = (S.bmax[1] - S.bmin[1]) / (float)S.ny, cz = (S.bmax[2] - S.bmin[2]) / (float)S.nz;
     return 0.25f * std::fmin(std::fmin(cx, cy), cz);
 }
-void launch_sun_clip(const SceneDev& S, const unsigned char* danger, float ds, unsigned short* out, hipStream_t st)
+void launch_sun_clip(const SceneDev& S, const unsigned char* danger, float ds, unsigned short* out, unsigned* fail, hipStream_t st)
 {
     size_t n = (size_t)S.nx * S.ny * S.nz;
-    hipLaunchKernelGGL(sun_clip_k, dim3((unsigned)((n + 255) / 256)), dim3(256), 0, st, S, danger, ds, out);
+    hipLaunchKernelGGL(sun_clip_k, dim3((unsigned)((n + 255) / 256)), dim3(256), 0, st, S, danger, ds, out, fail);
 }
 void launch_empty_table(const SceneDev& S, unsigned width, unsigned height, const unsigned char* danger, float4* table, hipStream_t st)
 {
diff --git a/cuda-volpath_amd/csrc/vp_kernels_fast.hip b/cuda-volpath_amd/csrc/vp_kernels_fast.hip
--- a/cuda-volpath_amd/csrc/vp_kernels_fast.hip
+++ b/cuda-volpath_amd/csrc/vp_kernels_fast.hip
@@ -74,6 +74,11 @@
     hipLaunchKernelGGL(fast::light_identity_k, dim3(1), dim3(256), 0, st, P, local ? 1 : 0, mask, flag);
 }
 
+void launch_sun_ray_const_fast(const SceneDev& S, SunRayDev* out, hipStream_t st)
+{
+    hipLaunchKernelGGL(fast::sun_ray_const_k, dim3(1), dim3(1), 0, st, S, out);
+}
+
 void launch_approach_fast(const SceneDev& S, const LaunchDev& L, int est, int rng, bool quant, hipStream_t st)
 {
     if ((est != EST_GLOBAL && est != EST_DECOMP) || (rng != RNG_PHILOX && rng != RNG_PHILOX7))
diff --git a/cuda-volpath_amd/csrc/vp_render.cpp b/cuda-volpath_amd/csrc/vp_render.cpp
--- a/cuda-volpath_amd/csrc/vp_render.cpp
+++ b/cuda-volpath_amd/csrc/vp_render.cpp
@@ -208,6 +208,7 @@
     A.per_frame = (size_t)PL.n_general + PL.n_light + PL.n_miss;
     if (A.per_frame == 0) return VP_OK;
     if ((rc = ensure_sun_clip(&L.sun_clip, &L.clip_ds))) return rc;
+    if ((rc = ensure_sun_ray(L.sun_clip, L.clip_ds, &L.sun))) return rc;
     L.count_clips = getenv("VP_DEBUG_COUNT_CLIPS") ? 1u : 0u;
     if ((rc = exit_flights(L))) return rc;
     A.light_const = false;
@@ -658,6 +659,8 @@
     if ((rc = ensure_crawl_table(&fine, &table))) return rc;
     if ((rc = ensure_pixel_lists(p, table, sh))) return rc;
     if (G.have_sun && (rc = ensure_sun_clip(&sc, &ds))) return rc;
+    SunRayDev sr;
+    if (G.have_sun && (rc = ensure_sun_ray(sc, ds, &sr))) return rc;
     if (G.est == VP_EST_GLOBAL && G.n_light && (rc = ensure_thr_table(p, &thr))) return rc;
     if (G.est == VP_EST_DECOMP && G.approach_fshift_max >= 6 && approach_possible(table, G.n_general) && (rc = ensure_segment_table(p, table, &seg))) return rc;
     HIPCHK(hipStreamSynchronize(G.stream));
diff --git a/cuda-volpath_amd/csrc/vp_state.h b/cuda-volpath_amd/csrc/vp_state.h
--- a/cuda-volpath_amd/csrc/vp_state.h
+++ b/cuda-volpath_amd/csrc/vp_state.h
@@ -177,6 +177,13 @@
     unsigned short* d_sunclip = nullptr;
     float       sunclip_ds  = 0.0f;
     std::vector<unsigned char> sunclip_key;
+    bool        use_sun_const = true;
+    bool        use_sun_inside = true;
+    struct SunRayScratch { SunRayDev r; unsigned clip_fail; };
+    SunRayScratch* d_sunray = nullptr;
+    unsigned    sunclip_fail = 1u;
+    SunRayDev   sunray      = {};
+    std::vector<unsigned char> sunray_key;
     bool        use_light_const = true;
     int         last_approach = 0;
     int         last_approach_table = 0;
@@ -262,6 +269,7 @@
 Param  subpixel_param(const Param* p);
 int    subpixel_check(const Param* p);
 int    ensure_sun_clip(const unsigned short** out, float* ds);
+int    ensure_sun_ray(const unsigned short* sun_clip, float clip_ds, SunRayDev* out);
 int    ensure_light_const(const Param* p, bool* out);
 int    ensure_light_identity(const Param* p, bool* out);
 int    ensure_fast_identity(const Param* p, bool* out);
diff --git a/cuda-volpath_amd/csrc/vp_tables.cpp b/cuda-volpath_amd/csrc/vp_tables.cpp
--- a/cuda-volpath_amd/csrc/vp_tables.cpp
+++ b/cuda-volpath_amd/csrc/vp_tables.cpp
@@ -8,6 +8,10 @@
     (void)la_quiesce();
 
     if (!G.have_volume) return fail(VP_E_STATE, "precompute_opacity before init_cuda");
+    {
+        const double l2 = (double)dir[0] * dir[0] + (double)dir[1] * dir[1] + (double)dir[2] * dir[2];
+        if (!(l2 >= 0.25 && l2 <= 4.0)) return fail(VP_E_ARG, "precompute_opacity needs a unit direction (length %g)", std::sqrt(l2));
+    }
     size_t n = (size_t)G.S.nx * G.S.ny * G.S.nz;
     if (!G.d_opacity) HIPCHK(hipMalloc((void**)&G.d_opacity, n * sizeof(float)));
     SceneDev S = G.S;
@@ -151,6 +155,15 @@
     return VP_OK;
 }
 
+static bool ensure_sun_scratch()
+{
+    if (!G.d_sunray && hipMalloc((void**)&G.d_sunray, sizeof(State::SunRayScratch)) != hipSuccess)
+    {
+        (void)hipGetLastError();
+        G.d_sunray = nullptr;
+    }
+    return G.d_sunray != nullptr;
+}
 int ensure_sun_clip(const unsigned short** out, float* ds)
 {
     *out = nullptr; *ds = 0.0f;
@@ -175,12 +188,40 @@
         SceneDev S = G.S;
         S.linear   = 1;
         G.sunclip_ds = sun_clip_step(S);
-        launch_sun_clip(S, G.d_danger, G.sunclip_ds, G.d_sunclip, G.stream);
-        HIPCHK(hipGetLastError());
+        G.sunclip_fail = 1u;
+        unsigned* const d_fail = ensure_sun_scratch() ? &G.d_sunray->clip_fail : nullptr;
+        if (d_fail) HIPCHK(hipMemsetAsync(d_fail, 0, sizeof(unsigned), G.stream));
+        launch_sun_clip(S, G.d_danger, G.sunclip_ds, G.d_sunclip, d_fail, G.stream);
+        HIPCHK(hipGetLastError());
+        if (d_fail) HIPCHK(hipMemcpyAsync(&G.sunclip_fail, d_fail, sizeof(unsigned), hipMemcpyDeviceToHost, G.stream));
         HIPCHK(hipStreamSynchronize(G.stream));
         G.sunclip_key = key;
     }
     *out = G.d_sunclip; *ds = G.sunclip_ds;
+    return VP_OK;
+}
+
+int ensure_sun_ray(const unsigned short* sun_clip, float clip_ds, SunRayDev* out)
+{
+    *out = SunRayDev{};
+    if (!G.use_sun_const || !G.have_sun) return VP_OK;
+    struct K { int nx, ny, nz, arith; float bmin[3], bmax[3], sun[3]; };
+    std::vector<unsigned char> key(sizeof(K), 0);
+    K* k = reinterpret_cast<K*>(key.data());
+    k->nx = G.S.nx; k->ny = G.S.ny; k->nz = G.S.nz; k->arith = G.arith;
+    memcpy(k->bmin, G.S.bmin, sizeof k->bmin); memcpy(k->bmax, G.S.bmax, sizeof k->bmax); memcpy(k->sun, G.S.sun_dir, sizeof k->sun);
+    if (key != G.sunray_key)
+    {
+        if (!ensure_sun_scratch()) return VP_OK;
+        if (G.arith == VP_ARITH_FAST) launch_sun_ray_const_fast(G.S, &G.d_sunray->r, G.stream);
+        else launch_sun_ray_const(G.S, &G.d_sunray->r, G.stream);
+        HIPCHK(hipGetLastError());
+        HIPCHK(hipMemcpyAsync(&G.sunray, &G.d_sunray->r, sizeof(SunRayDev), hipMemcpyDeviceToHost, G.stream));
+        HIPCHK(hipStreamSynchronize(G.stream));
+        G.sunray_key = key;
+    }
+    *out = G.sunray;
+    if (G.use_sun_inside && sun_clip && (out->flags & SUN_LEN_OK) && G.sunclip_fail == 0u && (float)0xfffe * clip_ds < out->len) out->flags |= SUN_INSIDE;
     return VP_OK;
 }
 
@@ -451,6 +492,20 @@
     if (step) *step = ds;
     return VP_OK;
 }
+int vp_get_sun_ray_certificates(unsigned* flags)
+{
+    int rc = ensure_device();
+    if (rc) return rc;
+    if (!flags) return fail(VP_E_ARG, "vp_get_sun_ray_certificates: null argument");
+    if (!G.have_volume || !G.have_sun) return fail(VP_E_STATE, "vp_get_sun_ray_certificates needs a volume and a sun");
+    const unsigned short* t = nullptr;
+    float ds = 0.0f;
+    SunRayDev R;
+    if ((rc = ensure_sun_clip(&t, &ds))) return rc;
+    if ((rc = ensure_sun_ray(t, ds, &R))) return rc;
+    *flags = R.flags;
+    return VP_OK;
+}
 int vp_get_null_collision_table(const Param* p, float* dst, size_t count)
 {
     int rc = ensure_device();
diff --git a/cuda-volpath_amd/volpath/__init__.py b/cuda-volpath_amd/volpath/__init__.py
--- a/cuda-volpath_amd/volpath/__init__.py
+++ b/cuda-volpath_amd/volpath/__init__.py
@@ -19,7 +19,7 @@
                  "render_kernel", "scale", "gamma_correct"]
 PART2_SYMBOLS = ["vp_last_error", "vp_version", "vp_device_count", "vp_set_device", "vp_set_stream", "vp_get_stream", "vp_synchronize",
                  "vp_set_estimator", "vp_set_rng", "vp_set_envmap_sampling", "vp_get_env_tables", "vp_set_lookahead", "vp_set_tracking", "vp_set_bound_brick", "vp_set_shard", "vp_render_frames",
-                 "vp_enable_counters", "vp_read_counters", "vp_render_time_ms", "vp_get_bound_table", "vp_get_opacity", "vp_get_pixel_table", "vp_get_null_collision_table", "vp_get_sun_clip_table", "vp_get_exit_table", "vp_set_exit_flights", "vp_render_class_time_ms", "vp_last_approach_mode", "vp_last_approach_table", "vp_last_light_const", "vp_last_lds_form", "vp_set_arithmetic", "vp_last_arithmetic", "vp_set_subpixel", "vp_get_subpixel", "vp_subpixel_offset", "vp_set_pipeline", "vp_last_pipelined", "vp_lookahead_stats", "vp_prepare", "vp_reserve_frames", "vp_get_pixel_lists",
+                 "vp_enable_counters", "vp_read_counters", "vp_render_time_ms", "vp_get_bound_table", "vp_get_opacity", "vp_get_pixel_table", "vp_get_null_collision_table", "vp_get_sun_clip_table", "vp_get_sun_ray_certificates", "vp_get_exit_table", "vp_set_exit_flights", "vp_render_class_time_ms", "vp_last_approach_mode", "vp_last_approach_table", "vp_last_light_const", "vp_last_lds_form", "vp_set_arithmetic", "vp_last_arithmetic", "vp_set_subpixel", "vp_get_subpixel", "vp_subpixel_offset", "vp_set_pipeline", "vp_last_pipelined", "vp_lookahead_stats", "vp_prepare", "vp_reserve_frames", "vp_get_pixel_lists",
                  "vp_render_frames_stats", "vp_render_adaptive", "vp_scale_by_count", "vp_stats_rel_error",
                  "vp_julia_voxelize", "vp_cloud_voxelize", "vp_test_math", "vp_test_rng", "vp_test_sample_density", "vp_test_hg", "vp_test_intersect_box",
                  "vp_test_eval_envmap", "vp_ctx_create", "vp_ctx_destroy", "vp_ctx_set_current", "vp_ctx_get_current", "vp_ctx_device",
@@ -108,6 +108,7 @@
         L.vp_get_pixel_table.argtypes = [C.POINTER(Param), C.c_void_p, C.c_size_t]
         L.vp_get_null_collision_table.argtypes = [C.POINTER(Param), C.c_void_p, C.c_size_t]
         L.vp_get_sun_clip_table.argtypes = [C.c_void_p, C.c_size_t, C.POINTER(C.c_float)]
+        L.vp_get_sun_ray_certificates.argtypes = [C.POINTER(C.c_uint)]
         L.vp_render_class_time_ms.argtypes = [C.POINTER(C.c_double), C.POINTER(C.c_uint32), C.c_int]
         L.vp_prepare.argtypes = [C.POINTER(Param)]
         L.vp_set_subpixel.argtypes = [C.c_int]
@@ -475,6 +476,15 @@
     return out, step.value
 
 
+SUN_ABS_X, SUN_ABS_Y, SUN_ABS_Z, SUN_LEN_OK, SUN_INSIDE = 1, 2, 4, 8, 16
+
+
+def sun_ray_certificates():
+    flags = C.c_uint()
+    _chk(lib().vp_get_sun_ray_certificates(C.byref(flags)))
+    return flags.value
+
+
 def set_exit_flights(mode):
     _chk(lib().vp_set_exit_flights(mode))
 
diff --git a/include/volpath.h b/include/volpath.h
--- a/include/volpath.h
+++ b/include/volpath.h
@@ -147,6 +147,12 @@
 int vp_get_opacity(float* dst, size_t count);
 int vp_get_pixel_table(const Param* p, float* dst, size_t count);
 int vp_get_sun_clip_table(unsigned short* dst, size_t count, float* step);
+#define VP_SUN_ABS_X 1u
+#define VP_SUN_ABS_Y 2u
+#define VP_SUN_ABS_Z 4u
+#define VP_SUN_LEN_OK 8u
+#define VP_SUN_INSIDE 16u
+int vp_get_sun_ray_certificates(unsigned* flags);
 int vp_get_exit_table(unsigned char* dst, size_t count);
 int vp_set_exit_flights(int mode);
 int vp_get_null_collision_table(const Param* p, float* dst, size_t count);
```

New measurement: 3505 Msamples/s (median of 6 runs). +4.6%, better.
